# uber/aresdb

Hardware: AMD Instinct MI355X
Metric: rows/sec, 1B-row filter -> group-by-agg (whole job) (higher is better)
Workload: dtype u32 keys / f64 sums; 1 GPU; C3: filter d1<90 -> dims [floor(ts,3600), d1, d2, d3] (4 x uint32) -> SUM(m float32 -> float64) via HashReduce, validity bitmaps with 1% nulls, shard resident in HBM; rows_per_gpu=1000000000, batch_rows=67108864, batches=15, streams_per_query=2, parallelism=1 shard(s), one per GPU

## Files before the change

aresdb_amd/abi.py:

```python
import ctypes as C
import os

_HERE = os.path.dirname(os.path.abspath(__file__))
REPO_ROOT = os.path.dirname(_HERE)
LIB_DIR = os.environ.get("ARES_LIB_DIR") or os.path.join(_HERE, "lib")

AGGR_SUM_UNSIGNED, AGGR_SUM_SIGNED, AGGR_SUM_FLOAT = 1, 2, 3
AGGR_MIN_UNSIGNED, AGGR_MIN_SIGNED, AGGR_MIN_FLOAT = 4, 5, 6
AGGR_MAX_UNSIGNED, AGGR_MAX_SIGNED, AGGR_MAX_FLOAT = 7, 8, 9
AGGR_HLL, AGGR_AVG_FLOAT = 10, 11

(Bool, Int8, Uint8, Int16, Uint16, Int32, Uint32, Float32, Int64, Uint64, Float64, GeoPoint,
 UUID) = range(13)
ConstInt, ConstFloat, ConstGeoPoint, ConstUUID = range(4)
(Negate, Not, BitwiseNot, IsNull, IsNotNull, Noop, GetWeekStart, GetMonthStart, GetQuarterStart,
 GetYearStart, GetDayOfMonth, GetDayOfYear, GetMonthOfYear, GetQuarterOfYear, GetHLLValue,
 ArrayLength) = range(16)
(And, Or, Equal, NotEqual, LessThan, LessThanOrEqual, GreaterThan, GreaterThanOrEqual, Plus, Minus,
 Multiply, Divide, Mod, BitwiseAnd, BitwiseOr, BitwiseXor, Floor, ArrayContains,
 ArrayElementAt) = range(19)
(VectorPartyInput, ScratchSpaceInput, ConstantInput, ForeignColumnInput,
 ArrayVectorPartyInput) = range(5)
ScratchSpaceOutput, MeasureOutput, DimensionOutput = range(3)
NUM_DIM_WIDTH = 5
# ... 55 lines not shown


class ForeignColumnVector(C.Structure):
    _fields_ = [("RecordIDs", C.c_void_p), ("Batches", C.c_void_p), ("BaseBatchID", C.c_int32),
                ("NumBatches", C.c_int32), ("NumRecordsInLastBatch", C.c_int32),
                ("TimezoneLookup", C.c_void_p), ("TimezoneLookupSize", C.c_int16),
                ("DataType", C.c_int), ("DefaultValue", DefaultValue)]


class ArrayVectorPartySlice(C.Structure):
    _fields_ = [("OffsetLengthVector", C.c_void_p), ("ValueOffsetAdj", C.c_uint32),
                ("DataType", C.c_int), ("Length", C.c_uint32)]


class _InputUnion(C.Union):
    _fields_ = [("Constant", ConstantVector), ("VP", VectorPartySlice),
                ("ScratchSpace", ScratchSpaceVector), ("ForeignVP", ForeignColumnVector),
                ("ArrayVP", ArrayVectorPartySlice)]


class InputVector(C.Structure):
    _fields_ = [("Vector", _InputUnion), ("Type", C.c_int)]


class DimensionVector(C.Structure):
    _fields_ = [("DimValues", C.c_void_p), ("HashValues", C.c_void_p), ("IndexVector", C.c_void_p),
                ("VectorCapacity", C.c_int), ("NumDimsPerDimWidth", C.c_uint8 * NUM_DIM_WIDTH)]


class DimensionOutputVector(C.Structure):
    _fields_ = [("DimValues", C.c_void_p), ("DimNulls", C.c_void_p), ("DataType", C.c_int)]


class MeasureOutputVector(C.Structure):
    _fields_ = [("Values", C.c_void_p), ("DataType", C.c_int), ("AggFunc", C.c_int)]


class _OutputUnion(C.Union):
    _fields_ = [("ScratchSpace", ScratchSpaceVector), ("Dimension", DimensionOutputVector),
                ("Measure", MeasureOutputVector)]


class OutputVector(C.Structure):
    _fields_ = [("Vector", _OutputUnion), ("Type", C.c_int)]


class GeoShapeBatch(C.Structure):
    _fields_ = [("LatLongs", C.c_void_p), ("TotalNumPoints", C.c_int32), ("TotalWords", C.c_uint8)]


class FusedExpr(C.Structure):
    _fields_ = [("lhs", InputVector), ("rhs", InputVector), ("arity", C.c_int), ("functor", C.c_int),
                ("outType", C.c_int)]


class FusedSelect(C.Structure):
    _fields_ = [("numFilters", C.c_int), ("filters", FusedExpr * 4), ("numDims", C.c_int),
                ("dims", FusedExpr * 8)]


class FusedJoin(C.Structure):
    _fields_ = [("key", InputVector), ("index", CuckooHashIndex)]


class FusedJoinSelect(C.Structure):
    _fields_ = [("numFilters", C.c_int), ("filters", FusedExpr * 4), ("numJoins", C.c_int), ("joins", FusedJoin * 2),
                ("numForeignFilters", C.c_int), ("foreignFilters", FusedExpr * 4), ("foreignFilterJoin", C.c_int * 4),
                ("numDims", C.c_int), ("dims", FusedExpr * 8), ("dimJoin", C.c_int * 8)]


class JoinedColumn(C.Structure):
    _fields_ = [("column", InputVector), ("out", C.c_void_p)]


class JoinColumns(C.Structure):
    _fields_ = [("numFilters", C.c_int), ("filters", FusedExpr * 4), ("join", FusedJoin), ("numColumns", C.c_int),
                ("columns", JoinedColumn * 4)]


class GeoShapeColumn(C.Structure):
    _fields_ = [("numFilters", C.c_int), ("filters", FusedExpr * 4), ("shapes", GeoShapeBatch), ("points", InputVector),
                ("inOrOut", C.c_int), ("out", C.c_void_p)]


class LocalTimeColumn(C.Structure):
    _fields_ = [("numFilters", C.c_int), ("filters", FusedExpr * 4), ("time", InputVector), ("join", FusedJoin),
                ("zone", InputVector), ("outType", C.c_int), ("out", C.c_void_p)]


ABI_SIZES = {CGoCallResHandle: 16, RecordID: 8, CuckooHashIndex: 40, DefaultValue: 24,
             VectorPartySlice: 56, ScratchSpaceVector: 16, ConstantVector: 24,
             ForeignColumnVector: 72, ArrayVectorPartySlice: 24, InputVector: 80,
             DimensionVector: 40, DimensionOutputVector: 24, MeasureOutputVector: 16,
             OutputVector: 32, GeoShapeBatch: 16}

_VP, _S, _I = C.c_void_p, C.c_void_p, C.c_int

ALGORITHM_SYMBOLS = {
    "InitIndexVector": [_VP, C.c_uint32, _I, _S, _I],
    "HashLookup": [InputVector, _VP, _VP, _I, _VP, C.c_uint32, CuckooHashIndex, _S, _I],
    "UnaryTransform": [InputVector, OutputVector, _VP, _I, _VP, C.c_uint32, _I, _S, _I],
    "UnaryFilter": [InputVector, _VP, _VP, _I, _VP, _I, _VP, C.c_uint32, _I, _S, _I],
    "BinaryTransform": [InputVector, InputVector, OutputVector, _VP, _I, _VP, C.c_uint32, _I, _S, _I],
    "BinaryFilter": [InputVector, InputVector, _VP, _VP, _I, _VP, _I, _VP, C.c_uint32, _I, _S, _I],
    "Sort": [DimensionVector, _I, _S, _I],
    "Reduce": [DimensionVector, _VP, DimensionVector, _VP, _I, _I, _I, _S, _I],
# ... 55 lines not shown
        for p in (memory_path, algorithm_path):
            if not os.path.exists(p):
                raise FileNotFoundError(
                    f"{name}: shared library {p} is missing — build it first "
                    f"(python -c 'import __graft_entry__ as g; g.build()')")
        self._mem = C.CDLL(memory_path, mode=os.RTLD_NOW | os.RTLD_LOCAL)
        self._algo = self._mem if algorithm_path == memory_path else \
            C.CDLL(algorithm_path, mode=os.RTLD_NOW | os.RTLD_LOCAL)
        self.algorithm_path, self.memory_path = algorithm_path, memory_path
        for sym, argtypes in ALGORITHM_SYMBOLS.items():
            fn = getattr(self._algo, sym)
            fn.argtypes, fn.restype = argtypes, CGoCallResHandle
            setattr(self, "_" + sym, fn)
        for sym, argtypes in MEMORY_SYMBOLS.items():
            fn = getattr(self._mem, sym)
            fn.argtypes, fn.restype = argtypes, CGoCallResHandle
            setattr(self, "_" + sym, fn)
        self._mem.GetFlags.argtypes, self._mem.GetFlags.restype = [], C.c_uint32
        self.has_profiler = hasattr(self._algo, "AresProfilerEnable")
        if self.has_profiler:
            self._algo.AresProfilerEnable.argtypes, self._algo.AresProfilerEnable.restype = [C.c_int], None
            self._algo.AresProfilerReport.argtypes = [C.c_char_p, C.c_size_t]
            self._algo.AresProfilerReport.restype = C.c_size_t

    def call(self, sym, *args):
        return _check(getattr(self, "_" + sym)(*args))

    def mem_driver_calls(self, device=0):
        if not hasattr(self._mem, "AresMemDriverCalls"):
            return None
        m, f, t = C.c_size_t(0), C.c_size_t(0), C.c_size_t(0)
        self._mem.AresMemDriverCalls.argtypes = [C.c_int, C.POINTER(C.c_size_t), C.POINTER(C.c_size_t), C.POINTER(C.c_size_t)]
        self._mem.AresMemDriverCalls.restype = None
        self._mem.AresMemDriverCalls(device, C.byref(m), C.byref(f), C.byref(t))
        return {"mallocs": m.value, "frees": f.value, "trims": t.value}

    def rtc_wait(self):
        if not hasattr(self._algo, "AresRtcWait"):
            return None
        c = (C.c_long * 3)()
        self._algo.AresRtcWait.argtypes, self._algo.AresRtcWait.restype = [C.POINTER(C.c_long)], C.c_size_t
        n = self._algo.AresRtcWait(c)
        return {"kernels": int(n), "compiles": int(c[0]), "disk_hits": int(c[1]), "evictions": int(c[2])}

    def reload_env(self):
        if hasattr(self._algo, "AresReloadEnv"):
            self._algo.AresReloadEnv.argtypes, self._algo.AresReloadEnv.restype = [], None
            self._algo.AresReloadEnv()

    def flags(self):
        return self._mem.GetFlags()

    @property
    def has_fused_select(self):
        return hasattr(self._algo, "AresFusedFilterSelect")

    def fused_filter_select(self, query, batch_rows, limit, out_keys, stream=None, device=0):
        fn = self._algo.AresFusedFilterSelect
        fn.argtypes = [C.POINTER(FusedSelect), C.c_int, C.c_int, DimensionVector, _S, _I]
        fn.restype = CGoCallResHandle
        return _check(fn(C.byref(query), int(batch_rows), int(limit), out_keys, stream, device))

    def select_stats(self):
        c = (C.c_ulonglong * 4)()
        self._algo.AresSelectStats.argtypes, self._algo.AresSelectStats.restype = [C.POINTER(C.c_ulonglong)], None
        self._algo.AresSelectStats(c)
        return {"batches": int(c[0]), "declined": int(c[1]), "tiles": int(c[2]), "rows": int(c[3])}

    @property
    def has_fused_join_select(self):
        return hasattr(self._algo, "AresFusedFilterJoinSelect")

    def fused_filter_join_select(self, query, batch_rows, limit, out_keys, stream=None, device=0):
        fn = self._algo.AresFusedFilterJoinSelect
        fn.argtypes = [C.POINTER(FusedJoinSelect), C.c_int, C.c_int, DimensionVector, _S, _I]
        fn.restype = CGoCallResHandle
        return _check(fn(C.byref(query), int(batch_rows), int(limit), out_keys, stream, device))

    def select_join_stats(self):
        c = (C.c_ulonglong * 5)()
        self._algo.AresSelectJoinStats.argtypes, self._algo.AresSelectJoinStats.restype = [C.POINTER(C.c_ulonglong)], None
        self._algo.AresSelectJoinStats(c)
        return {"batches": int(c[0]), "declined": int(c[1]), "tiles": int(c[2]), "rows": int(c[3]), "probed": int(c[4])}

    @property
    def has_join_columns(self):
        return hasattr(self._algo, "AresJoinColumnsRun")

    def join_column_bytes(self, rows, dtype):
        fn = self._algo.AresJoinColumnBytes
        fn.argtypes, fn.restype = [C.c_int, C.c_int], C.c_size_t
        return int(fn(int(rows), int(dtype)))

    def join_columns_run(self, query, batch_rows, stream=None, device=0):
        fn = self._algo.AresJoinColumnsRun
        fn.argtypes = [C.POINTER(JoinColumns), C.c_int, C.POINTER(VectorPartySlice), _S, _I]
        fn.restype = CGoCallResHandle
        slices = (VectorPartySlice * 4)()
        res = _check(fn(C.byref(query), int(batch_rows), slices, stream, device))
        assert res == batch_rows
        return slices

    def join_column_stats(self):
        c = (C.c_ulonglong * 4)()
        self._algo.AresJoinColumnStats.argtypes, self._algo.AresJoinColumnStats.restype = [C.POINTER(C.c_ulonglong)], None
        self._algo.AresJoinColumnStats(c)
# ... 90 lines not shown
```

aresdb_amd/csrc/algo/common.hpp:

```cpp
#pragma once

#include <hip/hip_runtime.h>

#include <atomic>
#include <chrono>
#include <cstdint>
#include <cstdio>
#include <cstdlib>
#include <cstring>
#include <stdexcept>
#include <string>

#include "ares_algorithm.h"

namespace ares {

class AlgorithmError : public std::runtime_error {
 public:
  explicit AlgorithmError(const std::string &m) : std::runtime_error(m) {}
};

void slow_trace(const char *what, double ms);
bool hr_trace_enabled();
class SlowScope {
 public:
  explicit SlowScope(const char *what) : what_(what), t0_(std::chrono::steady_clock::now()) {}
  ~SlowScope() {
    const double ms = std::chrono::duration<double, std::milli>(std::chrono::steady_clock::now() - t0_).count();
    if (ms > 5.0) slow_trace(what_, ms);
  }
  SlowScope(const SlowScope &) = delete;
  SlowScope &operator=(const SlowScope &) = delete;

 private:
  const char *what_;
  std::chrono::steady_clock::time_point t0_;
};
inline void hip_check(hipError_t e, const char *what) {
  if (e != hipSuccess) {
    (void)hipGetLastError();
    throw AlgorithmError(std::string("ERROR: ") + what + ": " + hipGetErrorString(e));
  }
}

template <class F>
inline void hip_check_timed(F &&call, const char *what) {
  SlowScope slow(what);
  hip_check(call(), what);
}
#define hip_check(expr, what) hip_check_timed([&]() -> hipError_t { return (expr); }, what)

extern void (*g_memNoteActivity)();
inline void mem_note_activity() {
  if (g_memNoteActivity) g_memNoteActivity();
}
inline void check_launch(const char *what) {
  mem_note_activity();
  hip_check(hipGetLastError(), what);
}

void flush_deferred(int device);
bool fuse_pending_into_hash_reduce(int device, hipStream_t stream, const DimensionVector &in, const uint8_t *inValues,
                                   const DimensionVector &out, uint8_t *outValues, int valueBytes, int length, int aggFunc,
                                   int *groups);
void invalidate_filter_journal(int device, const uint32_t *indexVector);
bool global_table_forced();
bool deferral_hooks_active();
void grouped_note_write(int device, const void *ptr, size_t bytes);
void grouped_note_write(int device, const DimensionVector &v);
void grouped_materialize_for_read(int device, const void *ptr, size_t bytes);
void grouped_trim(int device);
void flush_deferred_for_inputs(int device, const void *a, size_t aBytes, const void *b, size_t bBytes);
void flush_deferred_for_vector(int device, const DimensionVector &v, const void *values, size_t valueBytes);
void drop_skipped_outputs(int device, const void *a, size_t aBytes, const void *b, size_t bBytes);

bool defer_fill(int device, hipStream_t stream, void *dst, size_t bytes, uint64_t pattern, int unit);
bool pending_fill_exact(int device, const void *dst, size_t bytes, uint64_t *pattern, int *unit);
bool pending_fill_tail(int device, const void *base, int width, int length, int *prev, uint64_t *pattern);
void retire_fills_for_write(int device, const void *ptr, size_t bytes);
void materialize_fills_for_read(int device, const void *ptr, size_t bytes);
void launch_pending_writers(int device, const void *ptr, size_t bytes);
bool virtual_iota_peek(int device, const uint32_t *indexVector, int n, bool consume = false);
void materialize_index_vector(int device, const uint32_t *indexVector);
void settle_dimension_vector(int device, const DimensionVector &v, bool rowsOnly = false);
void temp_stats(size_t *handedOut, size_t *cached);

struct CallStream {
  hipStream_t stream;
  bool known;
};
extern thread_local CallStream t_callStream;
class CallStreamScope {
 public:
  CallStreamScope(void *stream, const char *entry) : saved_(t_callStream), slow_(entry) {
    t_callStream = CallStream{reinterpret_cast<hipStream_t>(stream), true};
  }
  ~CallStreamScope() { t_callStream = saved_; }
  CallStreamScope(const CallStreamScope &) = delete;
  CallStreamScope &operator=(const CallStreamScope &) = delete;

 private:
  CallStream saved_;
  SlowScope slow_;
};

#define ARES_ABI_BEGIN_NOFLUSH(device)                 \
  CGoCallResHandle resHandle = {nullptr, nullptr};     \
  try {                                                \
    ares::hip_check(hipSetDevice(device), "hipSetDevice");  \
    ares::CallStreamScope callStreamScope_(cudaStream, __func__);  \
    ares::mem_note_activity();                                      \
    (void)ares::deferral_hooks_active();

#define ARES_ABI_BEGIN(device)     \
  ARES_ABI_BEGIN_NOFLUSH(device)   \
  ares::flush_deferred(device);

#define ARES_ABI_END(name)                                            \
  }                                                                   \
  catch (std::exception & e) {                                        \
    fprintf(stderr, "Exception happened when doing %s: %s\n", name, e.what()); \
// ... 93 lines not shown
```

aresdb_amd/csrc/algo/hash_reduce_lds.hip:

```cpp
#include <hip/hip_runtime.h>

#include <atomic>
#include <functional>
#include <map>
#include <mutex>
#include <string>
#include <unordered_map>

#include <memory>
#include <mutex>
#include <vector>

#include "aggregate.hpp"
#include "common.hpp"
#include "device_model.hpp"
#include "ares_extensions.h"
#include "dim_layout.hpp"
#include "fast_eval.hpp"
#include "hash_reduce_lds.hpp"
#include "hr_kernels.hpp"
#include "hr_rtc.hpp"
#include "sort_reduce_fused.hpp"

namespace ares {
// ... 273 lines not shown
  ws.capA = ((2ull * (static_cast<uint64_t>(rowsA) / numParts) + 2 * kSlots) | 63ull) + 18;
  ws.capB = 0;
  ws.lineRecords = lineRecords;
  size_t bBytes = 0;
  if (streams > 0) {
    const uint64_t mean = (static_cast<uint64_t>(rowsB) / (static_cast<uint64_t>(numParts) * streams)) << record_stream_slack();
    if (lineRecords == static_cast<int>(kCompactLineRecords)) {
      ws.capB = static_cast<uint32_t>(((2 * mean + 64) / kCompactLineRecords + 2) | 1ull);
      bBytes = 128ull * ws.capB * numParts * streams;
    } else if (lineRecords) {
      ws.capB = static_cast<uint32_t>(((2 * mean + 64 + 7) / 8 * 8) | 8ull);
      bBytes = sizeof(uint32_t) * rwB * static_cast<size_t>(ws.capB) * numParts * streams;
    } else {
      ws.capB = static_cast<uint32_t>(((2 * mean + 64) | 15ull) + 6);
      bBytes = sizeof(uint32_t) * rwB * static_cast<size_t>(ws.capB) * numParts * streams;
    }
  }
  bBytes = (bBytes + 255) / 256 * 256;
  const size_t headBytes = (sizeof(uint32_t) * (numParts + 8) + 255) / 256 * 256;
  const size_t countsBytes = (sizeof(uint32_t) * static_cast<size_t>(numParts) * (streams > 0 ? streams : 1) + 255) / 256 * 256;
  const size_t aBytes = (sizeof(uint4) * ws.capA * numParts + 255) / 256 * 256;
  r.buf.reset(new StreamBuffer(headBytes + countsBytes + aBytes + bBytes + 256, stream));
  uint8_t *base = r.buf->as<uint8_t>();
  ws.cursorsA = reinterpret_cast<uint32_t *>(base);
  ws.outCount = ws.cursorsA + numParts;
  ws.countsB = reinterpret_cast<uint32_t *>(base + headBytes);
  ws.recA = reinterpret_cast<uint4 *>(base + headBytes + countsBytes);
  ws.recB = reinterpret_cast<uint32_t *>(base + headBytes + countsBytes + aBytes);
  r.headBytes = headBytes;
  hip_check(hipMemsetAsync(base, 0, headBytes, stream), "hipMemsetAsync");
}

struct MergeResult {
  uint32_t groups, overflow, stale, needGeneric;
};
MergeResult read_result(const Workspace &ws, hipStream_t stream) {
  uint32_t w[4] = {0, 0, 0, 0};
  read_back_u32(ws.outCount, w, 4, stream);
  return MergeResult{w[0], w[1], w[2], w[3]};
}
uint32_t *result_slot() {
  static EnvSwitch<bool> on("ARES_RESULT_PINNED", [](const char *e) { return e && e[0] == '1'; });
  return on.get() ? reinterpret_cast<uint32_t *>(pinned_words()) : nullptr;
}
MergeResult read_result_pinned(hipStream_t stream) {
  hip_check(hipStreamSynchronize(stream), "hipStreamSynchronize");
  const volatile uint32_t *w = result_slot();
  return MergeResult{w[0], w[1], w[2], w[3]};
}

}

void grouped_note_write(int device, const void *ptr, size_t bytes) {
  sorted_state_note_write(device, ptr, bytes);
  const uint8_t *lo = static_cast<const uint8_t *>(ptr);
  const uint8_t *hi = lo + (bytes ? bytes : 1);
  std::lock_guard<std::mutex> lock(g_groupedMutex);
  for (size_t i = 0; i < g_grouped.size();) {
    GroupedState &st = g_grouped[i];
    if (st.device == device && state_overlaps(st, lo, hi)) {
      const uint8_t *vlo = st.values, *vhi = st.values + static_cast<size_t>(st.valueBytes) * st.size;
      if (st.lazyValues && !(lo <= vlo && vhi <= hi)) materialize_values(st);
      g_grouped.erase(g_grouped.begin() + i);
    } else {
      i++;
    }
  }
}

void grouped_materialize_for_read(int device, const void *ptr, size_t bytes) {
  if (!ptr) return;
  const uint8_t *lo = static_cast<const uint8_t *>(ptr);
  const uint8_t *hi = lo + (bytes ? bytes : 1);
  std::lock_guard<std::mutex> lock(g_groupedMutex);
  for (GroupedState &st : g_grouped) {
    if (st.device != device || !st.lazyValues) continue;
    const uint8_t *vlo = st.values, *vhi = st.values + static_cast<size_t>(st.valueBytes) * st.size;
    if (vlo < hi && lo < vhi) materialize_values(st);
  }
}

void grouped_trim(int device) {
  std::vector<void *> idle;
  {
    std::lock_guard<std::mutex> lock(g_rangesMutex);
    for (size_t i = 0; i < g_freeRanges.size();)
      if (g_freeRanges[i].first == device) {
        idle.push_back(g_freeRanges[i].second);
        g_freeRanges[i] = g_freeRanges.back();
        g_freeRanges.pop_back();
      } else {
        i++;
      }
    for (size_t i = 0; i < g_freeImages.size();)
      if (g_freeImages[i].first == device) {
        idle.push_back(g_freeImages[i].second);
        g_freeImages[i] = g_freeImages.back();
        g_freeImages.pop_back();
      } else {
        i++;
      }
  }
  for (void *p : idle) (void)hipFree(p);
}

void grouped_note_write(int device, const DimensionVector &v) {
// ... 97 lines not shown
      memset(&none, 0, sizeof(none));
      rtc_merge_launch(leanMerge, none, inputKeys.DimValues, capacity, inputValues, static_cast<uint32_t>(start), outputKeys.DimValues,
                       capacity, outputValues, ws, stream, nullptr, result_slot());
    } else {
      generic_merge();
    }
    res = (leanMerge && result_slot()) ? read_result_pinned(stream) : read_result(ws, stream);
    mem_note_dim_rows(device, outputKeys, 0, res.groups);
    mem_note_write(device, outputValues, static_cast<size_t>(a.width) * res.groups);
    if (leanMerge && res.needGeneric && !res.overflow && !(grouped && res.stale)) {
      hip_check(hipMemsetAsync(ws.outCount, 0, 4 * sizeof(uint32_t), stream), "hipMemsetAsync");
      if (outRanges) hip_check(hipMemsetAsync(outRanges, 0, kRangesBytes, stream), "hipMemsetAsync");
      generic_merge();
      res = read_result(ws, stream);
      mem_note_dim_rows(device, outputKeys, 0, res.groups);
      mem_note_write(device, outputValues, static_cast<size_t>(a.width) * res.groups);
    }
#undef ARES_HR_MERGE_ND
#undef ARES_HR_MERGE
    if (hr_trace_enabled())
      fprintf(stderr, "hash_reduce_lds: length %d start %d rows %d streams %d capA %llu capB %u partBits %d -> groups %u overflow %u stale %u\n",
              length, start, rows, streams, static_cast<unsigned long long>(ws.capA), ws.capB, partBits, res.groups, res.overflow, res.stale);
    r.buf->mark_idle();
    if (grouped && res.stale) {
      grouped_note_write(device, inputKeys.DimValues, static_cast<size_t>(L.rowBytes) * capacity);
      grouped = false;
      continue;
    }
    break;
  }
  if (res.overflow) {
    static bool told = false;
    if (!told) {
      told = true;
      fprintf(stderr, "libalgorithm: a hash-partition region overflowed (skewed hashes?): HashReduce falls back to the global table\n");
    }
    return -1;
  }
  if (outRanges) {
    GroupedState s{device, outputKeys.DimValues, outputValues, capacity, slots, a.width, static_cast<int>(res.groups),
                   partBits, outRangesRef};
    if (res.groups > 0) grouped_register(s);
  }
  return static_cast<int>(res.groups);
}

static void fused_note_first_batch(size_t shape, int groups) {
  if (!shape || groups < 0) return;
  std::lock_guard<std::mutex> lock(g_shapeMutex);
  if (g_firstBatchGroups.size() > 4096) g_firstBatchGroups.clear();
  g_firstBatchGroups[shape] = groups;
}

int fused_hash_reduce_run(int device, const FusedPlanD &plan, int batchRows, const DimensionVector &prevKeys,
                          const uint8_t *prevValues, int prevSize, const DimensionVector &outKeys, uint8_t *outValues,
                          const AggSpec &a, hipStream_t stream) {
  SlotWidths slots;
  if (!slot_widths(outKeys.NumDimsPerDimWidth, &slots)) return kFusedUnavailable;
  const int nd = slots.nd;
  const bool narrow = fused_plan_narrow(plan, nd);
  const int mw = plan.measureWidth;
  const int64_t length = static_cast<int64_t>(batchRows) + prevSize;
  if (length == 0) return 0;
  const int partBits = std::max(part_bits_for(length), narrow ? 2 : 0);
  const int numParts = 1 << partBits;
  const size_t prevCapacity = static_cast<size_t>(prevKeys.VectorCapacity);
  const size_t outCapacity = static_cast<size_t>(outKeys.VectorCapacity);
  if (narrow && !(batchRows > 0 && rtc_scan_available())) return kFusedUnavailable;
  GroupedState outOld;
  const bool outFound = image_enabled() && grouped_lookup(device, outKeys.DimValues, outValues, outCapacity, slots, mw, &outOld);
  grouped_note_write(device, outValues, static_cast<size_t>(mw) * outCapacity);
  grouped_note_write(device, outKeys.DimValues, slots.row_bytes() * outCapacity);
  GroupedState prev;
  const bool found = prevSize > 0 && grouped_lookup(device, prevKeys.DimValues, prevValues, prevCapacity, slots, mw, &prev) &&
                     prev.partBits == partBits && prev.size == prevSize;
  bool grouped = found && prev.ranges != nullptr;
  const std::shared_ptr<uint32_t> outRangesRef = grouped_enabled() ? take_ranges(device) : nullptr;
  uint32_t *outRanges = outRangesRef.get();
  MergeResult res{0, 0, 0, 0};
  hr::Widen widen;
  widen.mode = mw == 8 ? 1 : 0;
  widen.rk = plan.measure.f.rk;
  widen.dtype = plan.measureDtype;
  size_t shape = 0;
  int expected = prevSize;
  bool known = prevSize > 0;
  const bool rtc = batchRows > 0 && rtc_scan_available();
  if (rtc && prevSize == 0) {
    const RtcSpec spec = rtc_spec_scan(plan, nd, 0, false);
    shape = std::hash<std::string>()(std::string(reinterpret_cast<const char *>(&spec), sizeof(spec)));
    std::lock_guard<std::mutex> lock(g_shapeMutex);
    auto it = g_firstBatchGroups.find(shape);
    if (it != g_firstBatchGroups.end()) {
      expected = it->second;
      known = true;
    }
  }
  const int chunkTiles = compact_enabled() ? rtc_compact_chunk_tiles(batchRows, partBits) : 0;
  const bool compact = chunkTiles > 0;
  const RtcKind leanKind = compact ? RTC_SCAN_COMPACT : RTC_SCAN_LINES16;
  RtcKernel lean, table, tableMerge, narrowMerge;
  SlowScope slowWhole("fused_hash_reduce_run");
  const bool wantLean = rtc && expected >= lean_min_groups() && (known || lean_min_groups() <= 0);
  const bool wantTable = rtc && !wantLean && (known || narrow);
  if (wantLean) lean = rtc_lookup(device, rtc_spec_scan(plan, nd, partBits, compact));
  else if (wantTable) table = rtc_lookup(device, rtc_spec_table_scan(plan, nd, partBits, a, widen));
  int imageMode = 0;
  RtcKernel imageMerge;
  std::shared_ptr<uint8_t> imageOut;
  uint32_t knownOut = 0;
  if (image_enabled() && wantLean && lean) {
    if (found && prev.image) imageMode = 2;
    else if (prevSize == 0 || grouped) imageMode = 1;
    if (imageMode) imageMerge = rtc_lookup(device, rtc_spec_merge(plan, nd, partBits, a, widen, compact, false, imageMode));
    if (!imageMerge) imageMode = 0;
  }
  if (imageMode == 2) {
    const bool mine = outFound && outOld.lineage == prev.lineage && outOld.image && outOld.image != prev.image &&
                      outOld.partBits == partBits && outOld.size <= prevSize && prev.parentGen != 0 && outOld.gen == prev.parentGen;
    knownOut = mine ? static_cast<uint32_t>(outOld.size) : 0u;
    imageOut = mine ? outOld.image : take_image(device);
    if (imageOut && !mine) hip_check(hipMemsetAsync(image_counts(imageOut.get()), 0xFF, sizeof(uint32_t) * kMaxPartitions, stream), "hipMemsetAsync");
  } else {
    if (imageMode == 1) imageOut = take_image(device);
    if (prevSize > 0) grouped_materialize_for_read(device, prevValues, static_cast<size_t>(mw) * prevSize);
  }
  if (imageMode && !imageOut) {
    imageMode = 0;
    knownOut = 0;
    if (prevSize > 0) grouped_materialize_for_read(device, prevValues, static_cast<size_t>(mw) * prevSize);
  }
  {
    if (hr_trace_enabled())
      fprintf(stderr, "fused_hash_reduce_run: batch %d prev %d partBits %d | found %d (state: size %d partBits %d ranges %d image %d lazy %d) grouped %d "
                      "| lean %d table %d compact %d narrow %d -> image mode %d knownOut %u\n",
              batchRows, prevSize, partBits, found ? 1 : 0, found ? prev.size : -1, found ? prev.partBits : -1, found && prev.ranges ? 1 : 0,
              found && prev.image ? 1 : 0, found && prev.lazyValues ? 1 : 0, grouped ? 1 : 0, lean ? 1 : 0, table ? 1 : 0, compact ? 1 : 0,
              narrow ? 1 : 0, imageMode, knownOut);
  }
  if (narrow && !imageMode) {
    narrowMerge = rtc_lookup(device, rtc_spec_merge(plan, nd, partBits, a, widen, wantLean && compact,
                                                    wantTable || (prevSize > 0 && !grouped)));
    if (!narrowMerge) return kFusedUnavailable;
  }
  if (narrow && !(wantLean ? lean : table)) return kFusedUnavailable;
  bool launched = false;
  for (;;) {
    const bool prevToA = narrow && prevSize > 0 && !grouped && imageMode != 2;
    if (narrow && !imageMode) {
      narrowMerge = rtc_lookup(device, rtc_spec_merge(plan, nd, partBits, a, widen, lean && compact, table || prevToA));
      if (!narrowMerge) return launched ? -1 : kFusedUnavailable;
      if (table) tableMerge = narrowMerge;
    }
    launched = true;
    const int streams = batchRows > 0 ? (lean ? rtc_scan_grid(batchRows) : table ? 0 : grid_for(batchRows)) : 0;
    Regions r;
    {
      SlowScope slow("make_regions");
      const int64_t rowsA = !lean ? length : (prevSize > 0 && !grouped && imageMode != 2) ? prevSize : 0;
      make_regions(r, partBits, rowsA, batchRows, streams, lean ? 4 : 3, stream,
                   !lean ? 0 : compact ? static_cast<int>(kCompactLineRecords) : 8);
    }
    Workspace &ws = r.ws;
    ws.widen = widen;
    ws.chunkRows = static_cast<uint32_t>(chunkTiles) * 4096u;
    ws.rowBase = static_cast<uint32_t>(prevSize);
    ws.prevRanges = (grouped && imageMode != 2) ? prev.ranges.get() : nullptr;
    ws.outRanges = outRanges;
    Workspace wsPrev = ws;
    wsPrev.streams = 0;
    RtcKernel leanMerge = imageMode ? imageMerge
                          : narrow  ? (lean ? narrowMerge : nullptr)
                          : (lean && (prevSize == 0 || grouped)) ? rtc_lookup(device, rtc_spec_merge(plan, nd, partBits, a, widen, compact)) : nullptr;
    RtcImageArgs imageArgs{nullptr, nullptr, nullptr, nullptr, 0u};
    if (imageMode) {
      imageArgs.in = imageMode == 2 ? prev.image.get() : nullptr;
      imageArgs.inCount = imageMode == 2 ? image_counts(prev.image.get()) : nullptr;
      imageArgs.out = imageOut.get();
      imageArgs.outCount = image_counts(imageOut.get());
      imageArgs.knownOut = knownOut;
    }
    const RtcImageArgs *imagePtr = imageMode ? &imageArgs : nullptr;
    if (prevToA) {
      const DimLayoutD prevLayout = make_dim_layout(prevKeys.NumDimsPerDimWidth);
      const int64_t tiles = (static_cast<int64_t>(prevSize) + kTileRows - 1) / kTileRows;
      ARES_LAUNCH("hr_partition_kernel", hr_partition_kernel, static_cast<int>(tiles < 256 ? tiles : 256), kThreads, stream,
                  prevKeys.DimValues, prevLayout, prevCapacity, prevValues, a, prevSize, wsPrev);
    }
    if (outRanges && !leanMerge && !tableMerge) hip_check(hipMemsetAsync(outRanges, 0, kRangesBytes, stream), "hipMemsetAsync");
#define ARES_FUSED_CASE(ND)                                                                                            \
  case ND:                                                                                                             \
    if (prevSize > 0 && !grouped && !narrow && imageMode != 2) {                                                       \
      if (mw == 8)                                                                                                     \
        ARES_LAUNCH("hr_partition4_kernel", (hr_partition4_kernel<ND, 8>), grid_for(prevSize), kThreads, stream,        \
                    prevKeys.DimValues, prevCapacity, prevValues, 0u, a, prevSize, wsPrev, 0);                         \
      else                                                                                                             \
        ARES_LAUNCH("hr_partition4_kernel", (hr_partition4_kernel<ND, 4>), grid_for(prevSize), kThreads, stream,        \
                    prevKeys.DimValues, prevCapacity, prevValues, 0u, a, prevSize, wsPrev, 0);                         \
    }                                                                                                                  \
    if (batchRows > 0 && lean)                                                                                         \
      rtc_scan_launch(lean, leanKind, plan, static_cast<uint32_t>(prevSize), batchRows, ws, stream);                   \
    else if (batchRows > 0 && table)                                                                                   \
      rtc_scan_launch(table, RTC_SCAN_TABLE, plan, static_cast<uint32_t>(prevSize), batchRows, ws, stream);            \
    else if (batchRows > 0)                                                                                            \
      ARES_LAUNCH("hr_fused_scan_kernel", hr_fused_scan_kernel<ND>, streams, kThreads, stream, plan,                   \
                  static_cast<uint32_t>(prevSize), a, batchRows, ws);                                                  \
    if (leanMerge || tableMerge)                                                                                       \
      rtc_merge_launch(leanMerge ? leanMerge : tableMerge, plan, prevKeys.DimValues, prevCapacity, prevValues,         \
                       static_cast<uint32_t>(prevSize), outKeys.DimValues, outCapacity, outValues, ws, stream, imagePtr, \
                       result_slot());                                                                                 \
    else if (lean)                                                                                                     \
      ARES_LAUNCH("hr_fused_merge_kernel", (hr_fused_merge_kernel<ND, 4>), numParts, kThreads, stream, plan,            \
                  prevKeys.DimValues, prevCapacity, prevValues, static_cast<uint32_t>(prevSize), outKeys.DimValues,    \
                  outCapacity, outValues, a, ws);                                                                      \
    else                                                                                                               \
      ARES_LAUNCH("hr_fused_merge_kernel", (hr_fused_merge_kernel<ND, 3>), numParts, kThreads, stream, plan,            \
                  prevKeys.DimValues, prevCapacity, prevValues, static_cast<uint32_t>(prevSize), outKeys.DimValues,    \
                  outCapacity, outValues, a, ws);                                                                      \
    break;
    switch (nd) {
      ARES_FUSED_CASE(1) ARES_FUSED_CASE(2) ARES_FUSED_CASE(3) ARES_FUSED_CASE(4)
      default:
        if (batchRows > 0 && lean) rtc_scan_launch(lean, leanKind, plan, static_cast<uint32_t>(prevSize), batchRows, ws, stream);
        else if (batchRows > 0 && table) rtc_scan_launch(table, RTC_SCAN_TABLE, plan, static_cast<uint32_t>(prevSize), batchRows, ws, stream);
        rtc_merge_launch(leanMerge ? leanMerge : tableMerge, plan, prevKeys.DimValues, prevCapacity, prevValues, static_cast<uint32_t>(prevSize),
                         outKeys.DimValues, outCapacity, outValues, ws, stream, imagePtr, result_slot());
        break;
    }
    {
      SlowScope slow("read_result");
      res = ((leanMerge || tableMerge) && result_slot()) ? read_result_pinned(stream) : read_result(ws, stream);
    }
    if (imageMode == 2) res.groups += static_cast<uint32_t>(prevSize);
    if (imageMode == 2) {
      if (res.groups > knownOut) mem_note_dim_rows(device, outKeys, knownOut, res.groups - knownOut);
    } else {
      mem_note_dim_rows(device, outKeys, 0, res.groups);
      mem_note_write(device, outValues, static_cast<size_t>(mw) * res.groups);
    }
    if ((narrow || imageMode == 2) && res.needGeneric) {
      r.buf->mark_idle();
      return -1;
    }
    if (imageMode == 1 && res.needGeneric) imageMode = 0;
    if (leanMerge && res.needGeneric && !res.overflow && !(grouped && res.stale)) {
      hip_check(hipMemsetAsync(ws.outCount, 0, 4 * sizeof(uint32_t), stream), "hipMemsetAsync");
      if (outRanges) hip_check(hipMemsetAsync(outRanges, 0, kRangesBytes, stream), "hipMemsetAsync");
      switch (nd) {
#define ARES_FUSED_REMERGE(ND)                                                                                         \
  case ND:                                                                                                             \
    ARES_LAUNCH("hr_fused_merge_kernel", (hr_fused_merge_kernel<ND, 4>), numParts, kThreads, stream, plan,              \
                prevKeys.DimValues, prevCapacity, prevValues, static_cast<uint32_t>(prevSize), outKeys.DimValues,      \
                outCapacity, outValues, a, ws);                                                                        \
    break;
        ARES_FUSED_REMERGE(1) ARES_FUSED_REMERGE(2) ARES_FUSED_REMERGE(3) ARES_FUSED_REMERGE(4)
#undef ARES_FUSED_REMERGE
      }
      res = read_result(ws, stream);
      mem_note_dim_rows(device, outKeys, 0, res.groups);
      mem_note_write(device, outValues, static_cast<size_t>(mw) * res.groups);
    }
#undef ARES_FUSED_CASE
    r.buf->mark_idle();
    if (grouped && res.stale) {
      grouped_note_write(device, prevKeys.DimValues, slots.row_bytes() * prevCapacity);
      grouped = false;
      imageMode = 0;
      continue;
    }
    if (res.overflow && lean && grow_record_stream_slack()) continue;
    break;
  }
  if (res.overflow) {
    return -1;
  }
  fused_note_first_batch(shape, static_cast<int>(res.groups));
  if (shape && !lean && !table) {
    if (static_cast<int>(res.groups) >= lean_min_groups()) {
      (void)rtc_lookup(device, rtc_spec_scan(plan, nd, partBits, compact));
      (void)rtc_lookup(device, rtc_spec_merge(plan, nd, partBits, a, widen, compact));
    } else {
      (void)rtc_lookup(device, rtc_spec_table_scan(plan, nd, partBits, a, widen));
    }
  }
  if (outRanges) {
    GroupedState s{device, outKeys.DimValues, outValues, outCapacity, slots, mw, static_cast<int>(res.groups), partBits, outRangesRef};
    if (imageMode == 2) {
      s.ranges = nullptr;
      s.image = imageOut;
      s.lineage = prev.lineage;
      s.gen = ++g_generation;
      s.parentGen = prev.gen;
      s.lazyValues = true;
    } else if (imageMode == 1) {
      s.image = imageOut;
      s.lineage = ++g_lineage;
      s.gen = ++g_generation;
    }
    if (res.groups > 0) grouped_register(s);
  }
  return static_cast<int>(res.groups);
}

namespace {

struct NotFusable : std::runtime_error {
  explicit NotFusable(const std::string &why) : std::runtime_error("not fusable: " + why) {}
};

void fused_expr(const AresFusedExpr &e, bool compareOnly, int batchRows, hipStream_t stream, FusedPlanD &plan, int maxCols,
                FusedExpr &out) {
  if (e.arity != 1 && e.arity != 2) throw NotFusable("arity");
  if (e.lhs.Type != VectorPartyInput || (e.arity == 2 && e.rhs.Type != ConstantInput))
    throw NotFusable("operands must be a main-table column and a constant");
  if (static_cast<int64_t>(e.lhs.Vector.VP.Length) < batchRows) throw NotFusable("column shorter than the batch");
  InputVector ins[2] = {e.lhs, e.arity == 2 ? e.rhs : e.lhs};
  EvalParams p;
  CallTemps temps;
  build_params(ins, e.arity, stream, nullptr, nullptr, 0, e.functor, p, temps);
  FastOperands f;
  if (!fast_operands(p, f, compareOnly)) throw NotFusable("expression shape");
  out.col = fused_column(plan, f, maxCols, compareOnly ? kFusedReuseFirst : kFusedNoReuse);
  if (out.col < 0) throw NotFusable("too many distinct columns");
  out.f = f;
  out.f.vals = nullptr;
  out.f.nulls = nullptr;
  out.outKind = e.outType == Int32 ? K_I32 : e.outType == Uint32 ? K_U32 : K_F32;
}
// ... 57 lines not shown
```

aresdb_amd/csrc/algo/hash_reduce_lds.hpp:

```cpp
#pragma once

#include <hip/hip_runtime.h>

#include "aggregate.hpp"
#include "ares_algorithm.h"
#include "dim_layout.hpp"
#include "fast_eval.hpp"

namespace ares {

bool hash_reduce_lds_supported(const AggSpec &a);

int hash_reduce_lds(int device, const DimensionVector &inputKeys, const uint8_t *inputValues,
                    const DimensionVector &outputKeys, uint8_t *outputValues, const AggSpec &a, int length,
                    hipStream_t stream);

constexpr int kFusedCols = 10, kFusedFilters = 6, kFusedDims = 8;
constexpr int kGenericFusedDims = 4;
constexpr int kExtensionFilters = 4;
constexpr int kSortVectorValueBytes = 32;
inline bool sort_vector_layout_supported(const uint8_t numDimsPerDimWidth[NUM_DIM_WIDTH]) {
  int nd = 0;
  for (int w = 0; w < NUM_DIM_WIDTH; w++) nd += numDimsPerDimWidth[w];
  const bool wide = numDimsPerDimWidth[0] || numDimsPerDimWidth[1];
  return nd >= 1 && nd <= kFusedDims && (!wide || dim_value_bytes(numDimsPerDimWidth) <= static_cast<size_t>(kSortVectorValueBytes));
}
struct FusedColumn {
  const uint32_t *vals;
  const uint8_t *nulls;
  uint32_t bitOff;
  uint32_t step;
};
struct FusedExpr {
  FastOperands f;
  int col;
  int outKind;
};
struct FusedPlanD {
  int numCols;
  FusedColumn cols[kFusedCols];
  int numFilters;
  FusedExpr filters[kFusedFilters];
  FusedExpr dims[kFusedDims];
  FusedExpr measure;
  int measureDtype, measureWidth;
  uint64_t identity;
  uint8_t dimWidth[kFusedDims];
  int measureAvg;
};
inline int fused_dim_width(const FusedPlanD &p, int d) { return p.dimWidth[d] ? p.dimWidth[d] : 4; }
inline int fused_col_step(const FusedPlanD &p, int c) { return p.cols[c].step ? static_cast<int>(p.cols[c].step) : 4; }
inline bool fused_plan_narrow(const FusedPlanD &p, int nd) {
  if (nd > kGenericFusedDims) return true;
  for (int d = 0; d < nd; d++)
    if (fused_dim_width(p, d) != 4) return true;
  for (int c = 0; c < p.numCols; c++)
    if (fused_col_step(p, c) != 4) return true;
  return false;
}

inline FusedColumn fused_column_of(const FastOperands &f) { return FusedColumn{f.vals, f.nulls, f.bitOff, static_cast<uint32_t>(f.step ? f.step : 4)}; }
inline FastOperands fused_strip(FastOperands f) {
  f.vals = nullptr;
  f.nulls = nullptr;
  f.idx = nullptr;
  f.pad = 0;
  return f;
}
inline int fused_kind_of(int dtype) { return (dtype == Int32 || dtype == Int16 || dtype == Int8) ? K_I32 : (dtype == Uint32 || dtype == Uint16 || dtype == Uint8) ? K_U32 : K_F32; }
enum FusedReuse { kFusedNoReuse, kFusedReuseFirst, kFusedReuseLast };
inline int fused_column(FusedPlanD &plan, const FastOperands &f, int maxCols, FusedReuse reuse) {
  const FusedColumn col = fused_column_of(f);
  int found = -1;
  for (int c = 0; reuse != kFusedNoReuse && c < plan.numCols; c++)
    if (plan.cols[c].vals == col.vals && plan.cols[c].nulls == col.nulls && plan.cols[c].bitOff == col.bitOff && plan.cols[c].step == col.step &&
        (found < 0 || reuse == kFusedReuseLast))
      found = c;
  if (found >= 0) return found;
  if (plan.numCols >= maxCols) return -1;
  plan.cols[plan.numCols] = col;
  return plan.numCols++;
}
inline void fused_plan_dim(FusedPlanD &plan, int d, const FastOperands &f, const SinkD &sink, int width) {
  plan.cols[d] = fused_column_of(f);
  plan.dims[d].f = fused_strip(f);
  plan.dims[d].col = d;
  plan.dims[d].outKind = fused_kind_of(sink.dtype);
  plan.dimWidth[d] = static_cast<uint8_t>(width);
}
inline void fused_plan_measure(FusedPlanD &plan, int nd, const FastOperands &f, const SinkD &sink, int valueBytes) {
  plan.cols[nd] = fused_column_of(f);
  plan.measure.f = fused_strip(f);
  plan.measure.col = nd;
  plan.measure.outKind = fused_kind_of(sink.dtype);
  plan.measureDtype = sink.dtype;
  plan.measureWidth = valueBytes;
  plan.identity = sink.identity;
  plan.measureAvg = sink.agg == AGGR_AVG_FLOAT ? 1 : 0;
  plan.numCols = nd + 1;
}
inline void fused_plan_const_measure(FusedPlanD &plan, int nd, uint64_t constBits, int dtype, int valueBytes) {
  plan.measure.col = -1;
  plan.measure.f.bbits = static_cast<uint32_t>(constBits);
  plan.measureDtype = dtype;
  plan.measureWidth = valueBytes;
  plan.numCols = nd;
}
inline bool fused_plan_filters(FusedPlanD &plan, const FastOperands *filters, size_t count) {
  if (count > static_cast<size_t>(kFusedFilters)) return false;
  for (size_t k = 0; k < count; k++) {
    const int col = fused_column(plan, filters[k], kFusedCols, kFusedReuseLast);
    if (col < 0) return false;
    plan.filters[k].f = fused_strip(filters[k]);
    plan.filters[k].col = col;
    plan.filters[k].outKind = K_BOOL;
  }
  plan.numFilters = static_cast<int>(count);
  return true;
}
inline void fused_plan_vector_columns(FusedPlanD &plan, const uint8_t *dimValues, size_t capacity, int nd, const int *widths, uint32_t rowBase) {
  plan.numCols = nd + 1;
  size_t valueBytes = 0, off = 0;
  for (int d = 0; d < nd; d++) valueBytes += static_cast<size_t>(widths ? widths[d] : 4);
  for (int d = 0; d < nd; d++) {
    const size_t w = static_cast<size_t>(widths ? widths[d] : 4);
    plan.cols[d].vals = reinterpret_cast<const uint32_t *>(dimValues + off * capacity + w * rowBase);
    plan.cols[d].nulls = dimValues + valueBytes * capacity + static_cast<size_t>(d) * capacity + rowBase;
    off += w;
  }
}

constexpr int kFusedUnavailable = -2;
int record_stream_slack();
bool grow_record_stream_slack();
int fused_hash_reduce_run(int device, const FusedPlanD &plan, int batchRows, const DimensionVector &prevKeys,
                          const uint8_t *prevValues, int prevSize, const DimensionVector &outKeys, uint8_t *outValues,
                          const AggSpec &a, hipStream_t stream);

}
```

aresdb_amd/csrc/algo/hr_rtc.hip:

```cpp
#include <dlfcn.h>
#include <hip/hip_runtime.h>
#include <sys/stat.h>
#include <cerrno>
#include <unistd.h>

#include <atomic>
#include <chrono>
#include <condition_variable>
#include <fstream>
#include <memory>
#include <mutex>
#include <string>
#include <thread>
#include <unordered_map>
#include <vector>

#include "common.hpp"
#include "hash_reduce_lds.hpp"
#include "hr_kernels.hpp"
#include "hr_rtc.hpp"

namespace ares {

bool phases_enabled() {
  static const bool on = [] { const char *e = getenv("ARES_HR_PHASES"); return e && e[0] == '1'; }();
  return on;
}

namespace {

typedef struct _hiprtcProgram *RtcProgram;
struct RtcApi {
  int (*create)(RtcProgram *, const char *, const char *, int, const char **, const char **) = nullptr;
  int (*compile)(RtcProgram, int, const char **) = nullptr;
  int (*logSize)(RtcProgram, size_t *) = nullptr;
  int (*log)(RtcProgram, char *) = nullptr;
  int (*codeSize)(RtcProgram, size_t *) = nullptr;
  int (*code)(RtcProgram, char *) = nullptr;
  int (*destroy)(RtcProgram *) = nullptr;
  int (*version)(int *, int *) = nullptr;
  bool ok = false;
};
const RtcApi &rtc_api() {
  static const RtcApi api = [] {
    RtcApi a;
    const char *e = getenv("ARES_RTC");
    if (e && e[0] == '0') return a;
    void *h = dlopen("libhiprtc.so", RTLD_NOW | RTLD_LOCAL);
    if (!h) h = dlopen("libhiprtc.so.7", RTLD_NOW | RTLD_LOCAL);
    if (!h) h = dlopen("/opt/rocm/lib/libhiprtc.so", RTLD_NOW | RTLD_LOCAL);
    if (!h) return a;
    a.create = reinterpret_cast<decltype(a.create)>(dlsym(h, "hiprtcCreateProgram"));
    a.compile = reinterpret_cast<decltype(a.compile)>(dlsym(h, "hiprtcCompileProgram"));
    a.logSize = reinterpret_cast<decltype(a.logSize)>(dlsym(h, "hiprtcGetProgramLogSize"));
    a.log = reinterpret_cast<decltype(a.log)>(dlsym(h, "hiprtcGetProgramLog"));
    a.codeSize = reinterpret_cast<decltype(a.codeSize)>(dlsym(h, "hiprtcGetCodeSize"));
    a.code = reinterpret_cast<decltype(a.code)>(dlsym(h, "hiprtcGetCode"));
    a.destroy = reinterpret_cast<decltype(a.destroy)>(dlsym(h, "hiprtcDestroyProgram"));
    a.version = reinterpret_cast<decltype(a.version)>(dlsym(h, "hiprtcVersion"));
    a.ok = a.create && a.compile && a.logSize && a.log && a.codeSize && a.code && a.destroy;
    return a;
  }();
  return api;
}

struct RtcArgs {
  const uint32_t *vals[kFusedCols];
  const uint8_t *nulls[kFusedCols];
  uint32_t *recB;
  uint32_t *countsB;
  uint32_t *overflow;
  uint64_t *phases;
  uint4 *recA;
  uint32_t *cursorsA;
  uint64_t capA;
  uint32_t bitOff[kFusedCols];
  uint32_t rowBase;
  int length;
  uint32_t capB;
  uint32_t chunkTiles;
  uint32_t k[kNumConsts];
  uint32_t pad;
};
static_assert(sizeof(RtcArgs) % 8 == 0, "Args is passed as one buffer");

struct RtcMergeArgs {
  const uint32_t *vals[kFusedCols];
  const uint8_t *nulls[kFusedCols];
  const uint32_t *recB;
  const uint32_t *countsB;
  const uint32_t *prevRanges;
  const uint8_t *prevDims;
  const uint8_t *prevValues;
  uint8_t *dimOut;
  uint8_t *outValues;
  uint32_t *outCount;
  uint32_t *outRanges;
  uint64_t prevCapacity, outCapacity;
  uint32_t bitOff[kFusedCols];
  uint32_t capB, streams, prevSize, chunkRows;
  uint64_t *phases;
  uint32_t k[kNumConsts];
  uint32_t pad;
  const uint4 *recA;
  const uint32_t *cursorsA;
  uint64_t capA;
  const uint4 *imgIn;
  uint4 *imgOut;
  const uint32_t *imgInCount;
  uint32_t *imgOutCount;
  uint32_t *hostOut;
  uint32_t knownOut, pad2;
};
static_assert(sizeof(RtcMergeArgs) % 8 == 0, "MArgs is passed as one buffer");

}

struct RtcEntry {
  int device = 0;
  std::mutex m;
  std::condition_variable cv;
  bool ready = false;
  bool codeReady = false;
  bool fromDisk = false;
  std::vector<char> code;
// ... 334 lines not shown
      }
    } else if (rtc_async() && !wait) {
      std::thread([e, source, name = std::string(entry)] { compile_entry(e, source, name); }).detach();
    } else {
      compile_entry(e, source, entry);
    }
  }
  std::unique_lock<std::mutex> lock(e->m);
  if (!e->ready && !e->codeReady) {
    if (rtc_async() && !wait) return nullptr;
    e->cv.wait(lock, [&] { return e->ready || e->codeReady; });
  }
  if (!e->ready) {
    (void)hipSetDevice(device);
    load_entry(*e, entry);
    e->cv.notify_all();
  }
  return e->fn ? e : nullptr;
}

template <typename Args>
void fill_columns(Args &args, const FusedPlanD &plan) {
  memset(&args, 0, sizeof(args));
  for (int c = 0; c < plan.numCols; c++) {
    args.vals[c] = plan.cols[c].vals;
    args.nulls[c] = plan.cols[c].nulls;
    args.bitOff[c] = plan.cols[c].bitOff;
  }
  for (int d = 0; d < kFusedDims; d++) args.k[const_slot_dim(d)] = plan.dims[d].f.bbits;
}

struct PhaseReport {
  uint64_t *dev = nullptr;
  int launches = 0;
  uint64_t *buffer(size_t workgroups) {
    if (!dev) hip_check(hipMalloc(reinterpret_cast<void **>(&dev), sizeof(uint64_t) * 8 * workgroups), "hipMalloc");
    return dev;
  }
  bool fetch(std::vector<uint64_t> &h, int workgroups, hipStream_t stream) {
    h.resize(static_cast<size_t>(8) * workgroups);
    hip_check(hipMemcpyAsync(h.data(), dev, sizeof(uint64_t) * h.size(), hipMemcpyDeviceToHost, stream), "hipMemcpyAsync");
    hip_check(hipStreamSynchronize(stream), "hipStreamSynchronize");
    return ++launches <= 3 || launches % 64 == 0;
  }
};

void launch(const RtcKernel &kernel, void *args, size_t size, unsigned grid, hipStream_t stream, const char *name) {
  void *config[] = {HIP_LAUNCH_PARAM_BUFFER_POINTER, args, HIP_LAUNCH_PARAM_BUFFER_SIZE, &size, HIP_LAUNCH_PARAM_END};
  KernelTimer timer(name, stream);
  hip_check(hipModuleLaunchKernel(kernel->fn, grid, 1, 1, hr::kThreads, 1, 1, 0, stream, nullptr, config), "hipModuleLaunchKernel");
}

void launch_scan(const RtcKernel &kernel, const FusedPlanD &plan, uint32_t rowBase, int length, const hr::Workspace &ws, int grid,
                 uint32_t chunkTiles, uint32_t pad, hipStream_t stream, const char *name) {
  RtcArgs args;
  fill_columns(args, plan);
  for (int k = 0; k < plan.numFilters && k < kFusedFilters; k++)
    args.k[const_slot_filter(k)] = host_cvt32(plan.filters[k].f.bbits, plan.filters[k].f.bkind, plan.filters[k].f.I);
  args.k[const_slot_measure()] = plan.measure.f.bbits;
  args.recB = ws.recB;
  args.countsB = ws.countsB;
  args.overflow = ws.outCount + 1;
  args.recA = ws.recA;
  args.cursorsA = ws.cursorsA;
  args.capA = ws.capA;
  args.rowBase = rowBase;
  args.length = length;
  args.capB = ws.capB;
  args.chunkTiles = chunkTiles;
  args.pad = pad;
  static PhaseReport report;
  if (phases_enabled()) args.phases = report.buffer(hr::kMaxStreams);
  launch(kernel, &args, sizeof(args), static_cast<unsigned>(grid), stream, name);
  std::vector<uint64_t> h;
  if (phases_enabled() && report.fetch(h, grid, stream)) {
    double sum[7] = {0, 0, 0, 0, 0, 0, 0};
    for (int g = 0; g < grid; g++)
      for (int k = 0; k < 7; k++) sum[k] += static_cast<double>(h[static_cast<size_t>(8) * g + k]);
    const double n = grid * 1e3;
    fprintf(stderr, "%s phases (launch %d, %d workgroups, %d rows): kcycles per workgroup: eval+count %.1f, scan %.1f, scatter %.1f, lines %.1f, leftovers %.1f, drain %.1f, last lines %.1f\n",
            name, report.launches, grid, length, sum[0] / n, sum[1] / n, sum[2] / n, sum[3] / n, sum[4] / n, sum[5] / n, sum[6] / n);
  }
}

}

bool rtc_scan_available() { return rtc_api().ok; }

int rtc_scan_grid(int64_t rows) {
  const int64_t tiles = (rows + 4095) / 4096;
  return static_cast<int>(tiles < hr::kMaxStreams ? (tiles < 1 ? 1 : tiles) : hr::kMaxStreams);
}

int rtc_compact_chunk_tiles(int64_t rows, int partBits) {
  if (partBits < 3 || rows <= 0) return 0;
  const int64_t tiles = (rows + 4095) / 4096;
  const int64_t grid = rtc_scan_grid(rows);
  const int64_t chunk = (tiles + grid - 1) / grid;
  return chunk <= (1ll << (partBits - 3)) ? static_cast<int>(chunk) : 0;
}

RtcKernel rtc_lookup(int device, const RtcSpec &spec, bool wait) {
  if (!rtc_api().ok) return nullptr;
  std::string key(reinterpret_cast<const char *>(&spec), sizeof(spec));
  key.append(reinterpret_cast<const char *>(&device), sizeof(device));
  RtcCache &c = cache();
  {
    std::lock_guard<std::mutex> lock(c.frontMu);
    auto it = c.front.find(key);
    if (it != c.front.end()) return it->second;
  }
  RtcKernel k = compiled_kernel(device, rtc_source(spec), rtc_entry_name(spec.kind), wait);
  if (k) {
    std::lock_guard<std::mutex> lock(c.frontMu);
    if (c.front.size() >= 64) c.front.clear();
    c.front.emplace(key, k);
  }
  return k;
}

void rtc_scan_launch(const RtcKernel &kernel, RtcKind kind, const FusedPlanD &plan, uint32_t rowBase, int length, const hr::Workspace &ws,
                     hipStream_t stream) {
  const int grid = kind == RTC_SCAN_TABLE ? rtc_scan_grid(length) : ws.streams;
  const uint32_t chunkTiles = kind == RTC_SCAN_COMPACT ? ws.chunkRows / 4096u : 0u;
  launch_scan(kernel, plan, rowBase, length, ws, grid, chunkTiles, 0u, stream,
              kind == RTC_SCAN_TABLE ? "hr_table_scan_rtc" : rtc_entry_name(kind));
}

void rtc_vector_scan_launch(const RtcKernel &kernel, RtcKind kind, const uint8_t *dimValues, size_t capacity, const void *measures, int nd,
                            const int *widths, uint32_t rowBase, int length, const hr::Workspace &ws, hipStream_t stream, int totalPartBits,
                            bool spread) {
  FusedPlanD plan;
  memset(&plan, 0, sizeof(plan));
  fused_plan_vector_columns(plan, dimValues, capacity, nd, widths, rowBase);
  plan.cols[nd].vals = static_cast<const uint32_t *>(measures);
  launch_scan(kernel, plan, rowBase, length, ws, ws.streams, totalPartBits > 0 ? static_cast<uint32_t>(32 - totalPartBits) : 0u,
              spread ? 1u : 0u, stream, kind == RTC_SORT_VECTOR_SCAN ? "sr_vector_scan_rtc" : rtc_entry_name(kind));
}

void rtc_merge_launch(const RtcKernel &kernel, const FusedPlanD &plan, const uint8_t *prevDims, size_t prevCapacity, const uint8_t *prevValues,
                      uint32_t prevSize, uint8_t *dimOut, size_t outCapacity, uint8_t *outValues, const hr::Workspace &ws,
                      hipStream_t stream, const RtcImageArgs *image, uint32_t *hostOut) {
  RtcMergeArgs args;
  fill_columns(args, plan);
  args.recB = ws.recB;
  args.countsB = ws.countsB;
  args.prevRanges = ws.prevRanges;
  args.prevDims = prevDims;
  args.prevValues = prevValues;
  args.dimOut = dimOut;
  args.outValues = outValues;
  args.outCount = ws.outCount;
  args.outRanges = ws.outRanges;
  args.prevCapacity = prevCapacity;
  args.outCapacity = outCapacity;
  args.capB = ws.capB;
  args.recA = ws.recA;
  args.cursorsA = ws.cursorsA;
  args.capA = ws.capA;
  args.streams = static_cast<uint32_t>(ws.streams);
  args.prevSize = prevSize;
  args.chunkRows = ws.chunkRows;
  if (image) {
    args.imgIn = reinterpret_cast<const uint4 *>(image->in);
    args.imgOut = reinterpret_cast<uint4 *>(image->out);
    args.imgInCount = image->inCount;
    args.imgOutCount = image->outCount;
    args.knownOut = image->knownOut;
  }
  args.hostOut = hostOut;
  static PhaseReport report;
  if (phases_enabled()) {
    args.phases = report.buffer(hr::kMaxPartitions);
    hip_check(hipMemsetAsync(args.phases, 0, sizeof(uint64_t) * 8 * hr::kMaxPartitions, stream), "hipMemsetAsync");
  }
  launch(kernel, &args, sizeof(args), 1u << ws.partBits, stream, "hr_merge_rtc");
  const int np = 1 << ws.partBits;
  std::vector<uint64_t> h;
  if (phases_enabled() && report.fetch(h, np, stream)) {
// ... 28 lines not shown
```

aresdb_amd/csrc/algo/hr_rtc.hpp:

```cpp
#pragma once

#include <hip/hip_runtime.h>

#include <memory>

#include "hr_rtc_gen.hpp"

namespace ares {
namespace hr { struct Workspace; }

struct RtcEntry;
using RtcKernel = std::shared_ptr<RtcEntry>;

bool rtc_scan_available();
int rtc_scan_grid(int64_t rows);
int rtc_compact_chunk_tiles(int64_t rows, int partBits);

RtcKernel rtc_lookup(int device, const RtcSpec &spec, bool wait = false);

void rtc_scan_launch(const RtcKernel &kernel, RtcKind kind, const FusedPlanD &plan, uint32_t rowBase, int length, const hr::Workspace &ws,
                     hipStream_t stream);
void rtc_vector_scan_launch(const RtcKernel &kernel, RtcKind kind, const uint8_t *dimValues, size_t capacity, const void *measures, int nd,
                            const int *widths, uint32_t rowBase, int length, const hr::Workspace &ws, hipStream_t stream,
                            int totalPartBits = 0, bool spread = false);
struct RtcImageArgs {
  const void *in;
  void *out;
  const uint32_t *inCount;
  uint32_t *outCount;
  uint32_t knownOut;
};
void rtc_merge_launch(const RtcKernel &kernel, const FusedPlanD &plan, const uint8_t *prevDims, size_t prevCapacity,
                      const uint8_t *prevValues, uint32_t prevSize, uint8_t *dimOut, size_t outCapacity, uint8_t *outValues,
                      const hr::Workspace &ws, hipStream_t stream, const RtcImageArgs *image = nullptr, uint32_t *hostOut = nullptr);

}
```

aresdb_amd/csrc/algo/hr_rtc_gen.hip:

```cpp
#include <cstdio>
#include <functional>
#include <sstream>
#include <string>
#include <vector>

#include "hr_kernels.hpp"
#include "hr_rtc_gen.hpp"

namespace ares {

namespace {

bool int_kind(int k) { return k == K_I32 || k == K_U32; }
bool col_kind(int k) { return k == K_I32 || k == K_U32 || k == K_F32; }

std::string hex(uint32_t v) {
  char b[16];
  snprintf(b, sizeof(b), "0x%08xu", v);
  return b;
}

std::string const_name(int slot) { return "a.k[" + std::to_string(slot) + "]"; }

bool gen_value(const RtcExpr &f, std::ostringstream &o, const char *v, const char *okb, const char *r, const std::string &kc,
// ... 9 lines not shown
      (f.functor == Plus || f.functor == Minus || f.functor == Multiply)) {
    o << "      " << r << " = " << okb << " ? __float_as_uint(__uint_as_float(" << v << ")"
      << (f.functor == Plus ? " + " : f.functor == Minus ? " - " : " * ") << "__uint_as_float(" << kc << ")) : 0u;\n";
    return true;
  }
  if (f.arity != 2 || !intKinds || !int_kind(f.I) || !int_kind(f.bkind) || !f.bok) return false;
  const uint32_t y = f.bbits;
  if (f.divLike) {
    const bool sgn = f.I == K_I32;
    const uint32_t mag = (sgn && static_cast<int32_t>(y) < 0) ? 0u - y : y;
    const bool yneg = sgn && static_cast<int32_t>(y) < 0;
    o << "      {\n";
    if (sgn) o << "        const bool xneg = (i32)" << v << " < 0; const u32 ax = xneg ? 0u - " << v << " : " << v << ";\n";
    else o << "        const u32 ax = " << v << ";\n";
    if (mag == 0) o << "        const u32 q = 0u, m = 0u;\n";
    else if (mag == 1) o << "        const u32 q = ax, m = 0u;\n";
    else o << "        const u32 q = ax / " << hex(mag) << ", m = ax % " << hex(mag) << ";\n";
    if (sgn) {
      o << "        const u32 sq = (xneg != " << (yneg ? "true" : "false") << ") ? 0u - q : q;\n";
      o << "        const u32 sm = xneg ? 0u - m : m;\n";
    } else {
      o << "        const u32 sq = q, sm = m;\n";
    }
    o << "        " << r << " = " << (f.functor == Divide ? "sq" : f.functor == Mod ? "sm" : std::string(v) + " - sm") << ";\n";
    o << "        if (!" << okb << ") " << r << " = 0u;\n      }\n";
    return true;
  }
  if (f.functor == Plus || f.functor == Minus || f.functor == Multiply) {
    o << "      " << r << " = " << okb << " ? (" << v << (f.functor == Plus ? " + " : f.functor == Minus ? " - " : " * ") << kc
      << ") : 0u;\n";
    return true;
  }
  return false;
}

bool gen_compare(const RtcExpr &f, std::ostringstream &o, const char *v, const char *okb, const char *keep, const std::string &kc) {
  if (!col_kind(f.akind) || f.arity != 2) return false;
  const bool sameBits = f.akind == f.I || (f.akind != K_F32 && f.I != K_F32 && f.akind != K_BOOL);
  if (!sameBits || !f.bok) return false;
  if (f.functor < Equal || f.functor > GreaterThanOrEqual) return false;
  if (!(f.I == K_F32 || f.I == K_I32 || f.I == K_U32)) return false;
  const char *op = f.functor == Equal ? "==" : f.functor == NotEqual ? "!=" : f.functor == LessThan ? "<"
                   : f.functor == LessThanOrEqual ? "<=" : f.functor == GreaterThan ? ">" : ">=";
  if (f.I == K_F32) o << "      " << keep << " &= (" << okb << " && (__uint_as_float(" << v << ") " << op << " __uint_as_float(" << kc << "))) ? 1u : 0u;\n";
  else if (f.I == K_I32) o << "      " << keep << " &= (" << okb << " && ((i32)" << v << " " << op << " (i32)" << kc << ")) ? 1u : 0u;\n";
  else o << "      " << keep << " &= (" << okb << " && (" << v << " " << op << " " << kc << ")) ? 1u : 0u;\n";
  return true;
}

bool plain_store(int rk, int outKind) { return rk == outKind || (rk != K_F32 && outKind != K_F32 && rk != K_BOOL); }

std::string args_text() {
  std::ostringstream o;
  o << "struct Args { const u32 *vals[" << kFusedCols << "]; const u8 *nulls[" << kFusedCols << "]; u32 *recB; u32 *countsB; u32 *overflow; u64 *phases;\n"
       "              uint4 *recA; u32 *cursorsA; u64 capA; u32 bitOff[" << kFusedCols << "]; u32 rowBase; int length; u32 capB; u32 chunkTiles;\n"
       "              u32 k[" << kNumConsts << "]; u32 pad; };\n";
  return o.str();
}

const char *kPrelude =
    "__device__ __forceinline__ unsigned int times5(unsigned int r) { unsigned int t; asm(\"v_lshl_add_u32 %0, %1, 2, %1\" : \"=v\"(t) : \"v\"(r)); return t; }\n"
    "#define TIMES5(r) times5(r)\n"
    "typedef unsigned int u32; typedef unsigned long long u64; typedef unsigned char u8; typedef unsigned short u16; typedef int i32; typedef long long i64;\n"
    "struct __attribute__((packed, aligned(1))) PU32x4 { u32 v[4]; };\n"
    "struct __attribute__((packed, aligned(1))) PU32 { u32 v; };\n"
    "struct __attribute__((packed, aligned(1))) PU16 { u16 v; };\n"
    "typedef u32 U4 __attribute__((ext_vector_type(4)));\n"
    "typedef U4 U4a __attribute__((aligned(4)));\n"
    "struct __attribute__((packed, aligned(1))) PU32x2 { u32 v[2]; };\n"
    "typedef u32 U2 __attribute__((ext_vector_type(2)));\n"
    "typedef U2 U2a __attribute__((aligned(2)));\n"
    "typedef u32 U1a __attribute__((aligned(1)));\n"
    "__device__ __forceinline__ u32 rotl(u32 x, int r) { return (x << r) | (x >> (32 - r)); }\n"
    "__device__ __forceinline__ u32 mix(u32 h, u32 k) { k *= 0xcc9e2d51u; k = rotl(k, 15) * 0x1b873593u; h ^= k; return TIMES5(rotl(h, 13)) + 0xe6546b64u; }\n";

void phase_macros(std::ostringstream &o, const RtcSpec &s) {
  if (s.phases)
    o << "#define PH_DECL u64 phT[8] = {0, 0, 0, 0, 0, 0, 0, 0}; u64 phLast = __builtin_readcyclecounter();\n"
         "#define PH(k) { const u64 now = __builtin_readcyclecounter(); phT[k] += now - phLast; phLast = now; }\n"
         "#define PH_OUT if (threadIdx.x == 0u) for (int k = 0; k < 8; k++) a.phases[(u64)blockIdx.x * 8u + k] = phT[k];\n";
  else
    o << "#define PH_DECL\n#define PH(k)\n#define PH_OUT\n";
}

bool gen_widen(std::ostringstream &o, const RtcSpec &s) {
  o << "__device__ __forceinline__ u64 widen(u32 raw) {\n";
  if (s.widenMode == 0) o << "  return raw;\n";
  else if (s.widenDtype == Float64)
    o << (s.widenRk == K_F32 ? "  return (u64)__double_as_longlong((double)__uint_as_float(raw));\n"
          : s.widenRk == K_I32 ? "  return (u64)__double_as_longlong((double)(i32)raw);\n"
                          : "  return (u64)__double_as_longlong((double)raw);\n");
  else
    o << (s.widenRk == K_F32 ? "  return (u64)(i64)__uint_as_float(raw);\n" : s.widenRk == K_I32 ? "  return (u64)(i64)(i32)raw;\n" : "  return (u64)(i64)raw;\n");
  o << "}\n";
  return true;
}

bool gen_agg(std::ostringstream &o, const RtcSpec &s) {
  o << "__device__ __forceinline__ void agg(u64 *slot, u64 bits) {\n";
  switch (s.aggVtype) {
    case V_F64: o << "  __hip_atomic_fetch_add(reinterpret_cast<double *>(slot), __longlong_as_double((long long)bits), __ATOMIC_RELAXED, __HIP_MEMORY_SCOPE_WORKGROUP);\n"; break;
    case V_U64: case V_I64: o << "  __hip_atomic_fetch_add(slot, bits, __ATOMIC_RELAXED, __HIP_MEMORY_SCOPE_WORKGROUP);\n"; break;
    case V_F32: o << "  __hip_atomic_fetch_add(reinterpret_cast<float *>(slot), __uint_as_float((u32)bits), __ATOMIC_RELAXED, __HIP_MEMORY_SCOPE_WORKGROUP);\n"; break;
    case V_U32:
      o << "  __hip_atomic_fetch_" << (s.aggOp == OP_SUM ? "add" : s.aggOp == OP_MIN ? "min" : "max")
        << "(reinterpret_cast<u32 *>(slot), (u32)bits, __ATOMIC_RELAXED, __HIP_MEMORY_SCOPE_WORKGROUP);\n";
      break;
// ... 113 lines not shown
       "      u32 cur = sCursor[tid] + myLines * 8u;\n"
       "      if (cur > a.capB) { *a.overflow = 1u; cur = a.capB; }\n"
       "      sCursor[tid] = cur;\n"
       "      cnt[tid] = 0u;\n"
       "    }\n"
       "    par ^= 1u;\n"
       "    tile = next;\n"
       "    PH(4)\n"
       "  }\n"
       "  __syncthreads();\n"
       "  PH(5)\n"
       "  for (u32 p = tid >> 3; p < NP; p += 128u) {\n"
       "    const u32 left = sLeftN[p], j = tid & 7u, cur = sCursor[p];\n"
       "    const bool fits = cur + 8u <= a.capB;\n"
       "    if (left && fits) myB[(u64)p * a.capB + cur + j] = j < left ? sLeft[p * 7u + j] : make_uint4(0xFFFFFFFFu, 0u, 0u, 0u);\n"
       "    if (left && !fits) *a.overflow = 1u;\n"
       "    if (j == 0u) a.countsB[(u64)blockIdx.x * NP + p] = (left && fits) ? cur + 8u : cur;\n"
       "  }\n"
       "  PH(6)\n"
       "  PH_OUT\n"
       "}\n";
}

static void kernel_body_compact(std::ostringstream &o, const RtcSpec &s) {
  phase_macros(o, s);
  o << "#define STORE_LINE(p, v) (*(p) = (v))\n"
       "#define T 4096u\n#define LR 14u\n#define LEFT 13u\n#define LPL 5u\n"
       "__device__ __forceinline__ u32 lane_up(u32 v, u32 lane, u32 off) { return (u32)__builtin_amdgcn_ds_bpermute((int)((lane - off) << 2), (int)v); }\n"
       "__device__ __forceinline__ u32 or8(u32 v) {\n"
       "  v |= (u32)__builtin_amdgcn_mov_dpp((int)v, 0xB1, 0xF, 0xF, true);\n"
       "  v |= (u32)__builtin_amdgcn_mov_dpp((int)v, 0x4E, 0xF, 0xF, true);\n"
       "  v |= (u32)__builtin_amdgcn_mov_dpp((int)v, 0x141, 0xF, 0xF, true);\n"
       "  return v;\n"
       "}\n"
       "__device__ __forceinline__ u32 wave_incl_scan(u32 v) {\n"
       "  v += (u32)__builtin_amdgcn_update_dpp(0, (int)v, 0x111, 0xF, 0xF, false);\n"
       "  v += (u32)__builtin_amdgcn_update_dpp(0, (int)v, 0x112, 0xF, 0xF, false);\n"
       "  v += (u32)__builtin_amdgcn_update_dpp(0, (int)v, 0x114, 0xF, 0xF, false);\n"
       "  v += (u32)__builtin_amdgcn_update_dpp(0, (int)v, 0x118, 0xF, 0xF, false);\n"
       "  v += (u32)__builtin_amdgcn_update_dpp(0, (int)v, 0x142, 0xA, 0xF, false);\n"
       "  v += (u32)__builtin_amdgcn_update_dpp(0, (int)v, 0x143, 0xC, 0xF, false);\n"
       "  return v;\n"
       "}\n"
       "extern \"C\" __global__ void __launch_bounds__(1024) hr_scan_rtc(Args a) {\n"
       "  __shared__ u64 sRec[T + NP * LEFT];\n"
       "  __shared__ u16 sLo[T + NP * LEFT];\n"
       "  __shared__ u32 sCount[2][NP];\n"
       "  __shared__ u32 sStart[NP];\n"
       "  __shared__ uint2 sLines[(T + NP * LEFT) / LR + 2u];\n"
       "  __shared__ u32 sWave[16];\n"
       "  __shared__ u32 sTotalLines;\n"
       "  const u32 tid = threadIdx.x, lane = tid & 63u, wave = tid >> 6;\n"
       "  for (u32 p = tid; p < NP; p += 1024u) { sCount[0][p] = 0u; sCount[1][p] = 0u; }\n"
       "  u32 myLeftN = 0u, myCursor = 0u;\n"
       "  __syncthreads();\n"
       "  u64 *myB = reinterpret_cast<u64 *>(a.recB) + (u64)blockIdx.x * NP * a.capB * 16u;\n"
       "  const u32 numTiles = ((u32)a.length + T - 1u) / T;\n"
       "  const u32 firstTile = blockIdx.x * a.chunkTiles;\n"
       "  const u32 endTile = firstTile + a.chunkTiles < numTiles ? firstTile + a.chunkTiles : numTiles;\n"
       "  u32 tile = firstTile, par = 0u;\n"
       "  Raw R;\n"
       "  PH_DECL\n"
       "  load_tile(R, a, tile * T + tid * 4u);\n"
       "  const u32 q = tid & 15u, r8 = q & 7u;\n"
       "  const u32 kk = (q >> 3) * 7u + (r8 ? r8 - 1u : 0u);\n"
       "  const u32 sh = r8 ? 9u * (r8 - 1u) : 0u;\n"
       "  while (tile < endTile) {\n"
       "    u32 i0 = tile * T + tid * 4u;\n"
       "    u32 hh[4], cv[4], cw[4], alive[4], rank[4];\n"
       "    const u32 next = tile + 1u;\n"
       "    eval4p(R, a, i0, hh, cv, cw, alive, next * T + tid * 4u);\n"
       "    const u32 rc0 = i0 - firstTile * T;\n"
       "    u32 *cnt = sCount[par];\n"
       "#pragma unroll\n"
       "    for (int j = 0; j < 4; j++) {\n"
       "      rank[j] = 0u;\n"
       "      if (alive[j]) rank[j] = __hip_atomic_fetch_add(&cnt[hh[j] >> (32 - PB)], 1u, __ATOMIC_RELAXED, __HIP_MEMORY_SCOPE_WORKGROUP);\n"
       "    }\n"
       "    __syncthreads();\n"
       "    PH(0)\n"
       "    u32 myCount = 0u, myLeft = 0u;\n"
       "    if (tid < NP) { myCount = cnt[tid]; myLeft = myLeftN; }\n"
       "    const u32 myHave = myCount + myLeft, myLines = myHave / LR;\n"
       "    const u32 packed = (myCount << 16) | myLines;\n"
       "    const u32 incl = wave_incl_scan(packed);\n"
       "    if (lane == 63u) sWave[wave] = incl;\n"
       "    __syncthreads();\n"
       "    u32 before = 0u;\n"
       "#pragma unroll\n"
       "    for (u32 w = 0u; w < (NP + 63u) / 64u; w++) { const u32 t = sWave[w]; before += w < wave ? t : 0u; }\n"
       "    const u32 excl = before + incl - packed;\n"
       "    const u32 myStart = excl >> 16, myLineStart = excl & 0xFFFFu;\n"
       "    if (tid < NP) {\n"
       "      sStart[tid] = myLines ? myStart : T + tid * LEFT + myLeft;\n"
       "      for (u32 c = 0u; c < myLines; c++) sLines[myLineStart + c] = make_uint2(tid | (c << 9) | (myLeft << 18), myStart | (myCursor << 13));\n"
       "      if (tid == NP - 1u) sTotalLines = myLineStart + myLines;\n"
       "    }\n"
       "    __syncthreads();\n"
       "    PH(1)\n"
       "#pragma unroll\n"
       "    for (int j = 0; j < 4; j++)\n"
       "      if (alive[j]) {\n"
       "        const u32 at = sStart[hh[j] >> (32 - PB)] + rank[j], rc = rc0 + (u32)j;\n"
       "        sRec[at] = ((u64)((hh[j] << PB) | (rc >> 9)) << 32) | cv[j];\n"
       "        sLo[at] = (u16)(rc & 511u);\n"
       "      }\n"
       "    __syncthreads();\n"
       "    PH(2)\n"
       "    const u32 totalLines = sTotalLines;\n"
       "    for (u32 L0 = tid >> 4; L0 < totalLines; L0 += 64u * LPL) {\n"
       "      u32 e[LPL], lf[LPL], st[LPL], cu[LPL], lo[LPL];\n"
       "      u64 rec[LPL];\n"
       "#pragma unroll\n"
       "      for (u32 j = 0u; j < LPL; j++) {\n"
       "        const u32 L = L0 + j * 64u;\n"
       "        const uint2 w = L < totalLines ? sLines[L] : make_uint2(0u, 0u);\n"
       "        e[j] = w.x & 0x3FFFFu; lf[j] = w.x >> 18; st[j] = w.y & 0x1FFFu; cu[j] = w.y >> 13;\n"
       "      }\n"
       "#pragma unroll\n"
       "      for (u32 j = 0u; j < LPL; j++) {\n"
       "        const u32 p = e[j] & 511u, idx = (e[j] >> 9) * LR + kk;\n"
       "        const u32 at = idx < lf[j] ? T + p * LEFT + idx : st[j] + idx - lf[j];\n"
       "        rec[j] = sRec[at];\n"
       "        lo[j] = sLo[at];\n"
       "      }\n"
       "#pragma unroll\n"
       "      for (u32 j = 0u; j < LPL; j++) {\n"
       "        const u64 mine = r8 ? (u64)lo[j] << sh : 0ull;\n"
       "        const u64 hdr = ((u64)or8((u32)(mine >> 32)) << 32) | or8((u32)mine);\n"
       "        const u32 p = e[j] & 511u, line = cu[j] + (e[j] >> 9);\n"
       "        if (L0 + j * 64u < totalLines && line < a.capB) STORE_LINE(&myB[((u64)p * a.capB + line) * 16u + q], r8 ? rec[j] : hdr);\n"
       "      }\n"
       "    }\n"
       "    __syncthreads();\n"
       "    PH(3)\n"
       "    if (tid < NP) {\n"
       "      const u32 rem = myHave - myLines * LR;\n"
       "      if (myLines) {\n"
       "        const u32 from = myStart + myLines * LR - myLeft, to = T + tid * LEFT;\n"
       "        u64 t[LEFT]; u16 tl[LEFT];\n"
       "#pragma unroll\n"
       "        for (u32 k = 0u; k < LEFT; k++) { t[k] = sRec[from + k]; tl[k] = sLo[from + k]; }\n"
       "#pragma unroll\n"
       "        for (u32 k = 0u; k < LEFT; k++) { sRec[to + k] = t[k]; sLo[to + k] = tl[k]; }\n"
       "      }\n"
       "      myLeftN = rem;\n"
       "      u32 cur = myCursor + myLines;\n"
       "      if (cur > a.capB) { *a.overflow = 1u; cur = a.capB; }\n"
       "      myCursor = cur;\n"
       "      cnt[tid] = 0u;\n"
       "    }\n"
       "    par ^= 1u;\n"
       "    tile = next;\n"
       "    PH(4)\n"
       "  }\n"
       "  __syncthreads();\n"
       "  if (tid < NP) sLines[tid] = make_uint2(myLeftN, myCursor);\n"
       "  __syncthreads();\n"
       "  PH(5)\n"
       "  for (u32 p = tid >> 4; p < NP; p += 64u) {\n"
       "    const uint2 m = sLines[p];\n"
       "    const u32 left = m.x, cur = m.y;\n"
       "    const bool fits = cur < a.capB, has = r8 && kk < left;\n"
       "    const u64 rec = has ? sRec[T + p * LEFT + kk] : 0ull;\n"
       "    const u64 mine = has ? (u64)sLo[T + p * LEFT + kk] << sh : 0ull;\n"
       "    const u64 hdr = ((u64)or8((u32)(mine >> 32)) << 32) | or8((u32)mine);\n"
       "    if (left && fits) STORE_LINE(&myB[((u64)p * a.capB + cur) * 16u + q], r8 ? rec : hdr);\n"
       "    if (left && !fits) *a.overflow = 1u;\n"
       "    if (q == 0u) a.countsB[(u64)blockIdx.x * NP + p] = cur * LR + ((left && fits) ? left : 0u);\n"
       "  }\n"
       "  PH(6)\n"
       "  PH_OUT\n"
       "}\n";
}

static void kernel_body_table(std::ostringstream &o) {
  o << "#define T 4096u\n#define SLOTS " << hr::kSlots << "u\n#define BUCKETS (SLOTS / 4u)\n#define LIMIT " << (hr::kSlots * 3 / 4)
    << "u\n#define EMPTY 0xFFFFFFFFu\n#define QCAP 128u\n"
       "struct Probe { u32 b, slot; bool done, spill; };\n"
       "__device__ __forceinline__ void probe_round(u32 *sKeys, u32 *sClaims, Probe &q, u32 h) {\n"
       "  const uint4 k = *reinterpret_cast<const uint4 *>(sKeys + 4u * q.b);\n"
       "  const bool e0 = k.x == EMPTY, e1 = k.y == EMPTY, e2 = k.z == EMPTY, e3 = k.w == EMPTY;\n"
       "  const bool m0 = k.x == h, m1 = k.y == h, m2 = k.z == h, m3 = k.w == h;\n"
       "  const bool anyM = m0 | m1 | m2 | m3, anyE = e0 | e1 | e2 | e3;\n"
       "  const u32 mi = m0 ? 0u : m1 ? 1u : m2 ? 2u : 3u, ei = e0 ? 0u : e1 ? 1u : e2 ? 2u : 3u;\n"
       "  const bool active = !q.done, hit = active & anyM;\n"
       "  q.slot = hit ? 4u * q.b + mi : q.slot;\n"
       "  bool claimed = false;\n"
       "  if (active & !anyM & anyE) {\n"
       "    if (__hip_atomic_load(sClaims, __ATOMIC_RELAXED, __HIP_MEMORY_SCOPE_WORKGROUP) >= LIMIT) {\n"
       "      q.spill = true; claimed = true;\n"
       "    } else {\n"
       "      u32 expected = EMPTY;\n"
       "      if (__hip_atomic_compare_exchange_strong(sKeys + 4u * q.b + ei, &expected, h, __ATOMIC_RELAXED, __ATOMIC_RELAXED, __HIP_MEMORY_SCOPE_WORKGROUP)) {\n"
       "        __hip_atomic_fetch_add(sClaims, 1u, __ATOMIC_RELAXED, __HIP_MEMORY_SCOPE_WORKGROUP);\n"
       "        q.slot = 4u * q.b + ei; claimed = true;\n"
       "      }\n"
       "    }\n"
       "  }\n"
       "  q.b = (active & !anyM & !anyE) ? (q.b + 1u) & (BUCKETS - 1u) : q.b;\n"
       "  q.done = q.done | hit | claimed;\n"
       "}\n"
       "__device__ __forceinline__ void insert(const Args &a, u32 *sKeys, u32 *sRows, u64 *sVals, u32 *sClaims, u32 row, u32 h, u32 carried) {\n"
       "  const u64 value = widen(carried);\n"
       "  Probe q; q.b = h & (BUCKETS - 1u); q.slot = 0u; q.done = false; q.spill = h == EMPTY;\n"
       "  for (u32 tries = 0u; tries < BUCKETS + 8u && !q.done && !q.spill; tries++) probe_round(sKeys, sClaims, q, h);\n"
       "  if (q.done && !q.spill) {\n"
       "    __hip_atomic_fetch_min(sRows + q.slot, row, __ATOMIC_RELAXED, __HIP_MEMORY_SCOPE_WORKGROUP);\n"
       "    agg(sVals + q.slot, value);\n"
       "  } else {\n"
       "    const u32 p = PB ? h >> (32 - (PB ? PB : 1)) : 0u;\n"
       "    const u64 at = atomicAdd(a.cursorsA + p, 1u);\n"
       "    if (at < a.capA) a.recA[(u64)p * a.capA + at] = make_uint4(row, h, (u32)value, (u32)(value >> 32));\n"
       "    else *a.overflow = 1u;\n"
       "  }\n"
       "}\n"
       "__device__ __forceinline__ void drain(const Args &a, u32 *queue, u32 first, u32 count, u32 lane, u32 *sKeys, u32 *sRows, u64 *sVals, u32 *sClaims) {\n"
       "  asm volatile(\"s_waitcnt lgkmcnt(0)\" ::: \"memory\");\n"
       "  if (lane < count) {\n"
       "    const u32 e = 3u * (first + lane);\n"
       "    insert(a, sKeys, sRows, sVals, sClaims, queue[e], queue[e + 1u], queue[e + 2u]);\n"
       "  }\n"
// ... 1059 lines not shown
```

aresdb_amd/csrc/algo/transform.hip:

```cpp
#include <hip/hip_runtime.h>

#include <dlfcn.h>

#include <algorithm>
#include <map>
#include <memory>
#include <mutex>
#include <string>
#include <vector>

#include "ares_extensions.h"

#include "binding.hpp"
#include "common.hpp"
#include "device_model.hpp"
#include "dim_layout.hpp"
#include "fast_eval.hpp"
#include "hash_reduce_lds.hpp"
#include "lookback.hpp"
#include "sort_reduce_fused.hpp"

#include "transform_kernels.hpp"

namespace ares {
// ... 85 lines not shown
  std::vector<uintptr_t> tags;
  void add(hipStream_t s) { tags.push_back(hold_tag(s)); }
  void run(int device) const {
    if (g_releaseHeld)
      for (uintptr_t t : tags) g_releaseHeld(device, t);
  }
};

struct LazyFilter {
  FastOperands f;
  uint32_t colRows;
  uint8_t *pred;
  int rowsBefore;
  std::shared_ptr<StreamBuffer> keep;
};
struct RunExpansion {
  const uint8_t *base;
  uint32_t nullsOff, valuesOff, length, bitOff, step, startCount;
  int rows;
  std::shared_ptr<StreamBuffer> copy;
  size_t valuesAt;
};
struct PredictedFilter {
  bool valid = false;
  FastOperands g;
  int count = 0;
  std::shared_ptr<StreamBuffer> bits;
};
struct CompactSpace {
  uint32_t *words = nullptr;
  int tiles = 0, passes = 1;
  static size_t bytes(int tiles, int passes, size_t extraWords) {
    return 64 + 4 * (static_cast<size_t>(tiles) * (2 + passes) + 1 + extraWords);
  }
  uint32_t *total() const { return words; }
  uint32_t *error() const { return words + 1; }
  unsigned int *tickets() const { return words + 2; }
  uint32_t *tileCounts() const { return words + 16; }
  uint32_t *tileOffsets() const { return tileCounts() + tiles; }
  uint32_t *loaded() const { return tileOffsets() + tiles + 1; }
  uint32_t *extra() const { return loaded() + static_cast<size_t>(tiles) * passes; }
};
struct PendingCompact {
  hipStream_t stream;
  uint32_t *idx;
  const uint8_t *pred;
  int n, pad;
  bool virtualIdx;
  std::shared_ptr<StreamBuffer> ws;
  CompactSpace space;
  std::vector<LazyFilter> todo;
  int n0 = 0, applied = 0, lastCount = 0;
  std::shared_ptr<StreamBuffer> bits;
  PredictedFilter predicted;
  uint64_t generation = 0;
};

struct FilterShape {
  int akind, functor, I, bkind;
  uint32_t bbits, bok;
  bool sameColumnAsPrevious;
  bool same_as(const FilterShape &o) const {
    return akind == o.akind && functor == o.functor && I == o.I && bkind == o.bkind && bbits == o.bbits && bok == o.bok &&
           sameColumnAsPrevious == o.sameColumnAsPrevious;
  }
};
struct FilterHistory {
  std::vector<FilterShape> previous, current;
};

struct PendingIota {
  hipStream_t stream;
  uint32_t start;
  int n;
  bool consumed = false;
  bool sorted = false;
};

struct PendingFill {
  hipStream_t stream;
  size_t bytes;
  uint64_t pattern;
  int unit;
  bool streamGone = false;
  const uint32_t *sortIdx = nullptr;
};

struct PendingSort {
  hipStream_t stream;
  DimensionVector keys;
  int length;
  bool reduced = false;
  bool fromVectors = false;
  DimensionVector outKeys;
  uint8_t *inValues = nullptr, *outValues = nullptr;
  int valueBytes = 0, aggFunc = 0, groups = 0;
  bool constMeasure = false;
  uint8_t *fillAt = nullptr;
  PendingFill fill;
};

void hook_on_wait(int device, void *stream);
uintptr_t hook_on_free(int device, void *ptr, size_t bytes);
void hook_on_access(int device, const void *ptr, size_t bytes);
void hook_on_write(int device, const void *ptr, size_t bytes);
void hook_on_stream_destroy(int device, void *stream);
// ... 939 lines not shown
    const int grid = capped_grid((static_cast<int64_t>(n) + kBlock * ITEMS - 1) / (kBlock * ITEMS), 256 * 16);
    ARES_LAUNCH("transform32_kernel", transform32_kernel<ITEMS>, grid, kBlock, stream, p, s, n);
  }
  return n;
}

namespace {
int compute_units(int device) {
  static std::mutex mu;
  static std::map<int, int> known;
  std::lock_guard<std::mutex> lock(mu);
  auto it = known.find(device);
  if (it != known.end()) return it->second;
  int cus = 0;
  if (hipDeviceGetAttribute(&cus, hipDeviceAttributeMultiprocessorCount, device) != hipSuccess || cus < 1) {
    (void)hipGetLastError();
    cus = 256;
  }
  return known[device] = cus;
}
int resident_blocks(int device, const void *kernel, int blockSize) {
  static std::mutex mu;
  static std::map<std::pair<int, const void *>, int> known;
  std::lock_guard<std::mutex> lock(mu);
  auto it = known.find({device, kernel});
  if (it != known.end()) return it->second;
  int perCU = 0;
  if (hipOccupancyMaxActiveBlocksPerMultiprocessor(&perCU, kernel, blockSize, 0) != hipSuccess || perCU < 1) {
    (void)hipGetLastError();
    perCU = 4;
  }
  return known[{device, kernel}] = perCU * compute_units(device);
}

bool row_space_enabled() {
  static EnvSwitch<bool> on("ARES_FILTER_ROWSPACE", [](const char *e) { return !(e && e[0] == '0'); });
  return on.get();
}
bool same_column(const FastOperands &a, const FastOperands &b) { return a.vals == b.vals && a.nulls == b.nulls && a.bitOff == b.bitOff; }
bool same_filter(const FastOperands &a, const FastOperands &b) {
  return same_column(a, b) && a.akind == b.akind && a.arity == b.arity && a.functor == b.functor && a.I == b.I && a.bkind == b.bkind &&
         a.bbits == b.bbits && a.bok == b.bok;
}

bool row_space_eligible(int device, hipStream_t stream, const uint32_t *indexVector, int n, uint32_t colRows) {
  if (!fuse_available() || !row_space_enabled()) return false;
  DeferLock lock(device);
  auto j = t_state->journals.find(indexVector);
  if (j == t_state->journals.end() || !j->second.valid || j->second.stream != stream || j->second.start != 0 ||
      j->second.filters.size() >= static_cast<size_t>(kFusedFilters) || colRows < static_cast<uint32_t>(j->second.n0))
    return false;
  auto c = t_state->compactions.find(indexVector);
  if (j->second.filters.empty()) return n == j->second.n0 && c == t_state->compactions.end();
  return c != t_state->compactions.end() && !c->second.todo.empty() && c->second.stream == stream &&
         c->second.applied + c->second.todo.size() == j->second.filters.size() && c->second.lastCount == n;
}

int run_filter_rows(int device, hipStream_t stream, FastOperands f, uint32_t *indexVector, uint8_t *pred, int n, uint32_t colRows,
                    bool virtualIdx, const std::shared_ptr<StreamBuffer> &keep = nullptr) {
  f.idx = nullptr;
  f.pad = 0;
  f.streaming = 1;
  constexpr int kGridCap = 2048;
  static_assert(2 * kGridCap <= kPinnedWords, "the partial counts are read back in one copy");
  std::shared_ptr<StreamBuffer> bits1, bits2;
  int grid = 0;
  bool two = false;
  FastOperands g = f;
  uint64_t generation = 0;
  {
    DeferLock lock(device);
    auto ins = t_state->compactions.find(indexVector);
    {
      auto jr = t_state->journals.find(indexVector);
      const size_t journalled = (jr != t_state->journals.end() && jr->second.valid) ? jr->second.filters.size() : 0;
      const bool first = ins == t_state->compactions.end() && journalled == 1 && jr->second.n0 == n;
      const bool next = ins != t_state->compactions.end() && !ins->second.todo.empty() && ins->second.stream == stream &&
                        ins->second.applied + ins->second.todo.size() + 1 == journalled && ins->second.lastCount == n;
      if (!first && !next) return -1;
    }
    if (ins == t_state->compactions.end()) {
      PendingCompact fresh{};
      fresh.stream = stream;
      fresh.idx = indexVector;
      fresh.virtualIdx = virtualIdx;
      fresh.n0 = n;
      fresh.applied = 0;
      fresh.lastCount = n;
      ins = t_state->compactions.emplace(indexVector, fresh).first;
    }
    PendingCompact &c = ins->second;
    FilterHistory &h = t_state->filterHistory[stream];
    FilterShape shape{f.akind, f.functor, f.I, f.bkind, f.bbits, f.bok, !c.todo.empty() && same_column(c.todo.back().f, f)};
    const size_t k = h.current.size();
    h.current.push_back(shape);
    if (c.predicted.valid && same_filter(c.predicted.g, f)) {
      const int count = c.predicted.count;
      c.todo.push_back(LazyFilter{f, colRows, pred, n, keep});
      c.bits = c.predicted.bits;
      c.lastCount = count;
      c.predicted = PredictedFilter{};
      auto j = t_state->journals.find(indexVector);
      if (j != t_state->journals.end() && j->second.valid) j->second.lastCount = count;
      return count;
    }
    c.predicted = PredictedFilter{};
    if (k + 1 < h.previous.size() && h.previous[k].same_as(shape) && h.previous[k + 1].sameColumnAsPrevious &&
        h.previous[k + 1].akind == f.akind && c.applied + c.todo.size() + 2 <= static_cast<size_t>(kFusedFilters)) {
      const FilterShape &nx = h.previous[k + 1];
      g.functor = nx.functor;
      g.I = nx.I;
      g.bkind = nx.bkind;
      g.bbits = nx.bbits;
      g.bok = nx.bok;
      two = true;
    }
    const int tiles = pred_tiles(c.n0, 0);
    const bool hasIn = static_cast<bool>(c.bits);
    auto kernel = two ? (hasIn ? &filter_rows_kernel<true, true> : &filter_rows_kernel<true, false>)
                      : (hasIn ? &filter_rows_kernel<false, true> : &filter_rows_kernel<false, false>);
    {
      const int resident = resident_blocks(device, reinterpret_cast<const void *>(kernel), kBlock), cus = compute_units(device);
      const int perUnit = std::max(1, std::min(resident / cus - 1, 6));
      grid = capped_grid(tiles, std::min(kGridCap, cus * perUnit));
    }
    const size_t bitBytes = static_cast<size_t>(tiles) * kBlock * sizeof(uint16_t);
    bits1 = std::make_shared<StreamBuffer>(bitBytes, stream);
    if (two) bits2 = std::make_shared<StreamBuffer>(bitBytes, stream);
    uint32_t *hostPartials = reinterpret_cast<uint32_t *>(pinned_words());
    ARES_LAUNCH("filter_rows_kernel", kernel, grid, kBlock, stream, f, g,
                hasIn ? c.bits->as<uint16_t>() : static_cast<const uint16_t *>(nullptr), bits1->as<uint16_t>(),
                two ? bits2->as<uint16_t>() : static_cast<uint16_t *>(nullptr), c.n0, tiles, hostPartials);
    c.todo.push_back(LazyFilter{f, colRows, pred, n, keep});
    c.bits = bits1;
    c.lastCount = -1;
    generation = ++t_state->filterGeneration;
    c.generation = generation;
  }
  hip_check(hipStreamSynchronize(stream), "hipStreamSynchronize");
  const volatile uint32_t *parts = reinterpret_cast<const volatile uint32_t *>(pinned_words());
  uint32_t count = 0, count2 = 0;
  for (int b = 0; b < grid; b++) {
    count += parts[2 * b];
    count2 += parts[2 * b + 1];
  }
  {
    DeferLock lock(device);
    auto it = t_state->compactions.find(indexVector);
    if (it != t_state->compactions.end() && it->second.generation == generation) {
      it->second.lastCount = static_cast<int>(count);
      if (two) {
        it->second.predicted.valid = true;
        it->second.predicted.g = g;
        it->second.predicted.count = static_cast<int>(count2);
        it->second.predicted.bits = bits2;
      }
    }
    auto j = t_state->journals.find(indexVector);
    if (j != t_state->journals.end() && j->second.valid) j->second.lastCount = static_cast<int>(count);
  }
  return static_cast<int>(count);
}

bool prepare_filter(int device, hipStream_t stream, const EvalParams &p, uint32_t *indexVector, uint8_t *pred, int n,
                    int numForeignTables, const uint32_t *baseCounts, bool *virtualIdx) {
  bool rowSpace = false;
  *virtualIdx = false;
  FastOperands probe;
  if (!is_wide(p.a.kind) && indexVector != nullptr && numForeignTables == 0 && fast_operands(p, probe, true)) {
    *virtualIdx = virtual_iota(device, indexVector, n, true);
    rowSpace = baseCounts == nullptr && row_space_eligible(device, stream, indexVector, n, p.a.length);
  }
  if (rowSpace) flush_deferred_impl(device, nullptr, nullptr, indexVector);
  else flush_deferred(device);
  rowSpace = rowSpace && row_space_eligible(device, stream, indexVector, n, p.a.length);
  if (!rowSpace) mem_note_write(device, pred, static_cast<size_t>(n));
  materialize_index_vector(device, indexVector);
  return rowSpace;
}

int run_filter_two_phase(int device, hipStream_t stream, FastOperands f, uint32_t *indexVector, uint8_t *pred, int n,
                         RecordID **recordIDVectors, int numForeignTables, bool virtualIdx) {
  f.pad = static_cast<int>(reinterpret_cast<uintptr_t>(pred) & 3);
  const int tiles = pred_tiles(n, f.pad);
  const int passes = 1 + numForeignTables;
  constexpr int kPredGridCap = 256 * 16;
  static_assert(kPredGridCap <= kPinnedWords, "the partial counts are read back in one copy");
  const int predGrid = capped_grid(tiles, kPredGridCap);
  auto wsBuf = std::make_shared<StreamBuffer>(CompactSpace::bytes(tiles, passes, predGrid), stream);
  const CompactSpace cs = clear_compact_space(*wsBuf, tiles, passes, predGrid, stream);
  if (virtualIdx) f.idx = nullptr;
  const bool lazy = numForeignTables == 0 && journal_is_valid(device, indexVector);
  uint32_t *partials = cs.extra();
  ARES_LAUNCH("filter_pred_kernel", filter_pred_kernel, predGrid, kBlock, stream, f, pred, cs.tileCounts(), n, tiles,
              lazy ? partials : nullptr);
  if (lazy) {
    uint32_t parts[kPredGridCap];
    read_back_u32(partials, parts, predGrid, stream);
    uint32_t count = 0;
    for (int b = 0; b < predGrid; b++) count += parts[b];
    PendingCompact c;
    c.stream = stream;
    c.idx = indexVector;
    c.pred = pred;
    c.n = n;
    c.pad = f.pad;
    c.virtualIdx = virtualIdx;
    c.ws = wsBuf;
    c.space = cs;
    DeferLock lock(device);
// ... 36 lines not shown
    ws.status = reinterpret_cast<uint64_t *>(base + 16);
    if (pass == 0) {
      totalDev = ws.total;
      if (is_wide(p.a.kind)) {
        ARES_LAUNCH("filter_kernel<2>", filter_kernel<2>, grid, kBlock, stream, p, pred, indexVector,
                           static_cast<uint64_t *>(nullptr), ws, n, numTiles);
      } else {
        ARES_LAUNCH("filter_kernel<0>", filter_kernel<0>, grid, kBlock, stream, p, pred, indexVector,
                    static_cast<uint64_t *>(nullptr), ws, n, numTiles);
      }
    } else {
      ARES_LAUNCH("filter_kernel<1>", filter_kernel<1>, grid, kBlock, stream, p, pred, indexVector,
                  reinterpret_cast<uint64_t *>(recordIDVectors[pass - 1]), ws, n, numTiles);
    }
  }
  uint32_t result[2] = {0, 0};
  read_back_u32(totalDev, result, 2, stream);
  if (result[1]) throw AlgorithmError("ERROR: filter: inter-tile scan timed out");
  return static_cast<int>(result[0]);
}
}

static int run_filter(const InputVector *ins, int arity, uint32_t *indexVector, uint8_t *pred, int n,
                      RecordID **recordIDVectors, int numForeignTables, uint32_t *baseCounts, uint32_t startCount,
                      int functor, hipStream_t stream, int device) {
  if (numForeignTables < 0 || numForeignTables > 8) throw std::invalid_argument("only support up to 8 foreign tables");
  if (n <= 0) {
    flush_deferred(device);
    return 0;
  }
  EvalParams p;
  CallTemps temps;
  const bool isArray = ins[0].Type == ArrayVectorPartyInput;
  ArrayD arr;
  std::shared_ptr<StreamBuffer> decoded;
  if (isArray) {
    bind_array(ins, arity, functor, Bool, arr);
    memset(&p, 0, sizeof(p));
    p.a.kind = K_UUID;
  } else {
    build_params(ins, arity, stream, indexVector, baseCounts, startCount, functor, p, temps);
    decoded = decode_run_length_operand(device, stream, p.a, indexVector, baseCounts, startCount);
  }
  p.needRow = 1;
  bool virtualIdx = false;
  const bool rowSpace = prepare_filter(device, stream, p, indexVector, pred, n, numForeignTables, baseCounts, &virtualIdx);
  FastOperands f;
  const bool fast = !is_wide(p.a.kind) && indexVector != nullptr && fast_operands(p, f, true);
  if (fast && numForeignTables == 0 && baseCounts == nullptr)
    journal_filter(device, indexVector, &f, p.a.length, n, decoded);
  else
    journal_filter(device, indexVector, nullptr, 0, 0);
  if (rowSpace && fast && journal_is_valid(device, indexVector)) {
    const int counted = run_filter_rows(device, stream, f, indexVector, pred, n, p.a.length, virtualIdx, decoded);
    if (counted >= 0) return counted;
  }
  if (rowSpace) {
    mem_note_write(device, pred, static_cast<size_t>(n));
    DeferLock lock(device);
    run_compaction(indexVector);
  }
  if (fast) return run_filter_two_phase(device, stream, f, indexVector, pred, n, recordIDVectors, numForeignTables, virtualIdx);
  return run_filter_generic(device, stream, p, isArray ? &arr : nullptr, indexVector, pred, n, recordIDVectors, numForeignTables);
}

namespace {
bool touches(const std::vector<ByteRange> &v, const ByteRange &r) {
  for (const ByteRange &x : v)
    if (x.overlaps(r)) return true;
  return false;
}
bool journal_touched(const uint32_t *indexVector, const FilterJournal &j, const ByteRange &r, bool *indexOnly) {
  const bool idx = range_of(indexVector, 4ull * (j.n0 > 0 ? j.n0 : 1)).overlaps(r);
  bool cols = false;
  for (size_t k = 0; k < j.filters.size(); k++) cols = cols || column_overlaps(j.filters[k], j.colRows[k], r);
  if (indexOnly) *indexOnly = idx && !cols;
  return idx || cols;
}

struct DeviceGuard {
  int previous = -1;
  explicit DeviceGuard(int device) {
    if (hipGetDevice(&previous) != hipSuccess) previous = -1;
    if (previous != device) (void)hipSetDevice(device);
  }
  ~DeviceGuard() {
    if (previous >= 0) (void)hipSetDevice(previous);
  }
};

void hook_on_wait(int device, void *streamPtr) {
  hipStream_t stream = reinterpret_cast<hipStream_t>(streamPtr);
  try {
    DeviceGuard guard(device);
    DeferLock lock(device);
    for (auto it = t_state->iotas.begin(); it != t_state->iotas.end();) {
      it = (it->second.stream == stream && !it->second.consumed) ? write_iota(it) : std::next(it);
    }
    for (auto &kv : t_state->pending) {
      if (kv.first != stream || kv.second.jobs.count == 0 || kv.second.overWait) continue;
      PendingQueue &q = kv.second;
      bool keep = g_fuseEnabled;
      if (keep && q.idx) {
        auto j = t_state->journals.find(q.idx);
        keep = j != t_state->journals.end() && j->second.valid && j->second.stream == stream && j->second.start == 0;
        if (keep)
          for (size_t k = 0; k < j->second.filters.size(); k++)
            column_ranges(j->second.filters[k], j->second.colRows[k], [&](const ByteRange &c) { q.reads.push_back(c); });
      }
      if (keep)
        q.overWait = true;
      else
        launch_queue(kv.first, q);
    }
  } catch (std::exception &e) {
    fprintf(stderr, "Exception happened when handling a stream wait: %s\n", e.what());
  }
}

uintptr_t hook_on_free(int device, void *ptr, size_t bytes) {
  const ByteRange r = range_of(ptr, bytes);
  grouped_note_write(device, ptr, bytes);
  uintptr_t hold = 0;
  ReleaseSet released;
  try {
    DeviceGuard guard(device);
    DeferLock lock(device);
    for (auto it = t_state->sorts.begin(); it != t_state->sorts.end();) {
      if (sort_touches(it->second, r)) {
        drop_sort(it->first);
        it = t_state->sorts.begin();
      } else {
        ++it;
      }
    }
    for (auto it = t_state->iotas.begin(); it != t_state->iotas.end();) {
      const ByteRange v = range_of(it->first, 4ull * it->second.n);
      it = v.overlaps(r) ? t_state->iotas.erase(it) : std::next(it);
    }
    retire_fills(r, true);
    forget_run_expansions(r);
    for (auto it = t_state->journals.begin(); it != t_state->journals.end();) {
      const bool dead = journal_touched(it->first, it->second, r, nullptr);
      bool kept = false;
      if (dead)
        for (auto &kv : t_state->pending) kept = kept || (kv.second.jobs.count && kv.second.overWait && kv.second.idx == it->first);
      it = (dead && !kept) ? t_state->journals.erase(it) : std::next(it);
    }
    for (auto &kv : t_state->pending) {
      if (kv.second.jobs.count == 0) continue;
      if (touches(kv.second.writes, r)) {
        released.add(kv.first);
        launch_queue(kv.first, kv.second);
      } else if (touches(kv.second.reads, r)) {
        if (kv.second.overWait) {
          hold = hold_tag(kv.first);
        } else {
          released.add(kv.first);
          launch_queue(kv.first, kv.second);
        }
      }
    }
    for (auto it = t_state->compactions.begin(); it != t_state->compactions.end();) {
      if (!compaction_touches(it->second, r)) {
        ++it;
        continue;
      }
      const uint32_t *key = it->first;
      const hipStream_t owner = it->second.stream;
      bool waited = false, queued = false, skipped = false;
      for (auto &kv : t_state->pending)
        if (kv.second.jobs.count && kv.second.idx == key) (kv.second.overWait ? waited : queued) = true;
      for (auto &kv : t_state->limbo) skipped = skipped || kv.second.idx == key;
      if (waited || skipped) {
        hold = hold_tag(owner);
// ... 15 lines not shown
    for (auto it = t_state->limbo.begin(); it != t_state->limbo.end();) {
      if (touches(it->second.writes, r)) {
        it = drop_limbo(it, &released);
      } else {
        if (touches(it->second.reads, r)) hold = hold_tag(it->first);
        ++it;
      }
    }
  } catch (std::exception &e) {
    fprintf(stderr, "Exception happened when handling a device free: %s\n", e.what());
  }
  released.run(device);
  return hold;
}

void hook_on_access(int device, const void *ptr, size_t bytes) {
  const ByteRange r = range_of(ptr, bytes);
  ReleaseSet released;
  try {
    DeviceGuard guard(device);
    grouped_materialize_for_read(device, ptr, bytes);
    DeferLock lock(device);
    for (auto it = t_state->iotas.begin(); it != t_state->iotas.end();) {
      const ByteRange v = range_of(it->first, 4ull * it->second.n);
      if (v.overlaps(r)) {
        t_syncAfterUnlock.push_back(it->second.stream);
        it = write_iota(it);
      } else {
        ++it;
      }
    }
    for (auto &kv : t_state->pending) {
      if (kv.second.jobs.count == 0) continue;
      if (touches(kv.second.writes, r) || touches(kv.second.reads, r)) {
        released.add(kv.first);
        launch_queue(kv.first, kv.second);
      }
    }
    forget_run_expansions(r);
    materialize_fills(&r, &t_syncAfterUnlock);
    materialize_limbo(&r, &released);
    for (auto it = t_state->compactions.begin(); it != t_state->compactions.end();) {
      if (compaction_touches(it->second, r)) {
        const hipStream_t cs = it->second.stream;
        run_compaction(it->first);
        t_syncAfterUnlock.push_back(cs);
        it = t_state->compactions.begin();
      } else {
        ++it;
      }
    }
    for (auto it = t_state->journals.begin(); it != t_state->journals.end();)
      it = journal_touched(it->first, it->second, r, nullptr) ? t_state->journals.erase(it) : std::next(it);
  } catch (std::exception &e) {
    fprintf(stderr, "Exception happened when handling a device copy: %s\n", e.what());
  }
  released.run(device);
}
}

namespace {
void hook_on_write(int device, const void *ptr, size_t bytes) { grouped_note_write(device, ptr, bytes); }

void hook_trim(int device) {
  try {
    DeviceGuard guard(device);
    stream_cache_trim(device);
    grouped_trim(device);
  } catch (std::exception &) {
  }
}

void hook_on_stream_destroy(int device, void *streamPtr) {
  hipStream_t stream = reinterpret_cast<hipStream_t>(streamPtr);
  try {
    DeviceGuard guard(device);
    {
      DeferLock lock(device);
      for (auto it = t_state->sorts.begin(); it != t_state->sorts.end();) {
        if (it->second.stream == stream) {
          drop_sort(it->first);
          it = t_state->sorts.begin();
        } else {
          ++it;
        }
      }
      t_state->pending.erase(stream);
      t_state->expansions.erase(stream);
      auto lim = t_state->limbo.find(stream);
      if (lim != t_state->limbo.end()) drop_limbo(lim, nullptr);
      for (auto it = t_state->journals.begin(); it != t_state->journals.end();)
        it = it->second.stream == stream ? t_state->journals.erase(it) : std::next(it);
      for (auto it = t_state->compactions.begin(); it != t_state->compactions.end();)
        it = it->second.stream == stream ? t_state->compactions.erase(it) : std::next(it);
      for (auto it = t_state->iotas.begin(); it != t_state->iotas.end();)
        it = it->second.stream == stream ? t_state->iotas.erase(it) : std::next(it);
      t_state->filterHistory.erase(stream);
      for (auto &kv : t_state->fills)
        if (kv.second.stream == stream) kv.second.streamGone = true;
      for (size_t i = 0; i < t_state->errorChecks.size();) {
        if (t_state->errorChecks[i].stream == stream) t_state->errorSeen = retire_error_check(i) || t_state->errorSeen;
        else i++;
      }
    }
    profiler_stream_gone(stream);
    if (g_releaseHeld) g_releaseHeld(device, hold_tag(stream));
    stream_cache_purge(device, stream);
  } catch (std::exception &e) {
    fprintf(stderr, "Exception happened when handling a stream destruction: %s\n", e.what());
  }
}
}

void launch_pending_writers(int device, const void *ptr, size_t bytes) {
  if (!ptr || bytes == 0 || !defer_available()) return;
  grouped_materialize_for_read(device, ptr, bytes);
  const ByteRange r = range_of(ptr, bytes);
  ReleaseSet released;
  {
    DeferLock lock(device);
    for (auto &kv : t_state->pending) {
      if (kv.second.jobs.count == 0 || !touches(kv.second.writes, r)) continue;
      if (kv.second.overWait) released.add(kv.first);
      launch_queue(kv.first, kv.second);
    }
    materialize_limbo(&r, &released);
  }
  released.run(device);
}

namespace {
bool match_jobs(const PendingQueue &pq, const DimensionVector &in, const DimLayoutD &L, int prev, int (&dimJob)[kFusedDims], int *measureJob) {
  const int nd = L.numDims;
  const size_t cap = static_cast<size_t>(in.VectorCapacity);
  if (nd < 1 || nd > kFusedDims || in.NumDimsPerDimWidth[0] || in.NumDimsPerDimWidth[1]) return false;
  if (pq.jobs.count != nd && pq.jobs.count != nd + 1) return false;
  for (int c = 0; c < kFusedDims; c++) dimJob[c] = -1;
  *measureJob = -1;
  for (int k = 0; k < pq.jobs.count; k++) {
    const SinkD &s = pq.jobs.s[k];
    if (s.type == SINK_MEASURE) {
// ... 39 lines not shown
  if (measureJob >= 0) fused_plan_measure(plan, nd, pq.jobs.f[measureJob], pq.jobs.s[measureJob], valueBytes);
  else fused_plan_const_measure(plan, nd, constBits, constDtype, valueBytes);
  return !journal || (columns_cover(journal->colRows.data(), journal->filters.size(), n0) &&
                      fused_plan_filters(plan, journal->filters.data(), journal->filters.size()));
}
void take_queue(PendingQueue &pq, PendingQueue &q) {
  q = pq;
  pq.jobs.count = 0;
  pq.reads.clear();
  pq.writes.clear();
  pq.keep.clear();
  pq.overWait = false;
  if (q.idx) {
    auto jk = t_state->journals.find(q.idx);
    if (jk != t_state->journals.end()) q.keep.insert(q.keep.end(), jk->second.keep.begin(), jk->second.keep.end());
    t_state->journals.erase(q.idx);
  }
}
template <typename Supported>
bool supported_agg_spec(int aggFunc, int valueBytes, Supported &&supported, AggSpec *a) {
  try {
    *a = make_agg_spec(aggFunc, valueBytes);
    return supported(*a);
  } catch (std::exception &) {
    return false;
  }
}
template <typename Attempt>
int guarded_attempt(const char *what, Attempt &&attempt) {
  try {
    return attempt();
  } catch (std::exception &e) {
    const std::string line = std::string(what) + " threw, the call falls back: " + e.what();
    slow_trace(line.c_str(), 0.0);
    if (hr_trace_enabled()) fprintf(stderr, "%s\n", line.c_str());
    return -1;
  }
}
}

bool fuse_pending_into_hash_reduce(int device, hipStream_t stream, const DimensionVector &in, const uint8_t *inValues,
                                   const DimensionVector &out, uint8_t *outValues, int valueBytes, int length, int aggFunc,
                                   int *groups) {
  if (!fuse_available()) return false;
  const bool forcedGlobal = global_table_forced();
  PendingQueue q;
  FusedPlanD plan;
  memset(&plan, 0, sizeof(plan));
  int nd = 0, prev = 0, n0 = 0;
  AggSpec a;
  {
    DeferLock lock(device);
    auto it = t_state->pending.find(stream);
    if (it == t_state->pending.end() || it->second.jobs.count == 0) return false;
    PendingQueue &pq = it->second;
    bool ok = !forcedGlobal;
    nd = in.NumDimsPerDimWidth[2] + in.NumDimsPerDimWidth[3] + in.NumDimsPerDimWidth[4];
    for (int k = 0; k < NUM_DIM_WIDTH; k++)
      ok = ok && (k >= 2 || in.NumDimsPerDimWidth[k] == 0) && out.NumDimsPerDimWidth[k] == in.NumDimsPerDimWidth[k];
    ok = ok && nd >= 1 && nd <= kFusedDims;
    DimLayoutD L;
    memset(&L, 0, sizeof(L));
    if (ok) L = make_dim_layout(in.NumDimsPerDimWidth);
    prev = length - pq.n;
    int dimJob[kFusedDims], measureJob = -1;
    ok = ok && prev >= 0 && pq.n > 0 && match_jobs(pq, in, L, prev, dimJob, &measureJob) && measureJob >= 0 &&
         measure_job_matches(pq.jobs.s[measureJob], inValues + static_cast<size_t>(valueBytes) * prev, valueBytes, aggFunc);
    ok = ok && supported_agg_spec(aggFunc, valueBytes, hash_reduce_lds_supported, &a);
    const FilterJournal *journal = nullptr;
    ok = ok && queue_survivors(pq, &journal, &n0) && columns_cover(pq.colRows, pq.jobs.count, n0) &&
         plan_from_queue(plan, pq, L, dimJob, measureJob, valueBytes, 0, 0, journal, n0);
    ok = ok && (plan.numCols <= nd + 2 || fused_plan_narrow(plan, nd));
    if (!ok) {
      launch_queue(stream, pq, true);
      g_releaseHeld(device, hold_tag(stream));
      return false;
    }
    take_queue(pq, q);
  }
  DimensionVector prevKeys = in;
  const int result = fused_hash_reduce_run(device, plan, n0, prevKeys, inValues, prev, out, outValues, a, stream);
  DeferLock lock(device);
  if (result < 0) {
    launch_queue(stream, q, true);
    lock.unlock();
    g_releaseHeld(device, hold_tag(stream));
    return false;
  }
  t_state->limbo[stream] = q;
  *groups = result;
  return true;
}

namespace {
bool same_vector(const DimensionVector &a, const DimensionVector &b) {
  return a.DimValues == b.DimValues && a.HashValues == b.HashValues && a.IndexVector == b.IndexVector && a.VectorCapacity == b.VectorCapacity &&
         memcmp(a.NumDimsPerDimWidth, b.NumDimsPerDimWidth, sizeof(a.NumDimsPerDimWidth)) == 0;
}
}

static void mark_sort_output(const PendingSort &ps, void *at, size_t bytes, int unit) {
  uint8_t *p = static_cast<uint8_t *>(at);
  retire_fills(range_of(p, bytes), false);
  t_state->fills[p] = PendingFill{ps.stream, bytes, 0, unit, false, ps.keys.IndexVector};
}
static void define_sort(const PendingSort &ps, PendingIota &io) {
  mark_sort_output(ps, ps.keys.HashValues, 8ull * static_cast<size_t>(ps.length), 8);
  t_state->sorts[ps.keys.IndexVector] = ps;
  io.consumed = true;
  io.sorted = true;
}

static void enter_reduced_sort(hipStream_t stream, PendingSort ps, const DimensionVector &in, uint8_t *inValues,
                               const DimensionVector &out, uint8_t *outValues, int valueBytes, int length, int aggFunc, int result) {
  ps.reduced = true;
  ps.outKeys = out;
  ps.inValues = inValues;
  ps.outValues = outValues;
  ps.valueBytes = valueBytes;
  ps.aggFunc = aggFunc;
  ps.groups = result;
  define_sort(ps, t_state->iotas[in.IndexVector] = PendingIota{stream, 0, length});
  if (result > 0) mark_sort_output(ps, out.IndexVector, 4ull * static_cast<size_t>(result), 4);
}

bool define_lazy_sort(int device, hipStream_t stream, const DimensionVector &keys, int length) {
  if (!fuse_available() || !fused_sort_reduce_enabled() || length <= 0 || !keys.DimValues || !keys.HashValues || !keys.IndexVector ||
      keys.VectorCapacity < length)
    return false;
  DimLayoutD L;
  try {
    L = make_dim_layout(keys.NumDimsPerDimWidth);
  } catch (std::exception &) {
    return false;
  }
  DeferLock lock(device);
  PendingIota *io = lazy_iota(keys.IndexVector, length);
  if (!io || io->consumed) return false;
  auto it = t_state->pending.find(stream);
  if (it == t_state->pending.end() || it->second.jobs.count == 0) return false;
  const PendingQueue &pq = it->second;
  const int prev = length - pq.n;
  int dimJob[kFusedDims], measureJob = -1, n0 = 0;
  const FilterJournal *journal = nullptr;
// ... 208 lines not shown
  ps.fillAt = fillAt;
  return reduced_sort_done(device, stream, ps, in, inValues, out, outValues, valueBytes, length, aggFunc, result, &q, groups);
}

int compact_by_predicate(const uint8_t *pred, uint32_t *indexVector, RecordID **recordIDVectors, int numForeignTables,
                         int n, hipStream_t stream) {
  if (n <= 0) return 0;
  {
    const int device = current_device();
    mem_note_write(device, indexVector, 4ull * static_cast<size_t>(n));
    for (int t = 0; t < numForeignTables; t++) mem_note_write(device, recordIDVectors[t], 8ull * static_cast<size_t>(n));
  }
  const int pad = static_cast<int>(reinterpret_cast<uintptr_t>(pred) & 3);
  const int tiles = pred_tiles(n, pad);
  const int passes = 1 + numForeignTables;
  StreamBuffer wsBuf(CompactSpace::bytes(tiles, passes, 0), stream);
  const CompactSpace cs = clear_compact_space(wsBuf, tiles, passes, 0, stream);
  ARES_LAUNCH("pred_count_kernel", pred_count_kernel, capped_grid(tiles, 256 * 16), kBlock, stream, pred, cs.tileCounts(), pad, n, tiles);
  launch_compaction(cs, pred, indexVector, false, recordIDVectors, pad, n, stream);
  return read_compaction_total(cs, stream);
}

}

using namespace ares;

extern "C" {

size_t AresStreamEvents(int device, void *stream) {
  size_t n = profiler_stream_events(reinterpret_cast<hipStream_t>(stream));
  if (device < 0 || device >= kMaxDevices) return n;
  DeferLock lock(device);
  for (const ErrorCheck &c : t_state->errorChecks) n += c.stream == reinterpret_cast<hipStream_t>(stream);
  return n;
}

void AresTempStats(size_t *handedOutBytes, size_t *cachedBytes) { temp_stats(handedOutBytes, cachedBytes); }

void AresFlushDeferred(int device) {
  int current = 0;
  if (hipGetDevice(&current) != hipSuccess) {
    (void)hipGetLastError();
    return;
  }
  try {
    if (current != device) hip_check(hipSetDevice(device), "hipSetDevice");
    flush_deferred(device);
    if (current != device) (void)hipSetDevice(current);
  } catch (std::exception &e) {
    fprintf(stderr, "Exception happened when flushing deferred transforms: %s\n", e.what());
  }
}

CGoCallResHandle InitIndexVector(uint32_t *indexVector, uint32_t start, int indexVectorLength, void *cudaStream,
                                 int device) {
  ARES_ABI_BEGIN_NOFLUSH(device)
  hipStream_t stream = reinterpret_cast<hipStream_t>(cudaStream);
  begin_batch(device, stream, indexVector, start, indexVectorLength);
  if (!defer_iota(device, stream, indexVector, start, indexVectorLength)) {
    flush_deferred(device);
    DeferLock lock(device);
    launch_init_index(indexVector, start, indexVectorLength, stream);
  }
  ARES_ABI_END("InitIndexVector")
}

CGoCallResHandle UnaryTransform(InputVector input, OutputVector output, uint32_t *indexVector,
                                int indexVectorLength, uint32_t *baseCounts, uint32_t startCount,
                                enum UnaryFunctorType functorType, void *cudaStream, int device) {
  ARES_ABI_BEGIN_NOFLUSH(device)
  resHandle.res = int_result(run_transform(&input, 1, output, indexVector, indexVectorLength, baseCounts,
                                           startCount, functorType, reinterpret_cast<hipStream_t>(cudaStream), device));
  ARES_ABI_END("UnaryTransform")
}

CGoCallResHandle BinaryTransform(InputVector lhs, InputVector rhs, OutputVector output, uint32_t *indexVector,
                                 int indexVectorLength, uint32_t *baseCounts, uint32_t startCount,
                                 enum BinaryFunctorType functorType, void *cudaStream, int device) {
  ARES_ABI_BEGIN_NOFLUSH(device)
  InputVector ins[2] = {lhs, rhs};
  resHandle.res = int_result(run_transform(ins, 2, output, indexVector, indexVectorLength, baseCounts, startCount,
                                           functorType, reinterpret_cast<hipStream_t>(cudaStream), device));
  ARES_ABI_END("BinaryTransform")
}

CGoCallResHandle UnaryFilter(InputVector input, uint32_t *indexVector, uint8_t *predicateVector,
                             int indexVectorLength, RecordID **recordIDVectors, int numForeignTables,
                             uint32_t *baseCounts, uint32_t startCount, enum UnaryFunctorType functorType,
                             void *cudaStream, int device) {
  ARES_ABI_BEGIN_NOFLUSH(device)
  resHandle.res = int_result(run_filter(&input, 1, indexVector, predicateVector, indexVectorLength, recordIDVectors,
                                        numForeignTables, baseCounts, startCount, functorType,
                                        reinterpret_cast<hipStream_t>(cudaStream), device));
  ARES_ABI_END("UnaryFilter")
}

CGoCallResHandle BinaryFilter(InputVector lhs, InputVector rhs, uint32_t *indexVector, uint8_t *predicateVector,
                              int indexVectorLength, RecordID **recordIDVectors, int numForeignTables,
                              uint32_t *baseCounts, uint32_t startCount, enum BinaryFunctorType functorType,
                              void *cudaStream, int device) {
  ARES_ABI_BEGIN_NOFLUSH(device)
  InputVector ins[2] = {lhs, rhs};
  resHandle.res = int_result(run_filter(ins, 2, indexVector, predicateVector, indexVectorLength, recordIDVectors,
                                        numForeignTables, baseCounts, startCount, functorType,
                                        reinterpret_cast<hipStream_t>(cudaStream), device));
  ARES_ABI_END("BinaryFilter")
}

}
```

aresdb_amd/csrc/host/abi_library.hpp:

```cpp
#pragma once

#include <dlfcn.h>

#include <cstdlib>
#include <cstring>
#include <stdexcept>
#include <string>

#include "ares_driver.h"
#include "ares_extensions.h"
#include "ares_memory.h"

namespace ares_host {

struct AbiError : std::runtime_error {
  explicit AbiError(const std::string &m) : std::runtime_error(m) {}
};

inline intptr_t check(CGoCallResHandle h) {
  if (h.pStrErr) {
    std::string msg(h.pStrErr);
    free(const_cast<char *>(h.pStrErr));
    throw AbiError(msg);
  }
  return reinterpret_cast<intptr_t>(h.res);
}

inline bool declined(CGoCallResHandle h) {
  if (!h.pStrErr || strncmp(h.pStrErr, "not fusable", 11) != 0) return false;
  free(const_cast<char *>(h.pStrErr));
  return true;
}

inline void set_err(char *err, int errLen, const char *msg) {
  if (err && errLen > 0) {
    strncpy(err, msg, static_cast<size_t>(errLen) - 1);
    err[errLen - 1] = 0;
  }
}

struct AbiLibrary {
  void *algoHandle = nullptr, *memHandle = nullptr;
  decltype(&::InitIndexVector) InitIndexVector;
  decltype(&::HashLookup) HashLookup;
  decltype(&::UnaryTransform) UnaryTransform;
  decltype(&::UnaryFilter) UnaryFilter;
  decltype(&::BinaryTransform) BinaryTransform;
  decltype(&::BinaryFilter) BinaryFilter;
  decltype(&::Sort) Sort;
  decltype(&::Reduce) Reduce;
  decltype(&::HashReduce) HashReduce;
  decltype(&::AresFusedFilterHashReduce) FusedFilterHashReduce = nullptr;
  decltype(&::AresFusedFilterSelect) FusedFilterSelect = nullptr;
  decltype(&::AresFusedFilterJoinSelect) FusedFilterJoinSelect = nullptr;
  decltype(&::AresJoinColumnsRun) JoinColumnsRun = nullptr;
  decltype(&::AresJoinColumnBytes) JoinColumnBytes = nullptr;
  decltype(&::AresGeoShapeColumnRun) GeoShapeColumnRun = nullptr;
  decltype(&::AresGeoShapeColumnBytes) GeoShapeColumnBytes = nullptr;
  decltype(&::AresLocalTimeColumnRun) LocalTimeColumnRun = nullptr;
  decltype(&::Expand) Expand;
  decltype(&::DeviceAllocate) DeviceAllocate;
  decltype(&::DeviceFree) DeviceFree;
  decltype(&::WaitForCudaStream) WaitForCudaStream;
  decltype(&::HyperLogLog) HyperLogLog;
  decltype(&::GeoBatchIntersects) GeoBatchIntersects;
  decltype(&::WriteGeoShapeDim) WriteGeoShapeDim;
  decltype(&::AsyncCopyDeviceToDevice) AsyncCopyDeviceToDevice;
  decltype(&::AsyncCopyDeviceToHost) AsyncCopyDeviceToHost;
  decltype(&::AsyncCopyHostToDevice) AsyncCopyHostToDevice;
  decltype(&::HostAlloc) HostAlloc;
  decltype(&::HostFree) HostFree;
  void (*NoteWrite)(int, const void *, size_t) = nullptr;
  void (*NoteActivity)() = nullptr;
  void noteWrite(int device, const void *p, size_t bytes) const {
    if (NoteWrite) NoteWrite(device, p, bytes);
    if (NoteActivity) NoteActivity();
  }

  template <typename F>
  void bind(void *handle, const char *name, F &fn, bool optional = false) {
    fn = reinterpret_cast<F>(dlsym(handle, name));
    if (!fn && !optional) throw AbiError(std::string("missing symbol ") + name);
  }

  AbiLibrary(const char *algoPath, const char *memPath) {
    memHandle = dlopen(memPath, RTLD_NOW | RTLD_LOCAL);
    if (!memHandle) throw AbiError(std::string("dlopen ") + memPath + ": " + dlerror());
    algoHandle = dlopen(algoPath, RTLD_NOW | RTLD_LOCAL);
    if (!algoHandle) throw AbiError(std::string("dlopen ") + algoPath + ": " + dlerror());
    bind(algoHandle, "InitIndexVector", InitIndexVector);
    bind(algoHandle, "HashLookup", HashLookup);
    bind(algoHandle, "UnaryTransform", UnaryTransform);
    bind(algoHandle, "UnaryFilter", UnaryFilter);
    bind(algoHandle, "BinaryTransform", BinaryTransform);
    bind(algoHandle, "BinaryFilter", BinaryFilter);
    bind(algoHandle, "Sort", Sort);
    bind(algoHandle, "Reduce", Reduce);
    bind(algoHandle, "HashReduce", HashReduce);
    bind(algoHandle, "HyperLogLog", HyperLogLog);
    bind(algoHandle, "GeoBatchIntersects", GeoBatchIntersects);
    bind(algoHandle, "WriteGeoShapeDim", WriteGeoShapeDim);
    bind(algoHandle, "Expand", Expand);
    bind(algoHandle, "AresFusedFilterHashReduce", FusedFilterHashReduce, true);
    bind(algoHandle, "AresFusedFilterSelect", FusedFilterSelect, true);
    bind(algoHandle, "AresFusedFilterJoinSelect", FusedFilterJoinSelect, true);
    bind(algoHandle, "AresJoinColumnsRun", JoinColumnsRun, true);
    bind(algoHandle, "AresJoinColumnBytes", JoinColumnBytes, true);
    bind(algoHandle, "AresGeoShapeColumnRun", GeoShapeColumnRun, true);
    bind(algoHandle, "AresGeoShapeColumnBytes", GeoShapeColumnBytes, true);
    bind(algoHandle, "AresLocalTimeColumnRun", LocalTimeColumnRun, true);
    bind(memHandle, "DeviceAllocate", DeviceAllocate);
    bind(memHandle, "DeviceFree", DeviceFree);
    bind(memHandle, "WaitForCudaStream", WaitForCudaStream);
    bind(memHandle, "AsyncCopyDeviceToDevice", AsyncCopyDeviceToDevice);
    bind(memHandle, "AsyncCopyDeviceToHost", AsyncCopyDeviceToHost);
    bind(memHandle, "AsyncCopyHostToDevice", AsyncCopyHostToDevice);
    bind(memHandle, "HostAlloc", HostAlloc);
    bind(memHandle, "HostFree", HostFree);
    bind(memHandle, "AresMemNoteWrite", NoteWrite, true);
    bind(memHandle, "AresMemNoteActivity", NoteActivity, true);
  }
  ~AbiLibrary() {
    if (algoHandle) dlclose(algoHandle);
    if (memHandle) dlclose(memHandle);
  }
};

template <typename T>
struct Pod {
  alignas(T) unsigned char bytes[sizeof(T)];
  Pod() { memset(bytes, 0, sizeof(bytes)); }
  T &operator*() { return *reinterpret_cast<T *>(bytes); }
  T *operator->() { return reinterpret_cast<T *>(bytes); }
  const T &get() const { return *reinterpret_cast<const T *>(bytes); }
};
using IV = Pod<InputVector>;
using OV = Pod<OutputVector>;

}
```

aresdb_amd/csrc/host/batch_executor.cpp:

```cpp
#include <algorithm>
#include <cstring>

#include "query.hpp"

using namespace ares_host;

void AresQuery::prepareForFiltering(const VectorPartySlice *cols, int ncols, int n, uint32_t *bc, uint32_t start) {
  columns = cols;
  numColumns = ncols;
  size = n;
  batchRows = n;
  baseCounts = bc;
  startRow = start;
  indexVec = alloc<uint32_t>(static_cast<size_t>(n) * 4);
  predVec = alloc<uint8_t>(static_cast<size_t>(n));
}

void AresQuery::prepareForDimAndMeasureEval() {
  if (resultSize + size <= resultCapacity) return;
  const int oldCapacity = resultCapacity;
  resultCapacity = resultSize + size;
  resultCapacity += resultCapacity / 8;
  const int64_t cap = resultCapacity;
  {
// ... 376 lines not shown
      const size_t bytes = n * (s < nd ? layout.widths[s] : 1);
      hostSections[s].insert(hostSections[s].end(), from, from + bytes);
      from += bytes;
    }
    check(lib->HostFree(host));
  }
  rowsWritten += resultSize;
  if (recordsNeeded() == 0) done = true;
  size = 0;
}

bool AresQuery::fusedExpr(int nodeIdx, int outType, AresFusedExpr *e, int *join) {
  const Plan &p = *batchPlan;
  const AresPlanNode &n = p.nodes.at(nodeIdx);
  memset(e, 0, sizeof(*e));
  e->outType = static_cast<DataType>(outType);
  auto leafColumn = [&](const AresPlanNode &c, InputVector *iv) {
    if (c.kind != ARES_NODE_COLUMN || c.table < 0 || c.table > static_cast<int>(p.foreign.size())) return false;
    if (c.table != 0 && !join) return false;
    if (join) *join = c.table - 1;
    memcpy(iv, &columnInput(c, false).get(), sizeof(InputVector));
    return true;
  };
  if (n.kind == ARES_NODE_COLUMN) {
    e->arity = 1;
    e->functor = Noop;
    return leafColumn(n, &e->lhs);
  }
  if (n.kind != ARES_NODE_BINARY) return false;
  const AresPlanNode &l = p.nodes.at(n.lhs), &r = p.nodes.at(n.rhs);
  if (r.kind != ARES_NODE_CONST_INT && r.kind != ARES_NODE_CONST_FLOAT) return false;
  if (!leafColumn(l, &e->lhs)) return false;
  memcpy(&e->rhs, &constantInput(r).get(), sizeof(InputVector));
  e->arity = 2;
  e->functor = n.op;
  return true;
}
bool AresQuery::fusedFilters(const std::vector<int> &roots, AresFusedExpr *out, int *count, int *joins) {
  *count = static_cast<int>(roots.size());
  for (size_t i = 0; i < roots.size(); i++)
    if (!fusedExpr(roots[i], Bool, &out[i], joins ? &joins[i] : nullptr) || (joins && joins[i] < 0)) return false;
  return true;
}
bool AresQuery::fusedDims(AresFusedExpr *out, int *count, int *joins) {
  const Plan &p = *batchPlan;
  *count = static_cast<int>(p.dimNodes.size());
  for (size_t i = 0; i < p.dimNodes.size(); i++) {
    const int at = layout.dimVectorIndex[i];
    if (!fusedExpr(p.dimNodes[i], p.dimTypes[i], &out[at], joins ? &joins[at] : nullptr)) return false;
  }
  return true;
}

bool AresQuery::runBatchFused(const VectorPartySlice *cols, int ncols, int n) {
  const Plan &p = *batchPlan;
  if (!p.useFusedExtension || !p.useHashReduction || fusedDeclined || !lib->FusedFilterHashReduce) return false;
  if (p.hasGeo || p.isHLL()) return false;
  if (!p.foreign.empty() || !p.foreignFilters.empty() || baseCounts) return false;
  if (p.dimNodes.empty() || p.dimNodes.size() > 4 || p.filters.size() > 4) return false;
  columns = cols;
  numColumns = ncols;
  Pod<AresFusedQuery> q;
  if (!fusedFilters(p.filters, q->filters, &q->numFilters)) return false;
  for (int t : p.dimTypes)
    if (data_type_bytes(t) != 4) return false;
  if (!fusedDims(q->dims, &q->numDims)) return false;
  if (!fusedExpr(p.measureNode, p.measureType, &q->measure)) return false;
  q->aggFunc = static_cast<AggregateFunction>(p.aggFunc);
  size = n;
  prepareForDimAndMeasureEval();
  calls++;
  CGoCallResHandle h = lib->FusedFilterHashReduce(&q.get(), n, dimensionVector(0), measureVec[0], resultSize,
                                                  dimensionVector(1), measureVec[1], stream, device);
  if (declined(h)) {
    fusedDeclined = true;
    size = 0;
    return false;
  }
  resultSize = static_cast<int>(check(h));
  wait();
  releaseInputColumns();
  swapResultBuffers();
  fusedBatches++;
  return true;
}

bool AresQuery::runBatchFusedSelect(const VectorPartySlice *cols, int ncols, int n) {
  const bool joins = !plan.foreign.empty() || !plan.foreignFilters.empty();
  if (!plan.useFusedExtension || fusedDeclined || !(joins ? lib->FusedFilterJoinSelect != nullptr : lib->FusedFilterSelect != nullptr)) return false;
  if (baseCounts || plan.hasGeo) return false;
  if (plan.foreign.size() > 2 || plan.foreignFilters.size() > 4) return false;
  if (plan.dimNodes.empty() || plan.dimNodes.size() > 8 || plan.filters.size() > 4) return false;
  columns = cols;
  numColumns = ncols;
  Pod<AresFusedJoinSelect> js;
  Pod<AresFusedSelect> s;
  if (joins) {
    if (!fusedFilters(plan.filters, js->filters, &js->numFilters)) return false;
    js->numJoins = static_cast<int>(plan.foreign.size());
    for (size_t k = 0; k < plan.foreign.size(); k++) {
      memcpy(&js->joins[k].key, &columnInput(main_column(plan.foreign[k].t.joinColumn)).get(), sizeof(InputVector));
      memcpy(&js->joins[k].index, &plan.foreign[k].t.index, sizeof(CuckooHashIndex));
    }
    if (!fusedFilters(plan.foreignFilters, js->foreignFilters, &js->numForeignFilters, js->foreignFilterJoin)) return false;
    if (!fusedDims(js->dims, &js->numDims, js->dimJoin)) return false;
  } else {
    if (!fusedFilters(plan.filters, s->filters, &s->numFilters) || !fusedDims(s->dims, &s->numDims)) return false;
  }
  size = n;
  batchRows = n;
  prepareForDimEval();
  calls++;
  CGoCallResHandle h = joins ? lib->FusedFilterJoinSelect(&js.get(), n, recordsNeeded(), dimensionVector(0), stream, device)
                             : lib->FusedFilterSelect(&s.get(), n, recordsNeeded(), dimensionVector(0), stream, device);
  if (declined(h)) {
    fusedDeclined = true;
    size = 0;
    return false;
  }
  resultSize = static_cast<int>(check(h));
  wait();
  releaseInputColumns();
  postExecNonAggr();
  fusedBatches++;
  return true;
}

void AresQuery::runBatchNonAggr(const VectorPartySlice *cols, int ncols, int n, uint32_t *bc, uint32_t start) {
  if (done) {
    ownedColumns.clear();
    return;
  }
  baseCounts = bc;
  if (!runBatchFusedSelect(cols, ncols, n)) {
    prepareForFiltering(cols, ncols, n, bc, start);
    preExec();
    filter();
    join();
    projectNonAggr();
    postExecNonAggr();
  }
  swapStreams();
}

void AresQuery::runBatch(const VectorPartySlice *cols, int ncols, int n, uint32_t *bc, uint32_t start) {
  if (plan.isNonAggregation) {
    runBatchNonAggr(cols, ncols, n, bc, start);
    return;
  }
  baseCounts = bc;
  struct Restore {
    AresQuery &q;
    ~Restore() { q.batchPlan = &q.plan; }
  } restore{*this};
  if (resolve(cols, ncols, n)) {
    batchPlan = &rowSpace->plan;
    cols = extendedColumns.data();
    ncols = static_cast<int>(extendedColumns.size());
  }
  if (runBatchFused(cols, ncols, n)) {
    swapStreams();
    return;
  }
  prepareForFiltering(cols, ncols, n, bc, start);
  preExec();
  filter();
  join();
  project();
  reduce();
  postExec();
  swapStreams();
}

extern "C" {

void *AresDriverOpen(const char *libalgorithmPath, const char *libmemPath, char *err, int errLen) {
  try {
    return new AbiLibrary(libalgorithmPath, libmemPath);
  } catch (std::exception &e) {
    set_err(err, errLen, e.what());
    return nullptr;
  }
}

void AresDriverClose(void *driver) { delete static_cast<AbiLibrary *>(driver); }

AresQuery *AresQueryCreate(void *driver, const AresQueryPlan *plan, int device, void *stream, char *err, int errLen) {
  try {
    return new AresQuery(static_cast<AbiLibrary *>(driver), *plan, device, stream);
  } catch (std::exception &e) {
    set_err(err, errLen, e.what());
    return nullptr;
  }
}

int AresQueryRunBatch(AresQuery *q, const VectorPartySlice *columns, int numColumns, int size, uint32_t *baseCounts,
                      uint32_t startRow, char *err, int errLen) {
  try {
    q->runBatch(columns, numColumns, size, baseCounts, startRow);
    return 0;
  } catch (std::exception &e) {
    set_err(err, errLen, e.what());
    try {
      q->cleanupBeforeAggregation();
    } catch (...) {
    }
    return -1;
  }
}

int AresQueryRunResidentBatches(AresQuery *q, const VectorPartySlice *columns, int numColumns, const int *sizes, int numBatches,
                                char *err, int errLen) {
  for (int b = 0; b < numBatches; b++) {
    q->ownedColumns.clear();
    q->isLastBatch = false;
    const int rc = AresQueryRunBatch(q, columns + static_cast<size_t>(b) * numColumns, numColumns, sizes[b], nullptr, 0, err, errLen);
    if (rc != 0) return rc;
// ... 62 lines not shown
```

aresdb_amd/csrc/host/query.hpp:

```cpp
#pragma once

#include <memory>
#include <utility>
#include <vector>

#include "plan.hpp"

namespace ares_host {

struct RowSpace {
  enum Kind { JOIN_COLUMNS, GEO_COLUMN } kind;
  Plan plan;
  std::vector<std::pair<int, int>> leaves;
  int numAdded = 0;
  struct JoinedTable {
    std::vector<int> columns;
    int first = 0;
  };
  std::vector<JoinedTable> tables;
  struct LocalTime {
    int timeColumn;
    int table;
    int zoneColumn;
    int outType;
// ... 69 lines not shown
  void d2h(void *dst, void *src, size_t bytes) { ares_host::check(lib->AsyncCopyDeviceToHost(dst, src, bytes, stream, device)); }
  void copyDimsD2D(uint8_t *to, uint8_t *from, int64_t length, int64_t offset, int64_t toCapacity, int64_t fromCapacity,
                   int64_t fromOffset = 0) {
    ares_host::copy_dimension_vector(layout, to, from, length, offset, toCapacity, fromCapacity,
                                     [this](void *d, void *s, size_t n) { d2d(d, s, n); }, fromOffset);
  }
  void copyDimsD2H(uint8_t *to, uint8_t *from, int64_t length, int64_t toCapacity, int64_t fromCapacity) {
    ares_host::copy_dimension_vector(layout, to, from, length, 0, toCapacity, fromCapacity,
                                     [this](void *d, void *s, size_t n) { d2h(d, s, n); });
  }

  void prepareForFiltering(const VectorPartySlice *cols, int ncols, int n, uint32_t *bc, uint32_t start);
  void prepareForDimAndMeasureEval();
  uint8_t *allocateStackFrame(int dataType, uint32_t *nullsOffset);
  void shrinkStackFrame();
  void releaseInputColumns();
  void cleanupBeforeAggregation();
  void swapResultBuffers();
  void releaseAll();
  DimensionVector dimensionVector(int which) const;

  struct Action {
    enum Kind { NONE, FILTER, MEASURE, DIMENSION } kind = NONE;
    int dimType = 0;
    int64_t valueOff = 0, nullOff = 0;
    int prevResultSize = 0;
  };
  IV columnInput(const AresPlanNode &n, bool withRids = true, bool withTimezone = false);
  void runAction(const Action &a, int functor, IV *in, int arity);
  IV processExpression(int nodeIdx, const Action &action, bool underConvertTz = false);

  void preExec();
  void filter();
  void join();
  void evalDimensions(int prev);
  void project();
  void reduce();
  void postExec() { swapResultBuffers(); }
  void swapStreams() {
    if (otherStream) std::swap(stream, otherStream);
  }
  void runBatch(const VectorPartySlice *cols, int ncols, int n, uint32_t *bc, uint32_t start);

  int recordsNeeded() const { return plan.limit < 0 ? -1 : std::max(plan.limit - rowsWritten, 0); }
  void prepareForDimEval();
  void expandDimensions();
  void projectNonAggr();
  void postExecNonAggr();
  void runBatchNonAggr(const VectorPartySlice *cols, int ncols, int n, uint32_t *bc, uint32_t start);

  bool fusedExpr(int nodeIdx, int outType, AresFusedExpr *e, int *join = nullptr);
  bool fusedFilters(const std::vector<int> &roots, AresFusedExpr *out, int *count, int *joins = nullptr);
  bool fusedDims(AresFusedExpr *out, int *count, int *joins = nullptr);
  bool runBatchFused(const VectorPartySlice *cols, int ncols, int n);
  bool runBatchFusedSelect(const VectorPartySlice *cols, int ncols, int n);

  void setRowSpace(ares_host::RowSpace::Kind kind, bool on);
  int pruningHints(AresFusedExpr *out);
  bool runJoinColumns(ares_host::RowSpace &rs, int n);
  bool runLocalTimeColumns(ares_host::RowSpace &rs, int n);
  bool runGeoColumn(int n);
  bool resolve(const VectorPartySlice *cols, int ncols, int n);
};
```

include/ares_extensions.h:

```cpp
#ifndef ARES_EXTENSIONS_H_
#define ARES_EXTENSIONS_H_

#include <stddef.h>
#include <stdint.h>

#include "ares_algorithm.h"

#ifdef __cplusplus
extern "C" {
#endif

void AresProfilerEnable(int on);
size_t AresProfilerReport(char *buf, size_t len);

void AresReloadEnv(void);

size_t AresRtcWait(long *counters);

void AresFlushDeferred(int device);
void AresMemSetFlushHook(void (*hook)(int device));

typedef struct {
  void (*flush)(int device);
  void (*on_wait)(int device, void *stream);
  uintptr_t (*on_free)(int device, void *ptr, size_t bytes);
  void (*on_access)(int device, const void *ptr, size_t bytes);
} AresDeferralHooks;
void AresMemSetDeferralHooks(const AresDeferralHooks *hooks);
void AresMemReleaseHeld(int device, uintptr_t tag);

typedef struct {
  size_t size;
  void (*on_write)(int device, const void *ptr, size_t bytes);
  void (*on_stream_destroy)(int device, void *stream);
  void (*trim)(int device);
} AresMemAuxHooks;
void AresMemSetAuxHooks(const AresMemAuxHooks *hooks);
void AresMemTrimCache(int device);
void AresMemNoteWrite(int device, const void *ptr, size_t bytes);
void AresMemEnableWriteTracking(void);

void AresMemNoteActivity(void);
void AresMemEnableActivityTracking(void);

void AresMemStats(int device, size_t *liveBytes, size_t *liveBlocks, size_t *heldBlocks, size_t *parkedBytes);
void AresMemDriverCalls(int device, size_t *mallocs, size_t *frees, size_t *trims);
size_t AresMemStreamEvents(int device, void *stream);
size_t AresStreamEvents(int device, void *stream);
void AresTempStats(size_t *handedOutBytes, size_t *cachedBytes);

void AresHllPreaggStats(unsigned long long *counters);

typedef struct {
  InputVector lhs, rhs;
  int arity;
  int functor;
  enum DataType outType;
} AresFusedExpr;

typedef struct {
  int numFilters;
  AresFusedExpr filters[4];
  int numDims;
  AresFusedExpr dims[4];
  AresFusedExpr measure;
  enum AggregateFunction aggFunc;
} AresFusedQuery;

CGoCallResHandle AresFusedFilterHashReduce(const AresFusedQuery *query, int batchRows, DimensionVector prevKeys,
                                           uint8_t *prevValues, int prevSize, DimensionVector outKeys,
                                           uint8_t *outValues, void *cudaStream, int device);

typedef struct {
  int numFilters;
  AresFusedExpr filters[4];
  int numDims;
  AresFusedExpr dims[8];
} AresFusedSelect;

CGoCallResHandle AresFusedFilterSelect(const AresFusedSelect *query, int batchRows, int limit ,
                                       DimensionVector outKeys, void *cudaStream, int device);
void AresSelectStats(unsigned long long *counters);
void AresSelectRunStats(unsigned long long *counters);

typedef struct {
  InputVector key;
  CuckooHashIndex index;
} AresFusedJoin;

typedef struct {
  int numFilters;
  AresFusedExpr filters[4];
  int numJoins;
  AresFusedJoin joins[2];
  int numForeignFilters;
  AresFusedExpr foreignFilters[4];
  int foreignFilterJoin[4];
  int numDims;
  AresFusedExpr dims[8];
  int dimJoin[8];
} AresFusedJoinSelect;

CGoCallResHandle AresFusedFilterJoinSelect(const AresFusedJoinSelect *query, int batchRows, int limit ,
                                           DimensionVector outKeys, void *cudaStream, int device);
void AresSelectJoinStats(unsigned long long *counters);

typedef struct {
  InputVector column;
  uint8_t *out;
} AresJoinedColumn;

typedef struct {
  int numFilters;
  AresFusedExpr filters[4];
  AresFusedJoin join;
  int numColumns;
  AresJoinedColumn columns[4];
} AresJoinColumns;

size_t AresJoinColumnBytes(int rows, enum DataType type);
CGoCallResHandle AresJoinColumnsRun(const AresJoinColumns *q, int batchRows, VectorPartySlice *outSlices, void *cudaStream,
                                    int device);
void AresJoinColumnStats(unsigned long long *counters);

// ... 33 lines not shown
```

Measured before the change: 89.19 billion rows/s.

## Launch fused filter/dim scan at filter time via batch hint and reuse at hash-reduce

The host now sends a per-batch hint with the fused query shape before the filter step. When the plan qualifies (lean, compact RTC scan), the library launches the scan kernel early and keeps its regions in a per-stream stash, which the later fused hash-reduce call takes instead of rescanning. The goal is to start the scan sooner and avoid redundant work or serialization between the unfused filter path and the hash-reduce. In exchange it adds bookkeeping for invalidation: write tracking, shape checks, and latching after repeated discards. A discarded stash wastes a whole scan, and a missed invalidation could produce stale results.

Measured after the change: 95.41 billion rows/s, median of 6. 1.07x the previous value.

```diff
diff --git a/aresdb_amd/abi.py b/aresdb_amd/abi.py
--- a/aresdb_amd/abi.py
+++ b/aresdb_amd/abi.py
@@ -131,6 +131,11 @@
 class FusedExpr(C.Structure):
     _fields_ = [("lhs", InputVector), ("rhs", InputVector), ("arity", C.c_int), ("functor", C.c_int),
                 ("outType", C.c_int)]
+
+
+class FusedQuery(C.Structure):
+    _fields_ = [("numFilters", C.c_int), ("filters", FusedExpr * 4), ("numDims", C.c_int), ("dims", FusedExpr * 4),
+                ("measure", FusedExpr), ("aggFunc", C.c_int)]
 
 
 class FusedSelect(C.Structure):
@@ -292,6 +297,24 @@
         return self._mem.GetFlags()
 
     @property
+    def has_scan_at_filter(self):
+        return hasattr(self._algo, "AresHintFusedBatch") and hasattr(self._algo, "AresScanAtFilterStats")
+
+    def hint_fused_batch(self, query, batch_rows, prev_size, measure_bytes, stream=None, device=0):
+        fn = self._algo.AresHintFusedBatch
+        fn.argtypes, fn.restype = [C.POINTER(FusedQuery), C.c_int, C.c_int, C.c_int, _S, _I], None
+        fn(C.byref(query), int(batch_rows), int(prev_size), int(measure_bytes), stream, device)
+
+    SCAN_AT_FILTER_COUNTERS = ("hints", "scans", "honoured", "declined", "discard_plan", "discard_shape", "discard_touched",
+                               "discard_abandoned", "retried", "latched")
+
+    def scan_at_filter_stats(self):
+        c = (C.c_ulonglong * len(self.SCAN_AT_FILTER_COUNTERS))()
+        self._algo.AresScanAtFilterStats.argtypes, self._algo.AresScanAtFilterStats.restype = [C.POINTER(C.c_ulonglong)], None
+        self._algo.AresScanAtFilterStats(c)
+        return {k: int(v) for k, v in zip(self.SCAN_AT_FILTER_COUNTERS, c)}
+
+    @property
     def has_fused_select(self):
         return hasattr(self._algo, "AresFusedFilterSelect")
 
diff --git a/aresdb_amd/csrc/algo/common.hpp b/aresdb_amd/csrc/algo/common.hpp
--- a/aresdb_amd/csrc/algo/common.hpp
+++ b/aresdb_amd/csrc/algo/common.hpp
@@ -67,6 +67,7 @@
 bool global_table_forced();
 bool deferral_hooks_active();
 void grouped_note_write(int device, const void *ptr, size_t bytes);
+void grouped_note_gone(int device, const void *ptr, size_t bytes);
 void grouped_note_write(int device, const DimensionVector &v);
 void grouped_materialize_for_read(int device, const void *ptr, size_t bytes);
 void grouped_trim(int device);
diff --git a/aresdb_amd/csrc/algo/hash_reduce_lds.hip b/aresdb_amd/csrc/algo/hash_reduce_lds.hip
--- a/aresdb_amd/csrc/algo/hash_reduce_lds.hip
+++ b/aresdb_amd/csrc/algo/hash_reduce_lds.hip
@@ -349,6 +349,10 @@
 }
 
 void grouped_note_write(int device, const void *ptr, size_t bytes) {
+  scan_ahead_note_touch(device, ptr, bytes, false);
+  grouped_note_gone(device, ptr, bytes);
+}
+void grouped_note_gone(int device, const void *ptr, size_t bytes) {
   sorted_state_note_write(device, ptr, bytes);
   const uint8_t *lo = static_cast<const uint8_t *>(ptr);
   const uint8_t *hi = lo + (bytes ? bytes : 1);
@@ -552,9 +556,259 @@
   g_firstBatchGroups[shape] = groups;
 }
 
+static hr::Widen widen_of(const FusedPlanD &plan) {
+  hr::Widen widen;
+  widen.mode = plan.measureWidth == 8 ? 1 : 0;
+  widen.rk = plan.measure.f.rk;
+  widen.dtype = plan.measureDtype;
+  return widen;
+}
+static int fused_part_bits(int64_t length, bool narrow) { return std::max(part_bits_for(length), narrow ? 2 : 0); }
+struct ScanChoice {
+  size_t shape = 0;
+  int chunkTiles = 0;
+  bool compact = false, wantLean = false, wantTable = false;
+  RtcKernel lean, table;
+};
+static ScanChoice choose_scan(int device, const FusedPlanD &plan, int nd, int batchRows, int prevSize, int partBits, bool narrow, const AggSpec *a) {
+  ScanChoice c;
+  int expected = prevSize;
+  bool known = prevSize > 0;
+  const bool rtc = batchRows > 0 && rtc_scan_available();
+  if (rtc && prevSize == 0) {
+    const RtcSpec spec = rtc_spec_scan(plan, nd, 0, false);
+    c.shape = std::hash<std::string>()(std::string(reinterpret_cast<const char *>(&spec), sizeof(spec)));
+    std::lock_guard<std::mutex> lock(g_shapeMutex);
+    auto it = g_firstBatchGroups.find(c.shape);
+    if (it != g_firstBatchGroups.end()) {
+      expected = it->second;
+      known = true;
+    }
+  }
+  c.chunkTiles = compact_enabled() ? rtc_compact_chunk_tiles(batchRows, partBits) : 0;
+  c.compact = c.chunkTiles > 0;
+  c.wantLean = rtc && expected >= lean_min_groups() && (known || lean_min_groups() <= 0);
+  c.wantTable = rtc && !c.wantLean && (known || narrow);
+  if (c.wantLean) c.lean = rtc_lookup(device, rtc_spec_scan(plan, nd, partBits, c.compact));
+  else if (c.wantTable && a) c.table = rtc_lookup(device, rtc_spec_table_scan(plan, nd, partBits, *a, widen_of(plan)));
+  return c;
+}
+static void prepare_direct_scan(Regions &r, const FusedPlanD &plan, int partBits, int64_t rowsA, int batchRows, int prevSize, int streams,
+                                int chunkTiles, hipStream_t stream) {
+  SlowScope slow("make_regions");
+  make_regions(r, partBits, rowsA, batchRows, streams, 4, stream, chunkTiles > 0 ? static_cast<int>(kCompactLineRecords) : 8);
+  r.ws.widen = widen_of(plan);
+  r.ws.chunkRows = static_cast<uint32_t>(chunkTiles) * 4096u;
+  r.ws.rowBase = static_cast<uint32_t>(prevSize);
+}
+
+struct ScanStash {
+  Regions r;
+  FusedPlanD plan;
+  int nd, batchRows, prevSize, partBits, chunkTiles, slack;
+  RtcKernel lean;
+};
+namespace {
+struct AheadEntry {
+  int device;
+  hipStream_t stream;
+  bool live = false;
+  int inits = 0;
+  ScanHint hint;
+  std::shared_ptr<ScanStash> stash;
+  int discardsInARow = 0;
+  bool latched = false;
+  FusedPlanD latchedShape;
+};
+std::mutex g_aheadMutex;
+std::vector<AheadEntry> g_ahead;
+std::atomic<unsigned long long> g_aheadCounters[kScanAheadCounters];
+
+AheadEntry *ahead_find(int device, hipStream_t stream) {
+  for (AheadEntry &e : g_ahead)
+    if (e.device == device && e.stream == stream) return &e;
+  return nullptr;
+}
+FusedPlanD shape_of(FusedPlanD plan) {
+  for (int c = 0; c < kFusedCols; c++) {
+    plan.cols[c].vals = nullptr;
+    plan.cols[c].nulls = nullptr;
+    plan.cols[c].bitOff = 0;
+  }
+  return plan;
+}
+void ahead_discarded(AheadEntry &e, int reason) {
+  scan_ahead_count(reason);
+  if (reason == kScanAheadDiscardRetry) return;
+  if (++e.discardsInARow >= 2 && !e.latched) {
+    e.latched = true;
+    e.latchedShape = shape_of(e.hint.plan);
+  }
+}
+bool ranges_hit(const ScanHint &h, const uint8_t *lo, const uint8_t *hi) {
+  for (int k = 0; k < h.numRanges; k++)
+    if (h.ranges[k].lo < hi && lo < h.ranges[k].hi) return true;
+  return false;
+}
+}
+
+void scan_ahead_count(int which) { g_aheadCounters[which].fetch_add(1, std::memory_order_relaxed); }
+void scan_ahead_stats(unsigned long long *out) {
+  for (int k = 0; k < kScanAheadCounters; k++) out[k] = g_aheadCounters[k].load(std::memory_order_relaxed);
+}
+bool scan_at_filter_enabled() {
+  static EnvSwitch<bool> on("ARES_SCAN_AT_FILTER", [](const char *e) { return !(e && e[0] == '0'); });
+  return on.get() && grouped_enabled();
+}
+
+void scan_hint_set(int device, hipStream_t stream, const ScanHint &hint) {
+  std::shared_ptr<ScanStash> old;
+  {
+    std::lock_guard<std::mutex> lock(g_aheadMutex);
+    AheadEntry *e = ahead_find(device, stream);
+    if (!e) {
+      g_ahead.emplace_back();
+      e = &g_ahead.back();
+      e->device = device;
+      e->stream = stream;
+    }
+    if (e->stash) ahead_discarded(*e, kScanAheadDiscardAbandoned);
+    old.swap(e->stash);
+    if (e->latched && fused_plan_equal(shape_of(hint.plan), e->latchedShape, hint.nd)) {
+      scan_ahead_count(kScanAheadLatched);
+      e->live = false;
+      return;
+    }
+    if (e->latched) {
+      e->latched = false;
+      e->discardsInARow = 0;
+    }
+    e->hint = hint;
+    e->live = true;
+    e->inits = 0;
+    scan_ahead_count(kScanAheadHints);
+  }
+}
+
+void scan_hint_init_index(int device, hipStream_t stream) {
+  std::shared_ptr<ScanStash> old;
+  std::lock_guard<std::mutex> lock(g_aheadMutex);
+  AheadEntry *e = ahead_find(device, stream);
+  if (!e) return;
+  if (e->stash) ahead_discarded(*e, kScanAheadDiscardAbandoned);
+  old.swap(e->stash);
+  if (e->live && ++e->inits > 1) e->live = false;
+}
+
+bool scan_hint_live(int device, hipStream_t stream, ScanHint *out) {
+  std::lock_guard<std::mutex> lock(g_aheadMutex);
+  AheadEntry *e = ahead_find(device, stream);
+  if (!e || !e->live || e->inits != 1 || e->stash) return false;
+  *out = e->hint;
+  return true;
+}
+
+void scan_stash_put(int device, hipStream_t stream, std::shared_ptr<ScanStash> stash) {
+  std::lock_guard<std::mutex> lock(g_aheadMutex);
+  AheadEntry *e = ahead_find(device, stream);
+  if (!e || !e->live) return;
+  e->stash.swap(stash);
+  scan_ahead_count(kScanAheadScans);
+}
+
+std::shared_ptr<ScanStash> scan_stash_take(int device, hipStream_t stream) {
+  std::lock_guard<std::mutex> lock(g_aheadMutex);
+  AheadEntry *e = ahead_find(device, stream);
+  if (!e || !e->stash) return nullptr;
+  std::shared_ptr<ScanStash> s;
+  s.swap(e->stash);
+  e->live = false;
+  return s;
+}
+
+void scan_stash_settled(int device, hipStream_t stream, int reason, bool blame) {
+  std::lock_guard<std::mutex> lock(g_aheadMutex);
+  AheadEntry *e = ahead_find(device, stream);
+  if (reason == kScanAheadHonoured) {
+    scan_ahead_count(kScanAheadHonoured);
+    if (e) e->discardsInARow = 0;
+  } else if (e && blame) {
+    ahead_discarded(*e, reason);
+  } else {
+    scan_ahead_count(reason);
+  }
+}
+
+void scan_ahead_note_touch(int device, const void *ptr, size_t bytes, bool freed) {
+  const uint8_t *lo = static_cast<const uint8_t *>(ptr), *hi = lo + (bytes ? bytes : 1);
+  std::vector<std::shared_ptr<ScanStash>> dead;
+  std::lock_guard<std::mutex> lock(g_aheadMutex);
+  for (AheadEntry &e : g_ahead) {
+    if (e.device != device || !(e.live || e.stash) || !ranges_hit(e.hint, lo, hi)) continue;
+    e.live = false;
+    if (e.stash && !freed) {
+      scan_ahead_count(kScanAheadDiscardTouched);
+      dead.push_back(std::move(e.stash));
+      e.stash = nullptr;
+    }
+  }
+}
+
+void scan_ahead_stream_gone(int device, hipStream_t stream) {
+  std::shared_ptr<ScanStash> old;
+  std::lock_guard<std::mutex> lock(g_aheadMutex);
+  for (size_t i = 0; i < g_ahead.size(); i++)
+    if (g_ahead[i].device == device && g_ahead[i].stream == stream) {
+      if (g_ahead[i].stash) scan_ahead_count(kScanAheadDiscardAbandoned);
+      old.swap(g_ahead[i].stash);
+      g_ahead[i] = g_ahead.back();
+      g_ahead.pop_back();
+      return;
+    }
+}
+
+std::shared_ptr<ScanStash> fused_scan_ahead(int device, const ScanHint &hint, hipStream_t stream, uint32_t *hostCount, int *grid) {
+  const FusedPlanD &plan = hint.plan;
+  const bool narrow = fused_plan_narrow(plan, hint.nd);
+  const int64_t length = static_cast<int64_t>(hint.batchRows) + hint.prevSize;
+  if (narrow || hint.batchRows <= 0 || length > INT32_MAX) return nullptr;
+  const int partBits = fused_part_bits(length, narrow);
+  const ScanChoice choice = choose_scan(device, plan, hint.nd, hint.batchRows, hint.prevSize, partBits, narrow, nullptr);
+  if (!choice.wantLean || !choice.lean || !choice.compact) return nullptr;
+  auto stash = std::make_shared<ScanStash>();
+  stash->plan = plan;
+  stash->nd = hint.nd;
+  stash->batchRows = hint.batchRows;
+  stash->prevSize = hint.prevSize;
+  stash->partBits = partBits;
+  stash->chunkTiles = choice.chunkTiles;
+  stash->slack = record_stream_slack();
+  stash->lean = choice.lean;
+  const int streams = rtc_scan_grid(hint.batchRows);
+  static_assert(kMaxStreams <= kPinnedWords, "one survivor count per workgroup fits the pinned slot");
+  prepare_direct_scan(stash->r, plan, partBits, 0, hint.batchRows, hint.prevSize, streams, choice.chunkTiles, stream);
+  rtc_scan_launch(choice.lean, RTC_SCAN_COMPACT, plan, static_cast<uint32_t>(hint.prevSize), hint.batchRows, stash->r.ws, stream, hostCount);
+  *grid = streams;
+  return stash;
+}
+
 int fused_hash_reduce_run(int device, const FusedPlanD &plan, int batchRows, const DimensionVector &prevKeys,
                           const uint8_t *prevValues, int prevSize, const DimensionVector &outKeys, uint8_t *outValues,
-                          const AggSpec &a, hipStream_t stream) {
+                          const AggSpec &a, hipStream_t stream, std::shared_ptr<ScanStash> stash) {
+  struct Settle {
+    std::shared_ptr<ScanStash> &stash;
+    int device;
+    hipStream_t stream;
+    bool taken = false, merged = false;
+    void rescanned() {
+      if (taken) scan_stash_settled(device, stream, kScanAheadDiscardRetry);
+      taken = false;
+    }
+    ~Settle() {
+      if (stash) scan_stash_settled(device, stream, kScanAheadDiscardShape, false);
+      else if (taken) scan_stash_settled(device, stream, merged ? kScanAheadHonoured : kScanAheadDiscardRetry);
+    }
+  } settle{stash, device, stream};
   SlotWidths slots;
   if (!slot_widths(outKeys.NumDimsPerDimWidth, &slots)) return kFusedUnavailable;
   const int nd = slots.nd;
@@ -562,7 +816,7 @@
   const int mw = plan.measureWidth;
   const int64_t length = static_cast<int64_t>(batchRows) + prevSize;
   if (length == 0) return 0;
-  const int partBits = std::max(part_bits_for(length), narrow ? 2 : 0);
+  const int partBits = fused_part_bits(length, narrow);
   const int numParts = 1 << partBits;
   const size_t prevCapacity = static_cast<size_t>(prevKeys.VectorCapacity);
   const size_t outCapacity = static_cast<size_t>(outKeys.VectorCapacity);
@@ -578,33 +832,14 @@
   const std::shared_ptr<uint32_t> outRangesRef = grouped_enabled() ? take_ranges(device) : nullptr;
   uint32_t *outRanges = outRangesRef.get();
   MergeResult res{0, 0, 0, 0};
-  hr::Widen widen;
-  widen.mode = mw == 8 ? 1 : 0;
-  widen.rk = plan.measure.f.rk;
-  widen.dtype = plan.measureDtype;
-  size_t shape = 0;
-  int expected = prevSize;
-  bool known = prevSize > 0;
-  const bool rtc = batchRows > 0 && rtc_scan_available();
-  if (rtc && prevSize == 0) {
-    const RtcSpec spec = rtc_spec_scan(plan, nd, 0, false);
-    shape = std::hash<std::string>()(std::string(reinterpret_cast<const char *>(&spec), sizeof(spec)));
-    std::lock_guard<std::mutex> lock(g_shapeMutex);
-    auto it = g_firstBatchGroups.find(shape);
-    if (it != g_firstBatchGroups.end()) {
-      expected = it->second;
-      known = true;
-    }
-  }
-  const int chunkTiles = compact_enabled() ? rtc_compact_chunk_tiles(batchRows, partBits) : 0;
-  const bool compact = chunkTiles > 0;
+  const hr::Widen widen = widen_of(plan);
+  SlowScope slowWhole("fused_hash_reduce_run");
+  const ScanChoice choice = choose_scan(device, plan, nd, batchRows, prevSize, partBits, narrow, &a);
+  const size_t shape = choice.shape;
+  const int chunkTiles = choice.chunkTiles;
+  const bool compact = choice.compact, wantLean = choice.wantLean, wantTable = choice.wantTable;
   const RtcKind leanKind = compact ? RTC_SCAN_COMPACT : RTC_SCAN_LINES16;
-  RtcKernel lean, table, tableMerge, narrowMerge;
-  SlowScope slowWhole("fused_hash_reduce_run");
-  const bool wantLean = rtc && expected >= lean_min_groups() && (known || lean_min_groups() <= 0);
-  const bool wantTable = rtc && !wantLean && (known || narrow);
-  if (wantLean) lean = rtc_lookup(device, rtc_spec_scan(plan, nd, partBits, compact));
-  else if (wantTable) table = rtc_lookup(device, rtc_spec_table_scan(plan, nd, partBits, a, widen));
+  RtcKernel lean = choice.lean, table = choice.table, tableMerge, narrowMerge;
   int imageMode = 0;
   RtcKernel imageMerge;
   std::shared_ptr<uint8_t> imageOut;
@@ -655,11 +890,39 @@
     launched = true;
     const int streams = batchRows > 0 ? (lean ? rtc_scan_grid(batchRows) : table ? 0 : grid_for(batchRows)) : 0;
     Regions r;
-    {
+    const int64_t rowsA = !lean ? length : (prevSize > 0 && !grouped && imageMode != 2) ? prevSize : 0;
+    bool scanned = false;
+    if (stash) {
+      const std::shared_ptr<ScanStash> st = std::move(stash);
+      stash = nullptr;
+      int why = -1;
+      if (!lean || !compact || st->nd != nd || !fused_plan_equal(st->plan, plan, nd)) why = kScanAheadDiscardPlan;
+      else if (st->batchRows != batchRows || st->prevSize != prevSize || st->partBits != partBits || st->chunkTiles != chunkTiles ||
+               st->slack != record_stream_slack() || st->lean != lean || st->r.ws.streams != streams || rowsA != 0)
+        why = kScanAheadDiscardShape;
+      if (hr_trace_enabled())
+        fprintf(stderr, "fused_hash_reduce_run: scan at filter %s | lean %d compact %d nd %d/%d plan equal %d | rows %d/%d prev %d/%d partBits %d/%d "
+                        "chunkTiles %d/%d slack %d/%d kernel %d streams %d/%d rowsA %lld\n",
+                why < 0 ? "honoured" : why == kScanAheadDiscardPlan ? "discarded (plan)" : "discarded (shape)", lean ? 1 : 0, compact ? 1 : 0, st->nd, nd,
+                fused_plan_equal(st->plan, plan, nd) ? 1 : 0, st->batchRows, batchRows, st->prevSize, prevSize, st->partBits, partBits, st->chunkTiles,
+                chunkTiles, st->slack, record_stream_slack(), st->lean == lean ? 1 : 0, st->r.ws.streams, streams, static_cast<long long>(rowsA));
+      if (why < 0) {
+        r = std::move(st->r);
+        scanned = true;
+        settle.taken = true;
+      }
+      const bool onlyRegionA = why == kScanAheadDiscardShape && st->batchRows == batchRows && st->prevSize == prevSize && st->partBits == partBits &&
+                               st->chunkTiles == chunkTiles && st->slack == record_stream_slack() && st->lean == lean && st->r.ws.streams == streams;
+      if (why >= 0) scan_stash_settled(device, stream, why, !onlyRegionA);
+    } else {
+      settle.rescanned();
+    }
+    if (scanned) {
+    } else if (lean) {
+      prepare_direct_scan(r, plan, partBits, rowsA, batchRows, prevSize, streams, chunkTiles, stream);
+    } else {
       SlowScope slow("make_regions");
-      const int64_t rowsA = !lean ? length : (prevSize > 0 && !grouped && imageMode != 2) ? prevSize : 0;
-      make_regions(r, partBits, rowsA, batchRows, streams, lean ? 4 : 3, stream,
-                   !lean ? 0 : compact ? static_cast<int>(kCompactLineRecords) : 8);
+      make_regions(r, partBits, rowsA, batchRows, streams, 3, stream, 0);
     }
     Workspace &ws = r.ws;
     ws.widen = widen;
@@ -698,7 +961,8 @@
         ARES_LAUNCH("hr_partition4_kernel", (hr_partition4_kernel<ND, 4>), grid_for(prevSize), kThreads, stream,        \
                     prevKeys.DimValues, prevCapacity, prevValues, 0u, a, prevSize, wsPrev, 0);                         \
     }                                                                                                                  \
-    if (batchRows > 0 && lean)                                                                                         \
+    if (scanned) {                                                                                                     \
+    } else if (batchRows > 0 && lean)                                                                                  \
       rtc_scan_launch(lean, leanKind, plan, static_cast<uint32_t>(prevSize), batchRows, ws, stream);                   \
     else if (batchRows > 0 && table)                                                                                   \
       rtc_scan_launch(table, RTC_SCAN_TABLE, plan, static_cast<uint32_t>(prevSize), batchRows, ws, stream);            \
@@ -721,7 +985,8 @@
     switch (nd) {
       ARES_FUSED_CASE(1) ARES_FUSED_CASE(2) ARES_FUSED_CASE(3) ARES_FUSED_CASE(4)
       default:
-        if (batchRows > 0 && lean) rtc_scan_launch(lean, leanKind, plan, static_cast<uint32_t>(prevSize), batchRows, ws, stream);
+        if (scanned) {
+        } else if (batchRows > 0 && lean) rtc_scan_launch(lean, leanKind, plan, static_cast<uint32_t>(prevSize), batchRows, ws, stream);
         else if (batchRows > 0 && table) rtc_scan_launch(table, RTC_SCAN_TABLE, plan, static_cast<uint32_t>(prevSize), batchRows, ws, stream);
         rtc_merge_launch(leanMerge ? leanMerge : tableMerge, plan, prevKeys.DimValues, prevCapacity, prevValues, static_cast<uint32_t>(prevSize),
                          outKeys.DimValues, outCapacity, outValues, ws, stream, imagePtr, result_slot());
@@ -774,6 +1039,7 @@
   if (res.overflow) {
     return -1;
   }
+  settle.merged = true;
   fused_note_first_batch(shape, static_cast<int>(res.groups));
   if (shape && !lean && !table) {
     if (static_cast<int>(res.groups) >= lean_min_groups()) {
diff --git a/aresdb_amd/csrc/algo/hash_reduce_lds.hpp b/aresdb_amd/csrc/algo/hash_reduce_lds.hpp
--- a/aresdb_amd/csrc/algo/hash_reduce_lds.hpp
+++ b/aresdb_amd/csrc/algo/hash_reduce_lds.hpp
@@ -1,6 +1,8 @@
 #pragma once
 
 #include <hip/hip_runtime.h>
+
+#include <memory>
 
 #include "aggregate.hpp"
 #include "ares_algorithm.h"
@@ -48,6 +50,25 @@
   uint8_t dimWidth[kFusedDims];
   int measureAvg;
 };
+inline bool fused_expr_equal(const FusedExpr &a, const FusedExpr &b) {
+  return a.col == b.col && a.outKind == b.outKind && a.f.akind == b.f.akind && a.f.arity == b.f.arity && a.f.functor == b.f.functor &&
+         a.f.I == b.f.I && a.f.rk == b.f.rk && a.f.bkind == b.f.bkind && a.f.bbits == b.f.bbits && a.f.bok == b.f.bok &&
+         a.f.divLike == b.f.divLike && (a.f.step ? a.f.step : 4) == (b.f.step ? b.f.step : 4);
+}
+inline bool fused_plan_equal(const FusedPlanD &a, const FusedPlanD &b, int nd) {
+  if (a.numCols != b.numCols || a.numFilters != b.numFilters || a.measureDtype != b.measureDtype || a.measureWidth != b.measureWidth ||
+      a.identity != b.identity || a.measureAvg != b.measureAvg)
+    return false;
+  for (int c = 0; c < a.numCols; c++)
+    if (a.cols[c].vals != b.cols[c].vals || a.cols[c].nulls != b.cols[c].nulls || a.cols[c].bitOff != b.cols[c].bitOff ||
+        (a.cols[c].step ? a.cols[c].step : 4) != (b.cols[c].step ? b.cols[c].step : 4))
+      return false;
+  for (int k = 0; k < a.numFilters; k++)
+    if (!fused_expr_equal(a.filters[k], b.filters[k])) return false;
+  for (int d = 0; d < nd; d++)
+    if (!fused_expr_equal(a.dims[d], b.dims[d]) || (a.dimWidth[d] ? a.dimWidth[d] : 4) != (b.dimWidth[d] ? b.dimWidth[d] : 4)) return false;
+  return fused_expr_equal(a.measure, b.measure);
+}
 inline int fused_dim_width(const FusedPlanD &p, int d) { return p.dimWidth[d] ? p.dimWidth[d] : 4; }
 inline int fused_col_step(const FusedPlanD &p, int c) { return p.cols[c].step ? static_cast<int>(p.cols[c].step) : 4; }
 inline bool fused_plan_narrow(const FusedPlanD &p, int nd) {
@@ -133,8 +154,44 @@
 constexpr int kFusedUnavailable = -2;
 int record_stream_slack();
 bool grow_record_stream_slack();
+struct ScanStash;
 int fused_hash_reduce_run(int device, const FusedPlanD &plan, int batchRows, const DimensionVector &prevKeys,
                           const uint8_t *prevValues, int prevSize, const DimensionVector &outKeys, uint8_t *outValues,
-                          const AggSpec &a, hipStream_t stream);
+                          const AggSpec &a, hipStream_t stream, std::shared_ptr<ScanStash> stash = nullptr);
+
+struct ScanHint {
+  FusedPlanD plan;
+  int nd, batchRows, prevSize;
+  FastOperands filters[kFusedFilters];
+  struct Range {
+    const uint8_t *lo, *hi;
+  } ranges[2 * kFusedCols];
+  int numRanges;
+};
+enum ScanAheadCounter {
+  kScanAheadHints,
+  kScanAheadScans,
+  kScanAheadHonoured,
+  kScanAheadDeclined,
+  kScanAheadDiscardPlan,
+  kScanAheadDiscardShape,
+  kScanAheadDiscardTouched,
+  kScanAheadDiscardAbandoned,
+  kScanAheadDiscardRetry,
+  kScanAheadLatched,
+  kScanAheadCounters
+};
+void scan_ahead_count(int which);
+void scan_ahead_stats(unsigned long long *out);
+bool scan_at_filter_enabled();
+void scan_hint_set(int device, hipStream_t stream, const ScanHint &hint);
+void scan_hint_init_index(int device, hipStream_t stream);
+bool scan_hint_live(int device, hipStream_t stream, ScanHint *out);
+std::shared_ptr<ScanStash> fused_scan_ahead(int device, const ScanHint &hint, hipStream_t stream, uint32_t *hostCount, int *grid);
+void scan_stash_put(int device, hipStream_t stream, std::shared_ptr<ScanStash> stash);
+std::shared_ptr<ScanStash> scan_stash_take(int device, hipStream_t stream);
+void scan_stash_settled(int device, hipStream_t stream, int reason, bool blame = true);
+void scan_ahead_note_touch(int device, const void *ptr, size_t bytes, bool freed);
+void scan_ahead_stream_gone(int device, hipStream_t stream);
 
 }
diff --git a/aresdb_amd/csrc/algo/hr_rtc.hip b/aresdb_amd/csrc/algo/hr_rtc.hip
--- a/aresdb_amd/csrc/algo/hr_rtc.hip
+++ b/aresdb_amd/csrc/algo/hr_rtc.hip
@@ -71,6 +71,7 @@
   uint32_t *countsB;
   uint32_t *overflow;
   uint64_t *phases;
+  uint32_t *hostCount;
   uint4 *recA;
   uint32_t *cursorsA;
   uint64_t capA;
@@ -511,7 +512,7 @@
 }
 
 void launch_scan(const RtcKernel &kernel, const FusedPlanD &plan, uint32_t rowBase, int length, const hr::Workspace &ws, int grid,
-                 uint32_t chunkTiles, uint32_t pad, hipStream_t stream, const char *name) {
+                 uint32_t chunkTiles, uint32_t pad, hipStream_t stream, const char *name, uint32_t *hostCount = nullptr) {
   RtcArgs args;
   fill_columns(args, plan);
   for (int k = 0; k < plan.numFilters && k < kFusedFilters; k++)
@@ -520,6 +521,7 @@
   args.recB = ws.recB;
   args.countsB = ws.countsB;
   args.overflow = ws.outCount + 1;
+  args.hostCount = hostCount;
   args.recA = ws.recA;
   args.cursorsA = ws.cursorsA;
   args.capA = ws.capA;
@@ -579,11 +581,11 @@
 }
 
 void rtc_scan_launch(const RtcKernel &kernel, RtcKind kind, const FusedPlanD &plan, uint32_t rowBase, int length, const hr::Workspace &ws,
-                     hipStream_t stream) {
+                     hipStream_t stream, uint32_t *hostCount) {
   const int grid = kind == RTC_SCAN_TABLE ? rtc_scan_grid(length) : ws.streams;
   const uint32_t chunkTiles = kind == RTC_SCAN_COMPACT ? ws.chunkRows / 4096u : 0u;
   launch_scan(kernel, plan, rowBase, length, ws, grid, chunkTiles, 0u, stream,
-              kind == RTC_SCAN_TABLE ? "hr_table_scan_rtc" : rtc_entry_name(kind));
+              kind == RTC_SCAN_TABLE ? "hr_table_scan_rtc" : rtc_entry_name(kind), kind == RTC_SCAN_COMPACT ? hostCount : nullptr);
 }
 
 void rtc_vector_scan_launch(const RtcKernel &kernel, RtcKind kind, const uint8_t *dimValues, size_t capacity, const void *measures, int nd,
diff --git a/aresdb_amd/csrc/algo/hr_rtc.hpp b/aresdb_amd/csrc/algo/hr_rtc.hpp
--- a/aresdb_amd/csrc/algo/hr_rtc.hpp
+++ b/aresdb_amd/csrc/algo/hr_rtc.hpp
@@ -19,7 +19,7 @@
 RtcKernel rtc_lookup(int device, const RtcSpec &spec, bool wait = false);
 
 void rtc_scan_launch(const RtcKernel &kernel, RtcKind kind, const FusedPlanD &plan, uint32_t rowBase, int length, const hr::Workspace &ws,
-                     hipStream_t stream);
+                     hipStream_t stream, uint32_t *hostCount = nullptr);
 void rtc_vector_scan_launch(const RtcKernel &kernel, RtcKind kind, const uint8_t *dimValues, size_t capacity, const void *measures, int nd,
                             const int *widths, uint32_t rowBase, int length, const hr::Workspace &ws, hipStream_t stream,
                             int totalPartBits = 0, bool spread = false);
diff --git a/aresdb_amd/csrc/algo/hr_rtc_gen.hip b/aresdb_amd/csrc/algo/hr_rtc_gen.hip
--- a/aresdb_amd/csrc/algo/hr_rtc_gen.hip
+++ b/aresdb_amd/csrc/algo/hr_rtc_gen.hip
@@ -85,7 +85,7 @@
 
 std::string args_text() {
   std::ostringstream o;
-  o << "struct Args { const u32 *vals[" << kFusedCols << "]; const u8 *nulls[" << kFusedCols << "]; u32 *recB; u32 *countsB; u32 *overflow; u64 *phases;\n"
+  o << "struct Args { const u32 *vals[" << kFusedCols << "]; const u8 *nulls[" << kFusedCols << "]; u32 *recB; u32 *countsB; u32 *overflow; u64 *phases; u32 *hostCount;\n"
        "              uint4 *recA; u32 *cursorsA; u64 capA; u32 bitOff[" << kFusedCols << "]; u32 rowBase; int length; u32 capB; u32 chunkTiles;\n"
        "              u32 k[" << kNumConsts << "]; u32 pad; };\n";
   return o.str();
@@ -305,7 +305,7 @@
        "  __shared__ u32 sTotalLines;\n"
        "  const u32 tid = threadIdx.x, lane = tid & 63u, wave = tid >> 6;\n"
        "  for (u32 p = tid; p < NP; p += 1024u) { sCount[0][p] = 0u; sCount[1][p] = 0u; }\n"
-       "  u32 myLeftN = 0u, myCursor = 0u;\n"
+       "  u32 myLeftN = 0u, myCursor = 0u, mySeen = 0u;\n"
        "  __syncthreads();\n"
        "  u64 *myB = reinterpret_cast<u64 *>(a.recB) + (u64)blockIdx.x * NP * a.capB * 16u;\n"
        "  const u32 numTiles = ((u32)a.length + T - 1u) / T;\n"
@@ -335,6 +335,7 @@
        "    u32 myCount = 0u, myLeft = 0u;\n"
        "    if (tid < NP) { myCount = cnt[tid]; myLeft = myLeftN; }\n"
        "    const u32 myHave = myCount + myLeft, myLines = myHave / LR;\n"
+       "    mySeen += myCount;\n"
        "    const u32 packed = (myCount << 16) | myLines;\n"
        "    const u32 incl = wave_incl_scan(packed);\n"
        "    if (lane == 63u) sWave[wave] = incl;\n"
@@ -421,6 +422,12 @@
        "    if (left && fits) STORE_LINE(&myB[((u64)p * a.capB + cur) * 16u + q], r8 ? rec : hdr);\n"
        "    if (left && !fits) *a.overflow = 1u;\n"
        "    if (q == 0u) a.countsB[(u64)blockIdx.x * NP + p] = cur * LR + ((left && fits) ? left : 0u);\n"
+       "  }\n"
+       "  if (a.hostCount) {\n"
+       "    const u32 seen = wave_incl_scan(mySeen);\n"
+       "    if (lane == 63u) sWave[wave] = seen;\n"
+       "    __syncthreads();\n"
+       "    if (tid == 0u) { u32 t = 0u; for (u32 w = 0u; w < 16u; w++) t += sWave[w]; a.hostCount[blockIdx.x] = t; }\n"
        "  }\n"
        "  PH(6)\n"
        "  PH_OUT\n"
diff --git a/aresdb_amd/csrc/algo/transform.hip b/aresdb_amd/csrc/algo/transform.hip
--- a/aresdb_amd/csrc/algo/transform.hip
+++ b/aresdb_amd/csrc/algo/transform.hip
@@ -161,6 +161,7 @@
   std::vector<LazyFilter> todo;
   int n0 = 0, applied = 0, lastCount = 0;
   std::shared_ptr<StreamBuffer> bits;
+  bool noBits = false;
   PredictedFilter predicted;
   uint64_t generation = 0;
 };
@@ -1206,8 +1207,24 @@
     return false;
   auto c = t_state->compactions.find(indexVector);
   if (j->second.filters.empty()) return n == j->second.n0 && c == t_state->compactions.end();
-  return c != t_state->compactions.end() && !c->second.todo.empty() && c->second.stream == stream &&
+  return c != t_state->compactions.end() && !c->second.todo.empty() && c->second.stream == stream && !c->second.noBits &&
          c->second.applied + c->second.todo.size() == j->second.filters.size() && c->second.lastCount == n;
+}
+
+std::map<const uint32_t *, PendingCompact>::iterator open_row_space(hipStream_t stream, uint32_t *indexVector, bool virtualIdx, int n) {
+  PendingCompact fresh{};
+  fresh.stream = stream;
+  fresh.idx = indexVector;
+  fresh.virtualIdx = virtualIdx;
+  fresh.n0 = n;
+  fresh.applied = 0;
+  fresh.lastCount = n;
+  return t_state->compactions.emplace(indexVector, fresh).first;
+}
+FilterShape note_filter_shape(FilterHistory &h, const PendingCompact &c, const FastOperands &f) {
+  const FilterShape shape{f.akind, f.functor, f.I, f.bkind, f.bbits, f.bok, !c.todo.empty() && same_column(c.todo.back().f, f)};
+  h.current.push_back(shape);
+  return shape;
 }
 
 int run_filter_rows(int device, hipStream_t stream, FastOperands f, uint32_t *indexVector, uint8_t *pred, int n, uint32_t colRows,
@@ -1229,25 +1246,15 @@
       auto jr = t_state->journals.find(indexVector);
       const size_t journalled = (jr != t_state->journals.end() && jr->second.valid) ? jr->second.filters.size() : 0;
       const bool first = ins == t_state->compactions.end() && journalled == 1 && jr->second.n0 == n;
-      const bool next = ins != t_state->compactions.end() && !ins->second.todo.empty() && ins->second.stream == stream &&
+      const bool next = ins != t_state->compactions.end() && !ins->second.todo.empty() && ins->second.stream == stream && !ins->second.noBits &&
                         ins->second.applied + ins->second.todo.size() + 1 == journalled && ins->second.lastCount == n;
       if (!first && !next) return -1;
     }
-    if (ins == t_state->compactions.end()) {
-      PendingCompact fresh{};
-      fresh.stream = stream;
-      fresh.idx = indexVector;
-      fresh.virtualIdx = virtualIdx;
-      fresh.n0 = n;
-      fresh.applied = 0;
-      fresh.lastCount = n;
-      ins = t_state->compactions.emplace(indexVector, fresh).first;
-    }
+    if (ins == t_state->compactions.end()) ins = open_row_space(stream, indexVector, virtualIdx, n);
     PendingCompact &c = ins->second;
     FilterHistory &h = t_state->filterHistory[stream];
-    FilterShape shape{f.akind, f.functor, f.I, f.bkind, f.bbits, f.bok, !c.todo.empty() && same_column(c.todo.back().f, f)};
-    const size_t k = h.current.size();
-    h.current.push_back(shape);
+    const FilterShape shape = note_filter_shape(h, c, f);
+    const size_t k = h.current.size() - 1;
     if (c.predicted.valid && same_filter(c.predicted.g, f)) {
       const int count = c.predicted.count;
       c.todo.push_back(LazyFilter{f, colRows, pred, n, keep});
@@ -1310,6 +1317,58 @@
         it->second.predicted.bits = bits2;
       }
     }
+    auto j = t_state->journals.find(indexVector);
+    if (j != t_state->journals.end() && j->second.valid) j->second.lastCount = static_cast<int>(count);
+  }
+  return static_cast<int>(count);
+}
+
+int run_filter_scan(int device, hipStream_t stream, FastOperands f, uint32_t *indexVector, uint8_t *pred, int n, uint32_t colRows,
+                    bool virtualIdx, const std::shared_ptr<StreamBuffer> &keep) {
+  ScanHint hint;
+  if (keep || !scan_at_filter_enabled() || !scan_hint_live(device, stream, &hint)) return -1;
+  f.idx = nullptr;
+  f.pad = 0;
+  int grid = 0;
+  uint64_t generation = 0;
+  {
+    DeferLock lock(device);
+    auto jr = t_state->journals.find(indexVector);
+    if (jr == t_state->journals.end() || !jr->second.valid || jr->second.stream != stream || jr->second.start != 0 ||
+        jr->second.n0 != hint.batchRows || jr->second.filters.size() != static_cast<size_t>(hint.plan.numFilters))
+      return -1;
+    const FilterJournal &j = jr->second;
+    for (size_t k = 0; k < j.filters.size(); k++)
+      if (!same_filter(j.filters[k], hint.filters[k]) || j.colRows[k] < static_cast<uint32_t>(j.n0)) return -1;
+    auto ins = t_state->compactions.find(indexVector);
+    const size_t journalled = j.filters.size();
+    const bool first = ins == t_state->compactions.end() && journalled == 1 && j.n0 == n;
+    const bool next = ins != t_state->compactions.end() && !ins->second.todo.empty() && ins->second.stream == stream && !ins->second.noBits &&
+                      ins->second.applied + ins->second.todo.size() + 1 == journalled && ins->second.lastCount == n;
+    if (!first && !next) return -1;
+    if (next && ins->second.predicted.valid && same_filter(ins->second.predicted.g, f)) return -1;
+    std::shared_ptr<ScanStash> stash = fused_scan_ahead(device, hint, stream, reinterpret_cast<uint32_t *>(pinned_words()), &grid);
+    if (!stash) return -1;
+    if (ins == t_state->compactions.end()) ins = open_row_space(stream, indexVector, virtualIdx, n);
+    PendingCompact &c = ins->second;
+    note_filter_shape(t_state->filterHistory[stream], c, f);
+    c.predicted = PredictedFilter{};
+    c.todo.push_back(LazyFilter{f, colRows, pred, n, keep});
+    c.bits = nullptr;
+    c.noBits = true;
+    c.lastCount = -1;
+    generation = ++t_state->filterGeneration;
+    c.generation = generation;
+    scan_stash_put(device, stream, std::move(stash));
+  }
+  hip_check(hipStreamSynchronize(stream), "hipStreamSynchronize");
+  const volatile uint32_t *parts = reinterpret_cast<const volatile uint32_t *>(pinned_words());
+  uint32_t count = 0;
+  for (int b = 0; b < grid; b++) count += parts[b];
+  {
+    DeferLock lock(device);
+    auto it = t_state->compactions.find(indexVector);
+    if (it != t_state->compactions.end() && it->second.generation == generation) it->second.lastCount = static_cast<int>(count);
     auto j = t_state->journals.find(indexVector);
     if (j != t_state->journals.end() && j->second.valid) j->second.lastCount = static_cast<int>(count);
   }
@@ -1452,6 +1511,8 @@
   else
     journal_filter(device, indexVector, nullptr, 0, 0);
   if (rowSpace && fast && journal_is_valid(device, indexVector)) {
+    const int scanned = run_filter_scan(device, stream, f, indexVector, pred, n, p.a.length, virtualIdx, decoded);
+    if (scanned >= 0) return scanned;
     const int counted = run_filter_rows(device, stream, f, indexVector, pred, n, p.a.length, virtualIdx, decoded);
     if (counted >= 0) return counted;
   }
@@ -1520,7 +1581,8 @@
 
 uintptr_t hook_on_free(int device, void *ptr, size_t bytes) {
   const ByteRange r = range_of(ptr, bytes);
-  grouped_note_write(device, ptr, bytes);
+  grouped_note_gone(device, ptr, bytes);
+  scan_ahead_note_touch(device, ptr, bytes, true);
   uintptr_t hold = 0;
   ReleaseSet released;
   try {
@@ -1642,6 +1704,7 @@
     }
     for (auto it = t_state->journals.begin(); it != t_state->journals.end();)
       it = journal_touched(it->first, it->second, r, nullptr) ? t_state->journals.erase(it) : std::next(it);
+    scan_ahead_note_touch(device, ptr, bytes, false);
   } catch (std::exception &e) {
     fprintf(stderr, "Exception happened when handling a device copy: %s\n", e.what());
   }
@@ -1677,6 +1740,7 @@
       }
       t_state->pending.erase(stream);
       t_state->expansions.erase(stream);
+      scan_ahead_stream_gone(device, stream);
       auto lim = t_state->limbo.find(stream);
       if (lim != t_state->limbo.end()) drop_limbo(lim, nullptr);
       for (auto it = t_state->journals.begin(); it != t_state->journals.end();)
@@ -1822,7 +1886,10 @@
   {
     DeferLock lock(device);
     auto it = t_state->pending.find(stream);
-    if (it == t_state->pending.end() || it->second.jobs.count == 0) return false;
+    if (it == t_state->pending.end() || it->second.jobs.count == 0) {
+      if (scan_stash_take(device, stream)) scan_stash_settled(device, stream, kScanAheadDiscardAbandoned);
+      return false;
+    }
     PendingQueue &pq = it->second;
     bool ok = !forcedGlobal;
     nd = in.NumDimsPerDimWidth[2] + in.NumDimsPerDimWidth[3] + in.NumDimsPerDimWidth[4];
@@ -1844,12 +1911,13 @@
     if (!ok) {
       launch_queue(stream, pq, true);
       g_releaseHeld(device, hold_tag(stream));
+      if (scan_stash_take(device, stream)) scan_stash_settled(device, stream, kScanAheadDiscardPlan);
       return false;
     }
     take_queue(pq, q);
   }
   DimensionVector prevKeys = in;
-  const int result = fused_hash_reduce_run(device, plan, n0, prevKeys, inValues, prev, out, outValues, a, stream);
+  const int result = fused_hash_reduce_run(device, plan, n0, prevKeys, inValues, prev, out, outValues, a, stream, scan_stash_take(device, stream));
   DeferLock lock(device);
   if (result < 0) {
     launch_queue(stream, q, true);
@@ -1860,6 +1928,71 @@
   t_state->limbo[stream] = q;
   *groups = result;
   return true;
+}
+
+namespace {
+bool hinted_operands(const AresFusedExpr &e, bool compareOnly, int batchRows, hipStream_t stream, FastOperands &f) {
+  if (e.arity != 1 && e.arity != 2) return false;
+  if (e.lhs.Type != VectorPartyInput || (e.arity == 2 && e.rhs.Type != ConstantInput)) return false;
+  if (static_cast<int64_t>(e.lhs.Vector.VP.Length) < batchRows) return false;
+  InputVector ins[2] = {e.lhs, e.arity == 2 ? e.rhs : e.lhs};
+  EvalParams p;
+  CallTemps temps;
+  build_params(ins, e.arity, stream, nullptr, nullptr, 0, e.functor, p, temps);
+  return p.a.length >= static_cast<uint32_t>(batchRows) && fast_operands(p, f, compareOnly) && f.step == 4;
+}
+bool hint_fused_batch(int device, hipStream_t stream, const AresFusedQuery &q, int batchRows, int prevSize, int measureBytes) {
+  if (!fuse_available() || !row_space_enabled() || !scan_at_filter_enabled()) return false;
+  if (q.numDims < 1 || q.numDims > kGenericFusedDims || q.numFilters < 1 || q.numFilters > kExtensionFilters) return false;
+  if (batchRows <= 0 || prevSize < 0 || static_cast<int64_t>(batchRows) + prevSize > INT32_MAX) return false;
+  if (measureBytes != 4 && measureBytes != 8) return false;
+  const int mt = q.measure.outType;
+  if (!(mt == Int32 || mt == Uint32 || mt == Float32 || mt == Int64 || mt == Float64) || measureBytes != ((mt == Int64 || mt == Float64) ? 8 : 4))
+    return false;
+  AggSpec a;
+  if (!supported_agg_spec(q.aggFunc, measureBytes, hash_reduce_lds_supported, &a)) return false;
+  ScanHint h;
+  memset(&h, 0, sizeof(h));
+  const int nd = q.numDims;
+  h.nd = nd;
+  h.batchRows = batchRows;
+  h.prevSize = prevSize;
+  auto note = [&](const FastOperands &f) {
+    column_ranges(f, static_cast<uint32_t>(batchRows), [&](const ByteRange &c) { h.ranges[h.numRanges++] = ScanHint::Range{c.lo, c.hi}; });
+  };
+  SinkD sink;
+  FastOperands f;
+  for (int d = 0; d < nd; d++) {
+    const int t = q.dims[d].outType;
+    if (!(t == Int32 || t == Uint32 || t == Float32) || !hinted_operands(q.dims[d], false, batchRows, stream, f)) return false;
+    memset(&sink, 0, sizeof(sink));
+    sink.type = SINK_DIM;
+    sink.dtype = t;
+    sink.width = 4;
+    fused_plan_dim(h.plan, d, f, sink, 4);
+    note(f);
+  }
+  if (!hinted_operands(q.measure, false, batchRows, stream, f)) return false;
+  memset(&sink, 0, sizeof(sink));
+  sink.type = SINK_MEASURE;
+  sink.dtype = mt;
+  sink.width = measureBytes;
+  sink.agg = q.aggFunc;
+  sink.identity = identity_bits(q.aggFunc, mt);
+  if (sink.agg == AGGR_AVG_FLOAT || (measureBytes == 8 && sink.identity != 0)) return false;
+  fused_plan_measure(h.plan, nd, f, sink, measureBytes);
+  note(f);
+  for (int k = 0; k < q.numFilters; k++) {
+    if (!hinted_operands(q.filters[k], true, batchRows, stream, f)) return false;
+    f.idx = nullptr;
+    h.filters[k] = f;
+    note(f);
+  }
+  if (!fused_plan_filters(h.plan, h.filters, static_cast<size_t>(q.numFilters))) return false;
+  if (h.plan.numCols > nd + 2 || fused_plan_narrow(h.plan, nd)) return false;
+  scan_hint_set(device, stream, h);
+  return true;
+}
 }
 
 namespace {
@@ -2174,10 +2307,25 @@
   }
 }
 
+void AresHintFusedBatch(const AresFusedQuery *query, int batchRows, int prevSize, int measureBytes, void *cudaStream, int device) {
+  bool taken = false;
+  try {
+    taken = query != nullptr && device >= 0 && device < kMaxDevices &&
+            hint_fused_batch(device, reinterpret_cast<hipStream_t>(cudaStream), *query, batchRows, prevSize, measureBytes);
+  } catch (std::exception &) {
+  }
+  if (!taken) scan_ahead_count(kScanAheadDeclined);
+}
+
+void AresScanAtFilterStats(unsigned long long *counters) {
+  if (counters) scan_ahead_stats(counters);
+}
+
 CGoCallResHandle InitIndexVector(uint32_t *indexVector, uint32_t start, int indexVectorLength, void *cudaStream,
                                  int device) {
   ARES_ABI_BEGIN_NOFLUSH(device)
   hipStream_t stream = reinterpret_cast<hipStream_t>(cudaStream);
+  scan_hint_init_index(device, stream);
   begin_batch(device, stream, indexVector, start, indexVectorLength);
   if (!defer_iota(device, stream, indexVector, start, indexVectorLength)) {
     flush_deferred(device);
diff --git a/aresdb_amd/csrc/host/abi_library.hpp b/aresdb_amd/csrc/host/abi_library.hpp
--- a/aresdb_amd/csrc/host/abi_library.hpp
+++ b/aresdb_amd/csrc/host/abi_library.hpp
@@ -51,6 +51,8 @@
   decltype(&::Reduce) Reduce;
   decltype(&::HashReduce) HashReduce;
   decltype(&::AresFusedFilterHashReduce) FusedFilterHashReduce = nullptr;
+  decltype(&::AresHintFusedBatch) HintFusedBatch = nullptr;
+  decltype(&::AresScanAtFilterStats) ScanAtFilterStats = nullptr;
   decltype(&::AresFusedFilterSelect) FusedFilterSelect = nullptr;
   decltype(&::AresFusedFilterJoinSelect) FusedFilterJoinSelect = nullptr;
   decltype(&::AresJoinColumnsRun) JoinColumnsRun = nullptr;
@@ -102,6 +104,8 @@
     bind(algoHandle, "WriteGeoShapeDim", WriteGeoShapeDim);
     bind(algoHandle, "Expand", Expand);
     bind(algoHandle, "AresFusedFilterHashReduce", FusedFilterHashReduce, true);
+    bind(algoHandle, "AresHintFusedBatch", HintFusedBatch, true);
+    bind(algoHandle, "AresScanAtFilterStats", ScanAtFilterStats, true);
     bind(algoHandle, "AresFusedFilterSelect", FusedFilterSelect, true);
     bind(algoHandle, "AresFusedFilterJoinSelect", FusedFilterJoinSelect, true);
     bind(algoHandle, "AresJoinColumnsRun", JoinColumnsRun, true);
diff --git a/aresdb_amd/csrc/host/batch_executor.cpp b/aresdb_amd/csrc/host/batch_executor.cpp
--- a/aresdb_amd/csrc/host/batch_executor.cpp
+++ b/aresdb_amd/csrc/host/batch_executor.cpp
@@ -452,21 +452,34 @@
   return true;
 }
 
-bool AresQuery::runBatchFused(const VectorPartySlice *cols, int ncols, int n) {
+bool AresQuery::fusedQuery(AresFusedQuery *q) {
   const Plan &p = *batchPlan;
-  if (!p.useFusedExtension || !p.useHashReduction || fusedDeclined || !lib->FusedFilterHashReduce) return false;
-  if (p.hasGeo || p.isHLL()) return false;
+  if (!p.useHashReduction || p.hasGeo || p.isHLL()) return false;
   if (!p.foreign.empty() || !p.foreignFilters.empty() || baseCounts) return false;
   if (p.dimNodes.empty() || p.dimNodes.size() > 4 || p.filters.size() > 4) return false;
-  columns = cols;
-  numColumns = ncols;
-  Pod<AresFusedQuery> q;
   if (!fusedFilters(p.filters, q->filters, &q->numFilters)) return false;
   for (int t : p.dimTypes)
     if (data_type_bytes(t) != 4) return false;
   if (!fusedDims(q->dims, &q->numDims)) return false;
   if (!fusedExpr(p.measureNode, p.measureType, &q->measure)) return false;
   q->aggFunc = static_cast<AggregateFunction>(p.aggFunc);
+  return true;
+}
+
+void AresQuery::hintBatch() {
+  if (!lib->HintFusedBatch || batchPlan->filters.empty()) return;
+  Pod<AresFusedQuery> q;
+  if (!fusedQuery(&*q)) return;
+  lib->HintFusedBatch(&q.get(), batchRows, resultSize, batchPlan->measureBytes(), stream, device);
+}
+
+bool AresQuery::runBatchFused(const VectorPartySlice *cols, int ncols, int n) {
+  const Plan &p = *batchPlan;
+  if (!p.useFusedExtension || fusedDeclined || !lib->FusedFilterHashReduce) return false;
+  columns = cols;
+  numColumns = ncols;
+  Pod<AresFusedQuery> q;
+  if (!fusedQuery(&*q)) return false;
   size = n;
   prepareForDimAndMeasureEval();
   calls++;
@@ -563,6 +576,7 @@
     return;
   }
   prepareForFiltering(cols, ncols, n, bc, start);
+  hintBatch();
   preExec();
   filter();
   join();
diff --git a/aresdb_amd/csrc/host/query.hpp b/aresdb_amd/csrc/host/query.hpp
--- a/aresdb_amd/csrc/host/query.hpp
+++ b/aresdb_amd/csrc/host/query.hpp
@@ -145,6 +145,8 @@
   bool fusedExpr(int nodeIdx, int outType, AresFusedExpr *e, int *join = nullptr);
   bool fusedFilters(const std::vector<int> &roots, AresFusedExpr *out, int *count, int *joins = nullptr);
   bool fusedDims(AresFusedExpr *out, int *count, int *joins = nullptr);
+  bool fusedQuery(AresFusedQuery *q);
+  void hintBatch();
   bool runBatchFused(const VectorPartySlice *cols, int ncols, int n);
   bool runBatchFusedSelect(const VectorPartySlice *cols, int ncols, int n);
 
diff --git a/include/ares_extensions.h b/include/ares_extensions.h
--- a/include/ares_extensions.h
+++ b/include/ares_extensions.h
@@ -70,6 +70,9 @@
 CGoCallResHandle AresFusedFilterHashReduce(const AresFusedQuery *query, int batchRows, DimensionVector prevKeys,
                                            uint8_t *prevValues, int prevSize, DimensionVector outKeys,
                                            uint8_t *outValues, void *cudaStream, int device);
+
+void AresHintFusedBatch(const AresFusedQuery *query, int batchRows, int prevSize, int measureBytes, void *cudaStream, int device);
+void AresScanAtFilterStats(unsigned long long *counters);
 
 typedef struct {
   int numFilters;
```
